# nipponjo/tts-arabic-pytorch

Hardware: AMD Instinct MI355X
Metric: audio samples/sec (FastPitch+HiFi-GAN, synthetic 64-phoneme inputs) (higher is better)
Workload: dtype f32

## Files before the change

include/ttsamd.h:

```cpp
#ifndef TTSAMD_H
#define TTSAMD_H

#include <stdint.h>

#ifdef __cplusplus
extern "C" {
#endif

#define TTSAMD_OK 0
#define TTSAMD_EINVAL (-1)
#define TTSAMD_EHIP (-2)
#define TTSAMD_ENOMEM (-3)

typedef struct ttsamd_tensor {
    const char* name;
    const float* data;
    int32_t ndim;
    int64_t shape[4];
} ttsamd_tensor;

typedef struct ttsamd_hifigan_cfg {
    int32_t num_mels;
    int32_t upsample_initial_channel;
    int32_t n_ups;
// ... 205 lines not shown
    int32_t hop_length;
    double fmin, fmax;
    int32_t n_thresholds;
    int32_t beta_a, beta_b;
    double boltzmann;
    double resolution;
    double max_transition_rate;
    double switch_prob;
    double no_trough_prob;
    int32_t pad_mode;
} ttsamd_pyin_cfg;
int32_t ttsamd_pyin_tables(const ttsamd_pyin_cfg* cfg, int32_t* dims, double* beta, double* expn, double* norm, double* trans,
                           float* logtrans, float* f0);
int32_t ttsamd_pyin_create(const ttsamd_pyin_cfg* cfg, void** handle);
int32_t ttsamd_pyin_destroy(void* handle);
int64_t ttsamd_pyin_workspace_bytes(void* handle, int32_t batch, int32_t n_frames);
int32_t ttsamd_pyin_forward(void* handle, const float* wave, int64_t wave_stride, const int64_t* nsamples, int32_t batch, int32_t t_max,
                            float* f0, uint8_t* voiced_flag, double* voiced_prob, int32_t* states, int64_t* frames_out,
                            void* workspace, int64_t workspace_bytes, void* stream);
int32_t ttsamd_pyin_obs_offsets(void* handle, int32_t batch, int32_t n_frames, int64_t* obs_offsets);

int32_t ttsamd_resample_create(const float* taps, int32_t o, int32_t n, int32_t width, void** handle);
int32_t ttsamd_resample_destroy(void* handle);
int64_t ttsamd_resample_out_len(void* handle, int64_t nsamples);
int32_t ttsamd_resample_mfma_eligible(void* handle);
int32_t ttsamd_resample_forward(void* handle, const float* wave, int64_t wave_stride, const int64_t* nsamples, int32_t batch, float* out,
                                int64_t out_stride, int64_t* nout, int32_t route, void* stream);

int64_t ttsamd_trim_workspace_bytes(int32_t batch, int64_t wave_stride, int32_t hop_length);
int32_t ttsamd_trim_bounds(const float* wave, int64_t wave_stride, const int64_t* nsamples, int32_t batch, float top_db,
                           int32_t frame_length, int32_t hop_length, float gain, int64_t* bounds, float* peak, void* workspace,
                           int64_t workspace_bytes, void* stream);
int32_t ttsamd_trim_apply(const float* wave, int64_t wave_stride, const int64_t* bounds, const float* peak, float gain, int64_t tail,
                          int32_t batch, float* out, int64_t out_stride, int64_t* lens_out, void* stream);
int32_t ttsamd_frames_compact(const float* mel, const float* extra, const int64_t* lens, int32_t batch, int32_t n_channels,
                              int32_t n_extra, int32_t t_max, float thresh, float* mel_out, float* extra_out, int64_t* lens_out,
                              void* stream);

int32_t ttsamd_tacotron2_create(const ttsamd_tensor* weights, int32_t n_weights,
                                const ttsamd_tacotron2_cfg* cfg, void** handle);
int32_t ttsamd_tacotron2_destroy(void* handle);
int64_t ttsamd_tacotron2_workspace_bytes(void* handle, int32_t batch, int32_t n_tokens, int32_t max_step);
int32_t ttsamd_tacotron2_infer(void* handle, const int64_t* tokens, const int64_t* lengths,
                               const int64_t* speaker_ids, int32_t batch, int32_t n_tokens, int32_t max_step,
                               int64_t dropout_seed, float* mel_post, int32_t* mel_lens, float* alignments,
                               float* mel_raw, int32_t* n_steps, void* workspace, int64_t workspace_bytes,
                               void* stream);

int64_t ttsamd_tacotron2_stream_bytes(void* handle, int32_t batch, int32_t n_tokens, int32_t max_step, int32_t max_chunk_steps);
int32_t ttsamd_tacotron2_stream_begin(void* handle, const int64_t* tokens, const int64_t* lengths, const int64_t* speaker_ids, int32_t batch,
                                      int32_t n_tokens, int32_t max_step, int32_t max_chunk_steps, int64_t dropout_seed,
                                      const int32_t* cut_columns, int32_t rows_to_batch_end, float* mel_raw, int32_t* mel_lens,
                                      float* alignments, void* workspace, int64_t workspace_bytes, void** session, void* stream);
int32_t ttsamd_tacotron2_stream_advance(void* session, int32_t n_steps, int32_t* steps_done, int32_t* ended, int32_t* rows, void* stream);
int32_t ttsamd_tacotron2_stream_end(void* session);
int32_t ttsamd_tacotron2_postnet_halo_frames(void* handle, int32_t* halo);
int64_t ttsamd_tacotron2_postnet_window_bytes(void* handle, int32_t batch, int32_t n_frames);
int32_t ttsamd_tacotron2_postnet_window(void* handle, const float* mel_raw, float* mel_post, int32_t batch, int32_t t_cap, int32_t t_known,
                                        int32_t t0, int32_t t1, int32_t ended, void* workspace, int64_t workspace_bytes, void* stream);

int32_t ttsamd_tagger_create(const ttsamd_tensor* weights, int32_t n_weights, const ttsamd_tagger_cfg* cfg,
                             void** handle);
int32_t ttsamd_tagger_destroy(void* handle);
int64_t ttsamd_tagger_workspace_bytes(void* handle, int32_t batch, int32_t n_chars);
int32_t ttsamd_tagger_forward(void* handle, const int64_t* ids, int32_t batch, int32_t n_chars, float* probs,
                              void* workspace, int64_t workspace_bytes, void* stream);


int64_t ttsamd_conv1d_packed_floats(int32_t cout, int32_t cin, int32_t k);
int32_t ttsamd_conv1d(const float* x, const float* w, const float* bias, const int64_t* lens,
                      int32_t batch, int32_t cin, int32_t cout, int32_t k, int32_t dilation,
                      int32_t lin, float in_slope, int32_t relu_out, float* y, float* packed,
                      void* stream);
int32_t ttsamd_conv1d_ex(const float* x, const float* w, const float* bias, const float* res, const int64_t* lens, int32_t batch,
                         int32_t cin, int32_t cout, int32_t k, int32_t dilation, int32_t lin, float in_slope,
                         int32_t relu_out, int32_t mode, float div, float* y, float* packed, void* stream);
int32_t ttsamd_conv1d_splitk(const float* x, const float* w, const float* bias, const float* res, const int64_t* lens, int32_t batch,
                             int32_t cin, int32_t cout, int32_t k, int32_t dilation, int32_t lin, float in_slope,
                             int32_t relu_out, int32_t mode, float div, float* y, float* packed, float* splitk_ws, int64_t splitk_floats,
                             void* stream);
int32_t ttsamd_conv_last_launch(int32_t* route, int32_t* ksplit);
int32_t ttsamd_conv1d_route(int32_t batch, int32_t cin, int32_t cout, int32_t k, int32_t dilation, int32_t lin, float in_slope,
                            int32_t relu_out, int32_t has_res, int32_t mode, int64_t splitk_floats, int32_t* route, int32_t* ksplit);
int64_t ttsamd_convt_packed_floats(int32_t cin, int32_t cout, int32_t u);
int64_t ttsamd_convt_wino_packed_floats(int32_t cin, int32_t cout, int32_t u);
int32_t ttsamd_convt_wino_pack_weight(const float* w, const float* bias, int32_t cin, int32_t cout, int32_t u, float* out);
int32_t ttsamd_conv_transpose1d(const float* x, const float* w, const float* bias, const int64_t* lens, int32_t batch, int32_t cin,
                                int32_t cout, int32_t u, int32_t lin, float in_slope, float* y, float* packed, void* stream);

int64_t ttsamd_resblock_pair_packed_floats(int32_t channels, int32_t k, int32_t variant);
int32_t ttsamd_resblock_pair(const float* x, float* y, const float* w1, const float* b1, const float* w2, const float* b2,
                             int32_t channels, int32_t k, int32_t dil, const int64_t* lens, int32_t len_mul, int32_t L,
                             int32_t batch, int32_t mode, float div, float slope, int32_t variant, float* packed, int64_t packed_floats,
                             void* stream);
int32_t ttsamd_resblock_pair_route(int32_t batch, int32_t channels, int32_t k, int32_t dilation, int32_t L, int32_t* kernel, int32_t* ntw,
                                   int32_t* wino_phases, int32_t* points, const char** name);

int64_t ttsamd_resblock2_packed_floats(int32_t channels, int32_t k, int32_t variant);
int32_t ttsamd_resblock2(const float* x, float* y, const float* w1, const float* b1, const float* w2, const float* b2, int32_t channels,
                         int32_t k, int32_t dil1, int32_t dil2, const int64_t* lens, int32_t len_mul, int32_t L, int32_t batch, int32_t mode,
                         float div, float slope, int32_t variant, float* packed, int64_t packed_floats, void* stream);

int32_t ttsamd_bfo_pack(const float* x, int32_t batch, int32_t channels, int32_t len, float slope, void* out, void* stream);
int32_t ttsamd_bfo_unpack(const void* in, int32_t batch, int32_t channels, int32_t len, float slope, float* out, void* stream);
int64_t ttsamd_bfo_weight_elems(int32_t cout, int32_t cin, int32_t k, int32_t up);
int32_t ttsamd_bfo_pack_weight(const float* w, int32_t cout, int32_t cin, int32_t k, int32_t up, uint16_t* out);
int32_t ttsamd_bfo_conv1d(const void* x, const void* w_packed, const float* bias, const void* res, const void* sum_in,
                          const int64_t* lens, int32_t len_mul, int32_t batch, int32_t cin, int32_t cout, int32_t k,
                          int32_t dilation, int32_t up, int32_t len_in, int32_t mode, float div, float res_slope,
                          float out_slope, void* y, float* y_f32, const float* res_f32, void* stream);
int32_t ttsamd_bfo_resblock_pair(const void* x, const void* w1, const float* b1, const void* w2, const float* b2,
                                 const void* sum_in, const int64_t* lens, int32_t len_mul, int32_t batch, int32_t channels,
                                 int32_t k, int32_t dilation, int32_t len, int32_t mode, float div, float in_slope,
                                 float mid_slope, float out_slope, void* y, void* stream);
int32_t ttsamd_bfo_resblock_chain(const void* x, const void* const* w1, const float* const* b1, const void* const* w2,
                                  const float* const* b2, const int32_t* dilations, const void* sum_in, const int64_t* lens,
                                  int32_t len_mul, int32_t batch, int32_t channels, int32_t len, int32_t mode, float div,
                                  float in_slope, float mid_slope, float out_slope, void* y, void* stream, int32_t k);
int32_t ttsamd_bfo_conv_post(const void* x, const float* w, const float* bias, const int64_t* lens, int32_t len_mul,
                             int32_t batch, int32_t channels, int32_t len, float* wave, int64_t wave_stride, void* stream);

int32_t ttsamd_bfo3_pack(const float* x, int32_t batch, int32_t channels, int32_t len, float slope, void* out, void* stream);
int32_t ttsamd_bfo3_unpack(const void* in, int32_t batch, int32_t channels, int32_t len, float slope, float* out, void* stream);
int64_t ttsamd_bfo3_weight_elems(int32_t cout, int32_t cin, int32_t k, int32_t up);
int32_t ttsamd_bfo3_pack_weight(const float* w, int32_t cout, int32_t cin, int32_t k, int32_t up, uint16_t* out);
int32_t ttsamd_bfo3_conv1d(const void* x, const void* w_packed, const float* bias, const void* res, const void* sum_in,
                           const int64_t* lens, int32_t len_mul, int32_t batch, int32_t cin, int32_t cout, int32_t k,
                           int32_t dilation, int32_t up, int32_t len_in, int32_t mode, float div, float res_slope,
                           float out_slope, void* y, float* y_f32, const float* res_f32, void* stream);
int32_t ttsamd_bfo3_resblock_pair(const void* x, const void* w1, const float* b1, const void* w2, const float* b2,
                                  const void* sum_in, const int64_t* lens, int32_t len_mul, int32_t batch, int32_t channels,
                                  int32_t k, int32_t dilation, int32_t len, int32_t mode, float div, float in_slope,
                                  float mid_slope, float out_slope, void* y, void* stream);
int32_t ttsamd_bfo3_resblock_chain(const void* x, const void* const* w1, const float* const* b1, const void* const* w2,
                                   const float* const* b2, const int32_t* dilations, const void* sum_in, const int64_t* lens,
                                   int32_t len_mul, int32_t batch, int32_t channels, int32_t len, int32_t mode, float div,
                                   float in_slope, float mid_slope, float out_slope, void* y, void* stream);
int32_t ttsamd_bfo3_conv_post(const void* x, const float* w, const float* bias, const int64_t* lens, int32_t len_mul,
                              int32_t batch, int32_t channels, int32_t len, float* wave, int64_t wave_stride, void* stream);

int32_t ttsamd_set_precision(int32_t precision);
int32_t ttsamd_get_precision(void);

#define TTSAMD_DP_ID_BYTES 128
#define TTSAMD_DP_HIFIGAN 0
#define TTSAMD_DP_FASTPITCH 1
int32_t ttsamd_dp_unique_id(void* id128 );
int32_t ttsamd_dp_init(int32_t rank, int32_t world, const void* id128 , void** comm);
int32_t ttsamd_dp_destroy(void* comm);
int32_t ttsamd_dp_rank(void* comm);
int32_t ttsamd_dp_world(void* comm);
int32_t ttsamd_dp_broadcast(void* comm, void* buf, int64_t nbytes, int32_t root, void* stream);
int32_t ttsamd_dp_broadcast_weights(void* comm, int32_t kind, void* handle, int32_t root, void* stream);
int32_t ttsamd_dp_allgather(void* comm, const void* send, void* recv, int64_t nbytes_per_rank, void* stream);
int32_t ttsamd_dp_pack_audio(const float* wave, int64_t wave_stride, const int64_t* nsamples, int32_t batch,
                             int64_t n_max, float* packed, void* stream);
int32_t ttsamd_dp_gather_audio(void* comm, const float* packed, float* recv, const int64_t* counts,
                               const int64_t* offsets, int32_t root, void* stream);

int32_t ttsamd_hifigan_halo_frames(void* handle, int32_t* left , int32_t* right );
int32_t ttsamd_denoiser_halo_frames(void);
#define TTSAMD_STREAM_MAX_WINDOWS 64
int32_t ttsamd_stream_gather(const float* pool, int32_t n_slots, int32_t num_mels, int32_t t_cap, const int32_t* slot ,
                             const int32_t* start , const int32_t* len , int32_t n_windows, int32_t w_max,
                             float* batch, int64_t* lens, void* stream);
int32_t ttsamd_stream_emit(const float* wave, int32_t n_windows, int32_t w_max, int32_t hop, const int32_t* core_off ,
// ... 84 lines not shown
```

profiles/launch_classes.py:

```python
import csv
import re
import sys
from collections import defaultdict


def classes(path):
    d = defaultdict(lambda: [0, 0])
    other = 0
    with open(path) as f:
        for r in csv.DictReader(f):
            dur = int(r['End_Timestamp']) - int(r['Start_Timestamp'])
            m = re.search(r'conv1d_wino4_f32<(\d+), (\d+), (\d+), (\d+), (\d+), (\d+)>', r['Kernel_Name'])
            if not m:
                other += dur
                continue
            k, noct, nst, epi, lp, pt = map(int, m.groups())
            key = (pt, k, lp, 'residual' if epi == 3 else 'plain', int(r['Grid_Size_X']) // int(r['Workgroup_Size_X']))
            d[key][0] += 1
            d[key][1] += dur
    return d, other


a, oa = classes(sys.argv[1])
b, ob = classes(sys.argv[2])
print(f'{"groups":>6} {"k":>3} {"window":>7} {"epilogue":>9} {"blocks":>7} {"calls":>6} {"us parent":>10} {"us tree":>9} {"ratio":>6}')
ta = tb = 0
for key in sorted(set(a) | set(b), key=lambda t: (-t[0], t[1], t[2], t[3], t[4])):
    ca, da = a.get(key, (0, 0))
    cb, db = b.get(key, (0, 0))
    ta += da
    tb += db
    ua, ub = (da / ca / 1e3 if ca else float('nan')), (db / cb / 1e3 if cb else float('nan'))
    print(f'{"seven" if key[0] == 7 else "six":>6} {key[1]:3d} {"vector" if key[2] == 1 else "strip":>7} {key[3]:>9} {key[4]:7d} {max(ca, cb):6d} '
          f'{ua:10.1f} {ub:9.1f} {ub / ua:6.3f}')
print(f'sum over the conv1d_wino4_f32 launches: {ta / 1e6:.2f} -> {tb / 1e6:.2f} ms; every other kernel: {oa / 1e6:.2f} -> {ob / 1e6:.2f} ms (whole trace)')
```

tts-arabic-pytorch_amd/csrc/api.hip:

```cpp
#include <cerrno>
#include <cstdio>
#include <cstdlib>
#include <cstring>
#include <algorithm>
#include <atomic>
#include <mutex>
#include <string>
#include <vector>

#include "kernels.hpp"

namespace ttsamd {

static thread_local std::string g_err;

void set_error(const char* fmt, ...) {
    char buf[1024];
    va_list ap;
    va_start(ap, fmt);
    vsnprintf(buf, sizeof(buf), fmt, ap);
    va_end(ap);
    g_err = buf;
}

// ... 155 lines not shown

__global__ void pack_conv_weight_kernel(const float* __restrict__ w, int cout, int cin, int k, int cp,
                                        float* __restrict__ out) {
    const int64_t i = (int64_t)blockIdx.x * 256 + threadIdx.x;
    const int64_t n = (int64_t)cin * k * cp;
    if (i >= n) return;
    const int pq = (int)(i % 4);
    const int co = (int)((i / 4) % cp);
    const int kk = (int)((i / (4 * (int64_t)cp)) % 2);
    const int t = (int)((i / (8 * (int64_t)cp)) % k);
    const int o = (int)(i / (8 * (int64_t)cp * k));
    out[i] = co < cout ? w[((int64_t)co * cin + (8 * o + 2 * pq + kk)) * k + t] : 0.f;
}

__global__ void pack_convt_weight_kernel(const float* __restrict__ w, int cin, int cout, int u, int cp, float* __restrict__ out) {
    const int64_t i = (int64_t)blockIdx.x * 256 + threadIdx.x;
    const int64_t n = (int64_t)u * cin * 2 * cp;
    if (i >= n) return;
    const int pq = (int)(i % 4);
    const int co = (int)((i / 4) % cp);
    const int kk = (int)((i / (4 * (int64_t)cp)) % 2);
    const int t = (int)((i / (8 * (int64_t)cp)) % 2);
    const int o = (int)((i / (16 * (int64_t)cp)) % (cin / 8));
    const int rho = (int)(i / (16 * (int64_t)cp * (cin / 8)));
    const int kidx = (rho + u / 2) % u + t * u;
    out[i] = co < cout ? w[((int64_t)(8 * o + 2 * pq + kk) * cout + co) * (2 * u) + kidx] : 0.f;
}

__global__ void pack_convt_wino_kernel(const float* __restrict__ w, const float* __restrict__ bias, int cin, int cout, int u,
                                       float* __restrict__ out) {
    const int64_t i = (int64_t)blockIdx.x * 256 + threadIdx.x;
    const int rows = u * cout;
    const int64_t n = (int64_t)6 * cin * rows;
    if (i >= n + rows) return;
    if (i >= n) {
        out[i] = bias ? bias[(i - n) / u] : 0.f;
        return;
    }
    const int pq = (int)(i & 3);
    const int64_t r = i >> 2;
    const int row = (int)(r % rows);
    const int64_t r2 = r / rows;
    const int kk = (int)(r2 & 1);
    const int64_t r3 = r2 >> 1;
    const int t = (int)(r3 % 6), o = (int)(r3 / 6);
    const int co = row / u, j = row % u;
    const float* g = w + ((int64_t)(8 * o + 2 * pq + kk) * cout + co) * 2 * u;
    const double g0 = g[j + u], g1 = g[j];
    out[i] = t == 0 ? (float)(g0 / 4) : (t == 1 ? (float)(-(g0 + g1) / 6) : (t == 2 ? (float)(-(g0 - g1) / 6) :
             (t == 3 ? (float)(g0 / 24 + g1 / 12) : (t == 4 ? (float)(g0 / 24 - g1 / 12) : 0.f))));
}

__global__ void split_bf16_kernel(const float* __restrict__ packed, int64_t n, unsigned short* __restrict__ out) {
    const int64_t i = (int64_t)blockIdx.x * 256 + threadIdx.x;
    if (i >= n) return;
    const float f = packed[i];
    unsigned u = __float_as_uint(f);
    u += 0x7fffu + ((u >> 16) & 1u);
    const unsigned h = u >> 16;
    const float r = f - __uint_as_float(h << 16);
    unsigned v = __float_as_uint(r);
    v += 0x7fffu + ((v >> 16) & 1u);
    out[i] = (unsigned short)h;
    out[n + i] = (unsigned short)(v >> 16);
}

namespace {
struct OptDesc { const char* name; int kind; long long lo, hi; };
const OptDesc kOpts[OPT_COUNT] = {
#define TTS_OPT_DESC(name, kind, lo, hi) {"TTSAMD_" #name, kind, lo, hi},
    TTS_OPTIONS(TTS_OPT_DESC)
#undef TTS_OPT_DESC
};
std::atomic<const char*> g_opt[OPT_COUNT];
std::once_flag g_opt_once;
std::string g_opt_env_error;

bool opt_valid(const OptDesc& d, const char* v) {
    if (!v || !*v) return false;
    char* end = nullptr;
    errno = 0;
    const long long x = std::strtoll(v, &end, d.kind == 1 ? 16 : 10);
    if (!(errno == 0 && end != v && *end == '\0' && x >= d.lo && x <= d.hi)) return false;
    if (&d == &kOpts[OPT_WINO4] && (((x & 32) && !(x & 2)) || ((x & 64) && !(x & 4)) || ((x & 128) && !(x & 8)))) return false;
    return true;
}
void opt_init() {
    std::call_once(g_opt_once, [] {
        for (int i = 0; i < OPT_COUNT; ++i) {
            const char* e = std::getenv(kOpts[i].name);
            if (!e || !*e) continue;
            if (!opt_valid(kOpts[i], e)) {
                if (g_opt_env_error.empty()) {
                    char buf[256];
                    std::snprintf(buf, sizeof buf, "%s='%s' in the environment is not a valid value (%s in [%llx, %llx])", kOpts[i].name, e,
                                  kOpts[i].kind == 1 ? "hex mask" : "integer", kOpts[i].lo, kOpts[i].hi);
                    g_opt_env_error = buf;
                }
                continue;
            }
            g_opt[i].store(strdup(e), std::memory_order_release);
        }
    });
}
int opt_find(const char* name) {
    if (!name) return -1;
    for (int i = 0; i < OPT_COUNT; ++i)
        if (std::strcmp(name, kOpts[i].name) == 0 || std::strcmp(name, kOpts[i].name + 7) == 0) return i;
    return -1;
}
}

int64_t opt_int(Opt o, int64_t unset) {
    opt_init();
    const char* v = g_opt[o].load(std::memory_order_acquire);
    return v ? (int64_t)std::strtoll(v, nullptr, kOpts[o].kind == 1 ? 16 : 10) : unset;
}

}

using namespace ttsamd;

extern "C" {

const char* ttsamd_last_error(void) { return g_err.c_str(); }
int32_t ttsamd_version(void) { return TTSAMD_ABI_VERSION; }

int32_t ttsamd_set_option(const char* name, const char* value) {
    opt_init();
    const int i = opt_find(name);
    TTS_REQUIRE(i >= 0, "set_option: unknown option '%s' (ttsamd_option_name lists them)", name ? name : "(null)");
    if (!value || !*value) {
        g_opt[i].store(nullptr, std::memory_order_release);
        return 0;
    }
    TTS_REQUIRE(opt_valid(kOpts[i], value), "set_option: %s='%s' is not a valid value (%s in [%llx, %llx])", kOpts[i].name, value,
                kOpts[i].kind == 1 ? "hex mask" : "integer", kOpts[i].lo, kOpts[i].hi);
    g_opt[i].store(strdup(value), std::memory_order_release);
    return 0;
}
int32_t ttsamd_get_option(const char* name, char* value, int32_t capacity) {
    opt_init();
    const int i = opt_find(name);
    TTS_REQUIRE(i >= 0 && value && capacity > 0, "get_option: unknown option '%s' or no buffer", name ? name : "(null)");
    const char* v = g_opt[i].load(std::memory_order_acquire);
    std::snprintf(value, (size_t)capacity, "%s", v ? v : "");
    return 0;
}
const char* ttsamd_option_name(int32_t index) { return (index >= 0 && index < OPT_COUNT) ? kOpts[index].name : nullptr; }
int32_t ttsamd_options_check(void) {
    opt_init();
    TTS_REQUIRE(g_opt_env_error.empty(), "%s", g_opt_env_error.c_str());
    return 0;
}

int32_t ttsamd_device_ok(void) {
    int n = 0;
    if (hipGetDeviceCount(&n) != hipSuccess || n <= 0) return 0;
    hipDeviceProp_t prop;
    if (hipGetDeviceProperties(&prop, 0) != hipSuccess) return 0;
    return std::string(prop.gcnArchName).rfind("gfx950", 0) == 0 ? 1 : 0;
}

int32_t ttsamd_hifigan_create(const ttsamd_tensor* weights, int32_t n, const ttsamd_hifigan_cfg* cfg, void** handle) {
    HifiGan* h = nullptr;
    const int32_t rc = hifigan_create(weights, n, cfg, &h);
    if (rc == 0) *handle = h;
// ... 508 lines not shown
            const double g0 = g[3 * s], g1 = g[3 * s + 1], g2 = g[3 * s + 2];
            v = j == 0 ? (float)g0 : (j == 1 ? (float)((g0 + g1 + g2) * 0.5) : (j == 2 ? (float)((g0 - g1 + g2) * 0.5) : (float)g2));
        } else {
            const int l = (t - 4 * ns) >> 1;
            v = ((t - 4 * ns) & 1) ? -g[3 * ns + l] : g[3 * ns + l];
        }
    }
    out[i] = v;
}

int32_t ttsamd_conv1d_ex(const float* x, const float* w, const float* bias, const float* res, const int64_t* lens, int32_t batch,
                         int32_t cin, int32_t cout, int32_t k, int32_t dilation, int32_t lin, float in_slope,
                         int32_t relu_out, int32_t mode, float div, float* y, float* packed, void* stream) {
    return ttsamd_conv1d_splitk(x, w, bias, res, lens, batch, cin, cout, k, dilation, lin, in_slope, relu_out, mode, div, y, packed, nullptr,
                                0, stream);
}

static int32_t conv1d_params(ConvParams& p, const float* x, const float* bias, const float* res, const int64_t* lens, int32_t batch,
                             int32_t cin, int32_t cout, int32_t k, int32_t dilation, int32_t lin, float in_slope, int32_t relu_out,
                             int32_t mode, float div, float* y, float* packed, float* splitk_ws, int64_t splitk_floats) {
    TTS_REQUIRE(mode >= 0 && mode <= 2 && (mode != 2 || div != 0.f), "conv1d: bad mode / div");
    TTS_REQUIRE(relu_out == 0 || mode == 0, "conv1d: relu_out with an accumulate mode (mode %d) is not defined", mode);
    const int cp = cout_padded(cout);
    const int64_t n = (int64_t)cin * k * cp;
    std::memset(&p, 0, sizeof(p));
    p.x = x; p.x_bs = (int64_t)cin * lin; p.x_cs = lin;
    p.w = packed; p.bias = bias;
    p.precision = default_precision();
    if (p.precision != 0) p.w_bf16 = packed + n;
    if ((k == 3 || k == 7 || k == 11) && p.precision == 0 && cin % 8 == 0) {
        p.w_wino = packed + 2 * n;
        p.w_wino4 = p.w_wino + (int64_t)cin * wino2_groups(k) * cp;
        if (wino44_groups(k) != 0) p.w_wino44 = p.w_wino4 + (int64_t)cin * wino4_groups(k) * cp;
    }
    p.y = y; p.y_bs = (int64_t)cout * lin; p.y_cs = lin; p.y_ts = 1;
    p.lens_in = lens; p.lens_out = lens; p.len_in_mul = 1; p.len_out_mul = 1;
    p.Lin = lin; p.Nout = lin; p.Cin = cin; p.Cout = cout; p.CoutP = cp; p.K = k;
    p.dil = dilation; p.pad = (k * dilation - dilation) / 2;
    p.res = res; p.r_bs = (int64_t)cout * lin; p.r_cs = lin;
    p.n_phase = 1; p.in_slope = in_slope; p.relu_out = relu_out; p.mode = mode; p.div = div; p.batch = batch;
    if (splitk_ws != nullptr && splitk_floats > 0) { p.splitk_ws = splitk_ws; p.splitk_floats = splitk_floats; }
    return 0;
}

int32_t ttsamd_conv1d_splitk(const float* x, const float* w, const float* bias, const float* res, const int64_t* lens, int32_t batch,
                             int32_t cin, int32_t cout, int32_t k, int32_t dilation, int32_t lin, float in_slope,
                             int32_t relu_out, int32_t mode, float div, float* y, float* packed, float* splitk_ws, int64_t splitk_floats,
                             void* stream) {
    TTS_REQUIRE(x && w && y && packed, "conv1d: null argument");
    TTS_REQUIRE(splitk_floats >= 0 && (splitk_ws != nullptr || splitk_floats == 0), "conv1d: %lld split-K floats without a workspace",
                (long long)splitk_floats);
    ConvParams p;
    TTS_TRY(conv1d_params(p, x, bias, res, lens, batch, cin, cout, k, dilation, lin, in_slope, relu_out, mode, div, y, packed, splitk_ws,
                          splitk_floats));
    hipStream_t s = (hipStream_t)stream;
    const int cp = p.CoutP;
    const int64_t n = (int64_t)cin * k * cp;
    const auto blocks = [](int64_t floats) { return dim3((unsigned)((floats + 255) / 256)); };
    hipLaunchKernelGGL(pack_conv_weight_kernel, blocks(n), dim3(256), 0, s, w, cout, cin, k, cp, packed);
    TTS_CHECK_HIP(hipGetLastError());
    if (p.w_bf16 != nullptr) {
        hipLaunchKernelGGL(split_bf16_kernel, blocks(n), dim3(256), 0, s, packed, n, reinterpret_cast<unsigned short*>(packed + n));
        TTS_CHECK_HIP(hipGetLastError());
    }
    if (p.w_wino != nullptr) {
        hipLaunchKernelGGL(pack_wino2_weight_kernel, blocks((int64_t)cin * wino2_groups(k) * cp), dim3(256), 0, s, w, cout, cin, k, cp,
                           const_cast<float*>(p.w_wino));
        TTS_CHECK_HIP(hipGetLastError());
        hipLaunchKernelGGL(pack_wino4_weight_kernel, blocks((int64_t)cin * wino4_groups(k) * cp), dim3(256), 0, s, w, cout, cin, k, cp,
                           const_cast<float*>(p.w_wino4));
        TTS_CHECK_HIP(hipGetLastError());
    }
    if (p.w_wino44 != nullptr) {
        hipLaunchKernelGGL(pack_wino44_weight_kernel, blocks((int64_t)cin * wino44_groups(k) * cp), dim3(256), 0, s, w, cout, cin, k, cp,
                           const_cast<float*>(p.w_wino44));
        TTS_CHECK_HIP(hipGetLastError());
    }
    prof_begin(s, 2.0 * cout * cin * k);
    const int32_t rc = launch_conv(p, s);
    prof_end(s);
    return rc;
}

int32_t ttsamd_conv1d_route(int32_t batch, int32_t cin, int32_t cout, int32_t k, int32_t dilation, int32_t lin, float in_slope,
                            int32_t relu_out, int32_t has_res, int32_t mode, int64_t splitk_floats, int32_t* route, int32_t* ksplit) {
    TTS_REQUIRE(route && ksplit, "conv1d_route: null argument");
    TTS_REQUIRE(batch >= 1 && cin >= 1 && cout >= 1 && k >= 1 && lin >= 1 && dilation >= 1 && dilation <= 5 && splitk_floats >= 0,
                "conv1d_route: bad shape");
    float* const any = reinterpret_cast<float*>((uintptr_t)256);
    ConvParams p;
    TTS_TRY(conv1d_params(p, any, any, has_res ? any : nullptr, nullptr, batch, cin, cout, k, dilation, lin, in_slope, relu_out, mode, 1.f, any,
                          any, any, splitk_floats));
    TTS_REQUIRE(p.precision == 0, "conv1d_route: the bf16 launchers keep their own choices (precision %d)", p.precision);
    const ConvRoute r = conv_route(p, conv_route_opts());
    TTS_REQUIRE(r.id >= 0 && (relu_out < 2 || k == 1 || k == 5), "conv1d_route: no fp32 kernel takes k = %d, Cin = %d, relu_out = %d", k, cin, relu_out);
    *route = r.id;
    *ksplit = r.ksplit;
    return 0;
}

int32_t ttsamd_conv1d(const float* x, const float* w, const float* bias, const int64_t* lens, int32_t batch,
                      int32_t cin, int32_t cout, int32_t k, int32_t dilation, int32_t lin, float in_slope,
                      int32_t relu_out, float* y, float* packed, void* stream) {
    return ttsamd_conv1d_ex(x, w, bias, nullptr, lens, batch, cin, cout, k, dilation, lin, in_slope, relu_out, 0, 1.f, y, packed, stream);
}

int32_t ttsamd_conv_last_launch(int32_t* route, int32_t* ksplit) {
    TTS_REQUIRE(route && ksplit, "conv_last_launch: null argument");
    last_conv_launch(route, ksplit);
    return 0;
}

int64_t ttsamd_convt_packed_floats(int32_t cin, int32_t cout, int32_t u) {
    if (cin < 1 || cout < 1 || u < 1) return 0;
    return 2 * (int64_t)u * cin * 2 * cout_padded(cout) + (convt_wino_packable(cin, cout, u) ? (int64_t)(6 * cin + 1) * u * cout : 0);
}

int64_t ttsamd_convt_wino_packed_floats(int32_t cin, int32_t cout, int32_t u) {
    return convt_wino_packable(cin, cout, u) ? (int64_t)(6 * cin + 1) * u * cout : 0;
}

int32_t ttsamd_convt_wino_pack_weight(const float* w, const float* bias, int32_t cin, int32_t cout, int32_t u, float* out) {
    TTS_REQUIRE(w && out, "convt_wino_pack_weight: null argument");
    TTS_REQUIRE(convt_wino_packable(cin, cout, u), "convt_wino_pack_weight: cin %d (a multiple of 16), cout %d, u %d (2 / 8, u cout a multiple of 64)",
                cin, cout, u);
    pack_convt_wino_weight(w, bias, cin, cout, u, out, out + (int64_t)6 * cin * u * cout);
    return 0;
}

int32_t ttsamd_conv_transpose1d(const float* x, const float* w, const float* bias, const int64_t* lens, int32_t batch, int32_t cin,
                                int32_t cout, int32_t u, int32_t lin, float in_slope, float* y, float* packed, void* stream) {
    TTS_REQUIRE(x && w && y && packed, "conv_transpose1d: null argument");
    TTS_REQUIRE(batch >= 1 && cin >= 8 && cin % 8 == 0 && cout >= 1 && lin >= 1, "conv_transpose1d: batch %d, cin %d (a multiple of 8), cout %d, lin %d",
                batch, cin, cout, lin);
    TTS_REQUIRE(u >= 2 && u % 2 == 0, "conv_transpose1d: stride %d (kernel 2 u, padding u / 2: u even)", u);
    TTS_REQUIRE((int64_t)lin * u < ((int64_t)1 << 31) / 4 / cout, "conv_transpose1d: %d x %d x %d outputs per row", cout, lin, u);
    hipStream_t s = (hipStream_t)stream;
    const int cp = cout_padded(cout);
    const int64_t n = (int64_t)u * cin * 2 * cp;
    hipLaunchKernelGGL(pack_convt_weight_kernel, dim3((unsigned)((n + 255) / 256)), dim3(256), 0, s, w, cin, cout, u, cp, packed);
    TTS_CHECK_HIP(hipGetLastError());
    unsigned short* planes = nullptr;
    if (default_precision() != 0) {
        planes = reinterpret_cast<unsigned short*>(packed + n);
        hipLaunchKernelGGL(split_bf16_kernel, dim3((unsigned)((n + 255) / 256)), dim3(256), 0, s, packed, n, planes);
        TTS_CHECK_HIP(hipGetLastError());
    }
    float* wino = nullptr;
    if (default_precision() == 0 && convt_wino_packable(cin, cout, u) && opt_int(OPT_CONVT_WINO, 1) != 0) {
        wino = packed + 2 * n;
        const int64_t nw = (int64_t)(6 * cin + 1) * u * cout;
        hipLaunchKernelGGL(pack_convt_wino_kernel, dim3((unsigned)((nw + 255) / 256)), dim3(256), 0, s, w, bias, cin, cout, u, wino);
        TTS_CHECK_HIP(hipGetLastError());
    }
    ConvParams p;
    std::memset(&p, 0, sizeof(p));
    p.batch = batch;
    p.lens_in = lens; p.lens_out = lens;
    prof_begin(s, 2.0 * cout * cin * 2 * u);
    const int32_t rc = launch_upsampler(p, x, packed, planes, bias, y, cin, cout, u, 2 * u, lin, 1, in_slope, opt_int(OPT_CONVT, 1) != 0, s, wino,
                                        wino ? wino + (int64_t)6 * cin * u * cout : nullptr);
    prof_end(s);
    return rc;
}

int64_t ttsamd_resblock_pair_packed_floats(int32_t channels, int32_t k, int32_t variant) {
    if (channels < 1 || k < 1) return 0;
    const int64_t n = 2 * (int64_t)channels * k * channels;
    const int nwino = (variant == 4 ? 1 : (variant == 5 ? 2 : 0));
    if (variant == 6) return n + ((k == 3 || k == 7 || k == 11) ? 2 * (int64_t)channels * wino4_groups(k) * channels : 0);
    if (variant == 7) return n + 2 * (int64_t)channels * wino44_groups(k) * channels;
    return n + ((k == 3 || k == 7 || k == 11) ? nwino * (int64_t)channels * wino2_groups(k) * channels : 0);
}

int32_t ttsamd_resblock_pair(const float* x, float* y, const float* w1, const float* b1, const float* w2, const float* b2,
                             int32_t channels, int32_t k, int32_t dil, const int64_t* lens, int32_t len_mul, int32_t L,
                             int32_t batch, int32_t mode, float div, float slope, int32_t variant, float* packed, int64_t packed_floats,
                             void* stream) {
    TTS_REQUIRE(x && y && w1 && b1 && w2 && b2 && packed && channels % 32 == 0 && k >= 1 && batch >= 1 && L >= 1 && len_mul >= 1 &&
                mode >= 0 && mode <= 2, "resblock_pair: bad argument");
    TTS_REQUIRE(packed_floats >= ttsamd_resblock_pair_packed_floats(channels, k, variant),
                "resblock_pair: `packed` holds %lld floats, variant %d at C = %d, k = %d needs %lld (ttsamd_resblock_pair_packed_floats)",
                (long long)packed_floats, variant, channels, k, (long long)ttsamd_resblock_pair_packed_floats(channels, k, variant));
    hipStream_t s = (hipStream_t)stream;
    PairConv c[2] = {{nullptr, b1, nullptr, nullptr, nullptr}, {nullptr, b2, nullptr, nullptr, nullptr}};
    float* next = packed;
    const auto pack = [&](void (*kernel)(const float*, int, int, int, int, float*), int groups, const float* w, const float*& form) {
        const int64_t nw = (int64_t)channels * groups * channels;
        hipLaunchKernelGGL(kernel, dim3((unsigned)((nw + 255) / 256)), dim3(256), 0, s, w, channels, channels, k, channels, next);
        form = next;
        next += nw;
        return hipGetLastError();
// ... 137 lines not shown
```

tts-arabic-pytorch_amd/csrc/common.hpp:

```cpp
#pragma once
#include <hip/hip_runtime.h>
#include <stdint.h>
#include <atomic>
#include <cstdarg>
#include <cstdio>
#include <cstdlib>
#include <string>

#include "../../include/ttsamd.h"

namespace ttsamd {

void set_error(const char* fmt, ...);

#define TTS_CHECK_HIP(expr)                                                         \
    do {                                                                            \
        hipError_t e_ = (expr);                                                     \
        if (e_ != hipSuccess) {                                                     \
            ttsamd::set_error("%s failed: %s (%s:%d)", #expr, hipGetErrorString(e_), \
                              __FILE__, __LINE__);                                  \
            return TTSAMD_EHIP;                                                     \
        }                                                                           \
    } while (0)

#define TTS_REQUIRE(cond, ...)              \
    do {                                    \
        if (!(cond)) {                      \
            ttsamd::set_error(__VA_ARGS__); \
            return TTSAMD_EINVAL;           \
        }                                   \
    } while (0)

#define TTS_TRY(expr)               \
    do {                            \
        int32_t rc_ = (expr);       \
        if (rc_ != 0) return rc_;   \
    } while (0)

inline int64_t align_up(int64_t x, int64_t a) { return (x + a - 1) / a * a; }

inline hipError_t lds_opt_in(const void* fn, int bytes, std::atomic<uint64_t>& done) {
    int dev = 0;
    hipError_t e = hipGetDevice(&dev);
    if (e != hipSuccess) return e;
    if (dev >= 0 && dev < 64 && ((done.load(std::memory_order_acquire) >> dev) & 1)) return hipSuccess;
    e = hipFuncSetAttribute(fn, hipFuncAttributeMaxDynamicSharedMemorySize, bytes);
    if (e == hipSuccess && dev >= 0 && dev < 64) done.fetch_or(1ull << dev, std::memory_order_release);
    return e;
}

#define TTS_OPTIONS(X)                                                                                     \
    X(HIFIGAN_STREAMS, 0, 0, 1)    \
    X(WINO, 0, 0, 1)                                              \
    X(WINO2, 0, 0, 31)             \
    X(WINO4, 0, 0, 255)            \
    X(FUSED_PAIR, 0, 0, 1)                   \
    X(FUSED2, 0, 0, 1)                                           \
    X(FUSED2_MASK, 1, 0, 0x1ff)               \
    X(FUSED2_MASK_N1, 1, 0, 0x1ff)          \
    X(FUSED2_WB, 0, 0, 2)                     \
    X(PAIR4, 0, 0, 2)              \
    X(CONVT, 0, 0, 1)                              \
    X(CONVT_WINO, 0, 0, 2)         \
    X(BFO, 0, 0, 1)                \
    X(BFO_CHAIN, 0, 0, 1)                           \
    X(BFO_CHAIN7, 0, 0, 1)                                 \
    X(BFO_FF, 0, 0, 1)                              \
    X(BFO_SPLITK, 0, 0, 1)                                              \
    X(BFO_SMALL_TILES, 0, 0, 1)            \
    X(BF16_ATTN, 0, 0, 1)                                         \
    X(BF16_PACKED_T, 0, 0, 1)                   \
    X(ATT_RA, 0, 1, 4)                             \
    X(ATT_SPLIT, 0, 0, 1)                      \
    X(XCD_W, 0, 0, 1)                            \
    X(XCD_WMAX_KB, 0, 0, 1 << 20)     \
    X(DEEP_SPLITK, 0, 0, 1)        \
    X(TACO_PERSISTENT, 0, 0, 2)    \
    X(TACO_SEG, 0, 8, 1 << 20)     \
    X(RESBLOCK2_PAIR, 1, 0, 0x3f)
enum Opt : int {
#define TTS_OPT_ENUM(name, kind, lo, hi) OPT_##name,
    TTS_OPTIONS(TTS_OPT_ENUM)
#undef TTS_OPT_ENUM
    OPT_COUNT
};
int64_t opt_int(Opt o, int64_t unset);

struct Arena {
    char* base;
    int64_t size;
    int64_t off = 0;
    bool ok = true;
    Arena(void* p, int64_t n) : base((char*)p), size(n) {}
    template <typename T>
    T* take(int64_t count) {
        int64_t bytes = align_up(count * (int64_t)sizeof(T), 256);
        if (base != nullptr && off + bytes > size) ok = false;
        T* r = base ? (T*)(base + off) : nullptr;
        off += bytes;
        return r;
    }
};

struct ConvParams {
    const float* x;
    int64_t x_bs;
    int32_t x_cs;
    const float* w;
    const void* w_bf16;
    const float* w_wino;
    const float* w_wino4;
    int32_t precision;
    const float* bias;
    float* y;
    int64_t y_bs;
    int32_t y_cs, y_ts;
    const float* res;
    int64_t r_bs;
    int32_t r_cs;
    const int64_t* lens_in;
    const int64_t* lens_out;
    int32_t len_in_mul, len_out_mul;
    int32_t Lin, Nout;
    int32_t Cin, Cout, CoutP, K;
    int32_t dil, pad;
    int32_t n_phase;
    int32_t phase_p;
    float in_slope;
    const float* scale;
    int32_t relu_out;
    int32_t mode;
    float div;
    int32_t batch;
    float* splitk_ws;
    int64_t splitk_floats;
    int32_t ksplit;
    int32_t y_packed;
    float pack_slope;
    int32_t x_packed;
    int32_t xcd_w;
    int32_t tile_major;
    int32_t compact;
    unsigned long long* timing;
    const float* w_wino44;
    int32_t res_late;
};
constexpr int64_t kSplitKFloats = 4 << 20;
constexpr int64_t kSplitKFloatsFp = 8 << 20;

void conv_log(const char* kind, int K, int cin, int cout, int nout, int batch, int has_res, int mode, int len_mul, int ragged,
              int n_phase);
bool compact_order(const void* lens, int batch);
int32_t launch_conv(const ConvParams& p, hipStream_t stream);
struct ConvRouteOpts { int wino, wino2, wino4, deep_splitk; };
struct ConvRoute {
    int id;
    int ksplit;
    int epi;
    int co_blk, nt_blk;
};
ConvRouteOpts conv_route_opts();
ConvRoute conv_route(const ConvParams& p, const ConvRouteOpts& o);
inline bool conv_rows_aligned(const ConvParams& p) {
    return (p.y_cs & 3) == 0 && (p.y_bs & 3) == 0 && ((uintptr_t)p.y & 15) == 0 &&
           (!p.res || ((p.r_cs & 3) == 0 && (p.r_bs & 3) == 0 && ((uintptr_t)p.res & 15) == 0));
}
constexpr int conv_chunk_channels(int k, int nt_blk, int co_blk) {
    return (k == 3 && nt_blk == 128 && co_blk == 128) ? 16 : (k == 1 ? 32 : (k == 2 ? 16 : 8));
}
void note_conv_launch(int32_t route, int32_t ksplit);
void last_conv_launch(int32_t* route, int32_t* ksplit);
bool convt_supported(const ConvParams& p);
int32_t launch_convt(const ConvParams& p, hipStream_t stream);
int32_t launch_upsampler(ConvParams& p, const float* x, const float* w, const void* w_bf16, const float* bias, float* y, int cin, int cout,
                         int u, int kt, int L, int len_mul, float in_slope, bool convt_ok, hipStream_t stream, const float* w_wino = nullptr,
                         const float* bias_wino = nullptr);
bool convt_wino_packable(int cin, int cout, int u);
void pack_convt_wino_weight(const float* w, const float* bias, int cin, int cout, int u, float* out_w, float* out_bias);
bool convt_wino_supported(const ConvParams& p, const float* w_wino, const float* bias_wino);
int32_t launch_convt_wino(const ConvParams& p, const float* w_wino, const float* bias_wino, hipStream_t stream);
struct PairRouteOpts { int fused_pair, fused2, fused2_mask, fused2_mask_n1, fused2_wb, pair4; };
struct ConvForms { bool wino2, wino4, wino44; };
struct PairShape { int32_t channels, k, dil, L, batch; bool square; const float *x, *y; ConvForms forms; int32_t precision; };
enum PairKernel : int32_t { PAIR_NONE = 0, PAIR_GEN1 = 1, PAIR_GEN2 = 2, PAIR_F43 = 3 };
struct PairRoute { int32_t kernel, ntw, wm, points; const char* name; };
PairRouteOpts pair_route_opts();
PairRoute pair_route(const PairShape& s, const PairRouteOpts& o);
PairRoute pair_route_of_variant(int32_t variant, int32_t channels, int32_t dil);
bool pair2_phases_built(int32_t channels, int32_t dil, int32_t ntw, int32_t wm);
ConvForms hifigan_conv_forms(int cin, int cout, int k);
struct PairConv { const float *w, *b, *w_wino2, *w_wino4, *w_wino44; };
struct PairArgs { int32_t channels, k, dil; const float* x; float* y; PairConv c1, c2; const int64_t* lens; int32_t len_mul, L, batch, mode; float div, slope; };
int32_t launch_pair(const PairRoute& r, const PairArgs& a, hipStream_t stream);
bool fused_pair_supported(int32_t channels, int32_t k, int32_t dil, int32_t L, const float* x, const float* y);
int32_t launch_fused_pair(const PairArgs& a, hipStream_t stream);
bool fused_pair2_supported(int32_t channels, int32_t k, int32_t dil, int32_t L, const float* x, const float* y, int32_t ntw);
int32_t launch_fused_pair2(const PairArgs& a, const PairRoute& r, hipStream_t stream);
bool fused_pair4_supported(int32_t channels, int32_t k, int32_t dil, int32_t L, const float* x, const float* y);
int32_t launch_fused_pair4(const PairArgs& a, const PairRoute& r, hipStream_t stream);
bool resblock2_conv_supported(int32_t channels, int32_t k, int32_t dil, int32_t L, const float* x, const float* y);
int32_t launch_resblock2_conv(int32_t channels, const float* x, float* y, const float* w, const float* b, int32_t k, int32_t dil,
                              const int64_t* lens, int32_t len_mul, int32_t L, int32_t batch, int32_t mode, float div, float slope,
                              hipStream_t stream);
bool resblock2_pair_supported(int32_t channels, int32_t k, int32_t d1, int32_t d2, int32_t L, const float* x, const float* y);
int32_t launch_resblock2_pair(int32_t channels, const float* x, float* y, const float* w1, const float* b1, const float* w2,
                              const float* b2, int32_t k, int32_t d1, int32_t d2, const int64_t* lens, int32_t len_mul, int32_t L,
                              int32_t batch, int32_t mode, float div, float slope, hipStream_t stream);
int32_t launch_wino(const ConvParams& p, hipStream_t stream);
void pack_wino_weight(const float* w, int cout, int cin, float* out);
int wino2_groups(int k);
__device__ __host__ constexpr int wino2_tile(int d, int npair) { return (2 * npair / ((d & 1) ? 4 * d : 2 * d)) * ((d & 1) ? 4 * d : 2 * d); }
int32_t launch_wino2(const ConvParams& p, hipStream_t stream);
void pack_wino2_weight(const float* w, int cout, int cin, int k, float* out);
int wino4_groups(int k);
int wino44_groups(int k);
constexpr int kWino4Default = 255;
__device__ __host__ constexpr int wino4_tile(int d, int ntup) { return (4 * ntup / (4 * d)) * (4 * d); }
__host__ __device__ constexpr int wino4_pk_tuples(int n, int d) { return d * ((n + 4 * d - 1) / (4 * d)); }
__host__ __device__ constexpr int wino4_pk_tiles(int n, int d) { return (wino4_pk_tuples(n, d) + 63) / 64; }
__host__ __device__ constexpr int wino4_pk_col(int t, int d) { return (t / d) * 4 * d + t % d; }
__host__ __device__ constexpr int wino4_pk_q0(int tile, int d) { return (64 * tile / d) * 4 * d; }
__host__ __device__ constexpr int wino4_pk_r0(int tile, int d) { return 64 * tile % d; }
int32_t launch_splitk_reduce(const ConvParams& q, hipStream_t stream);
int32_t launch_wino4(const ConvParams& p, const ConvRoute& r, hipStream_t stream);
void wino4_filter_groups(const float* g, int k, float* o);
void pack_wino4_weight(const float* w, int cout, int cin, int k, float* out);
void wino44_filter_groups(const float* g, int k, float* o);
void pack_wino44_weight(const float* w, int cout, int cin, int k, float* out);
void pack_conv_weight(const float* w, int cout, int cin, int k, float* out);
void pack_convt_weight(const float* w, int cin, int cout, int kt, int u, int p, float* out);
inline int cout_padded(int cout) { return (int)align_up(cout, 32); }
void split_packed_bf16(const float* packed, int64_t n, uint16_t* out);
int32_t default_precision();

#ifdef __HIPCC__
template <int EXTRA = 0, bool PACKED = false>
__device__ __forceinline__ bool live_tile(const int64_t* __restrict__ lens, const int mul, const int n_max, const int tile_w,
                                          const int batch, const unsigned lin, int& b, int& tile, const int pk_dil = 0) {
    const int lane = threadIdx.x & 63;
    unsigned base = 0;
    for (int u0 = 0; u0 < batch; u0 += 64) {
        int n = 0;
        if constexpr (EXTRA != 0) {
            if (u0 + lane < batch) {
                const int len = (int)lens[u0 + lane] * mul;
                n = (max(min(n_max, len > 0 ? len + EXTRA : 0), 0) + tile_w - 1) / tile_w;
            }
        } else if constexpr (PACKED) {
            if (u0 + lane < batch) n = wino4_pk_tiles(max(min(n_max, (int)lens[u0 + lane] * mul), 0), pk_dil);
        } else {
            if (u0 + lane < batch) n = (max(min(n_max, (int)lens[u0 + lane] * mul), 0) + tile_w - 1) / tile_w;
        }
        int incl = n;
#pragma unroll
        for (int d = 1; d < 64; d <<= 1) {
            const int t = __shfl_up(incl, d, 64);
            if (lane >= d) incl += t;
        }
        const unsigned total = (unsigned)__shfl(incl, 63, 64);
        if (lin < base + total) {
            const unsigned long long m = __ballot(base + (unsigned)incl > lin);
            const int l = __ffsll((long long)m) - 1;
            b = u0 + l;
            tile = (int)(lin - base) - (__shfl(incl, l, 64) - __shfl(n, l, 64));
            return true;
        }
        base += total;
    }
    return false;
}
#endif

}
```

tts-arabic-pytorch_amd/csrc/conv_mfma.hip:

```cpp
#include <cstdio>
#include <cstdlib>
#include <cstring>

#include <algorithm>

#include "conv_mfma_common.hpp"
#include "conv_row_epilogue.hpp"

namespace ttsamd {

template <int K, int NT_BLK, int CO_BLK>
struct Geo {
    static constexpr int KC = conv_chunk_channels(K, NT_BLK, CO_BLK);
    static constexpr int NOCT = KC / 8;
    static constexpr int WS = NT_BLK + (K - 1) * DMAX;
    static constexpr int XI = 2 * NOCT * WS;
    static constexpr int NXI = (XI + 255) / 256;
    static constexpr int W4 = NOCT * K * 2 * CO_BLK;
    static constexpr int NW = (W4 + 255) / 256;
    static constexpr int BUF4 = XI + W4;
    static constexpr int NSTAGE = (CO_BLK > 32 && 3 * BUF4 * 16 <= 80 * 1024 && !(K == 7 && CO_BLK == 64 && NT_BLK >= 128)) ? 3 : 2;
    static constexpr int NGRP = NOCT * K;
};

// ... 312 lines not shown
                    const int r = h * 8 + r8;
                    const int co = co_w0 + i * 32 + (r & 3) + 8 * (r >> 2) + 4 * kk;
                    const int coc = min(co, Cout - 1);
                    bv[r8] = bias ? bias[coc] : 0.f;
                    sv[r8] = scale ? scale[coc] : 1.f;
                    rv[r8] = rb ? rb[(int64_t)coc * r_cs + (int64_t)qc * y_ts] : 0.f;
                    pv[r8] = mode != 0 ? yb[(int64_t)coc * y_cs + (int64_t)qc * y_ts] : 0.f;
                }
#pragma unroll
                for (int r8 = 0; r8 < 8; ++r8) {
                    const int r = h * 8 + r8;
                    const int co = co_w0 + i * 32 + (r & 3) + 8 * (r >> 2) + 4 * kk;
                    float v = acc[i][j][r] + bv[r8];
                    if constexpr (K == 1 || K == 5) { if (relu_out == 2) v = 0.5f * v * (1.0f + erff(v * 0.70710678118654752440f)); }
                    v = v * sv[r8] + rv[r8];
                    if (relu_out == 1) v = fmaxf(v, 0.f);
                    if constexpr (K == 1 || K == 5) { if (relu_out == 3) v = tanhf(v); }
                    if (mode == 1) v = pv[r8] + v;
                    else if (mode == 2) v = (pv[r8] + v) / div;
                    if (q_ok && co < Cout) yb[(int64_t)co * y_cs + (int64_t)q * y_ts] = v;
                }
            }
        }
    }
    }
}

template <int K, int MT, int NTL, int WM, int WN, int EPI>
__global__ __launch_bounds__(256, kConvMinWaves) void conv1d_mfma_f32(const ConvParams p) {
    extern __shared__ __attribute__((aligned(16))) float4 smem4[];
    constexpr int NT_BLK = WN * NTL * 32;
    unsigned bx_ = blockIdx.x, by_ = blockIdx.y, bz_ = blockIdx.z;
    if (p.xcd_w) {
        const unsigned lin = bx_ + gridDim.x * (by_ + gridDim.y * bz_), xcd = lin & 7u, slot = lin >> 3;
        const unsigned nct = gridDim.y, g = (unsigned)p.xcd_w & 0xffu, per = nct / g;
        unsigned rest;
        if (p.xcd_w & 0x100) {
            rest = (slot / per) * (8u / g) + xcd / g;
            by_ = xcd % g + g * (slot % per);
        } else {
            const unsigned idx2 = slot * (8u / g) + xcd / g;
            rest = idx2 / per;
            by_ = xcd % g + g * (idx2 % per);
        }
        bx_ = rest % gridDim.x; bz_ = rest / gridDim.x;
    }
    int b = p.tile_major ? (int)((bx_ + bz_) % (unsigned)p.batch) : (int)bz_;
    int q0 = (p.tile_major ? bz_ : bx_) * NT_BLK;
    if (p.compact) {
        int tile = 0;
        if (!live_tile(p.lens_out, p.len_out_mul, p.Nout, NT_BLK, p.batch, bz_ * gridDim.x + bx_, b, tile)) return;
        b = __builtin_amdgcn_readfirstlane(b);
        q0 = __builtin_amdgcn_readfirstlane(tile) * NT_BLK;
    }
    conv_tile<K, MT, NTL, WM, WN, EPI>(p, smem4, b, q0, by_);
}

__global__ __launch_bounds__(256) void splitk_reduce_kernel(const ConvParams p) {
    const int b = blockIdx.z, co = blockIdx.y, q = blockIdx.x * 256 + threadIdx.x;
    int n_out = p.Nout;
    if (p.lens_out) n_out = min(n_out, (int)p.lens_out[b] * p.len_out_mul);
    if (q >= n_out) return;
    const int64_t per = (int64_t)p.batch * p.Cout * p.Nout;
    const float* __restrict__ pp = p.splitk_ws + ((int64_t)b * p.Cout + co) * p.Nout + q;
    float v = 0.f;
    for (int k0 = 0; k0 < p.ksplit; k0 += 8) {
        float tq[8];
#pragma unroll
        for (int j = 0; j < 8; ++j) tq[j] = pp[(int64_t)min(k0 + j, p.ksplit - 1) * per];
#pragma unroll
        for (int j = 0; j < 8; ++j) v = (k0 + j < p.ksplit) ? v + tq[j] : v;
    }
    v += p.bias ? p.bias[co] : 0.f;
    if (p.relu_out == 2) v = 0.5f * v * (1.0f + erff(v * 0.70710678118654752440f));
    v = v * (p.scale ? p.scale[co] : 1.f) + (p.res ? p.res[(int64_t)b * p.r_bs + (int64_t)co * p.r_cs + q] : 0.f);
    if (p.relu_out == 1) v = fmaxf(v, 0.f);
    else if (p.relu_out == 3) v = tanhf(v);
    float* yp = p.y + (int64_t)b * p.y_bs + (int64_t)co * p.y_cs + q;
    if (p.mode == 1) v = *yp + v;
    else if (p.mode == 2) v = (*yp + v) / p.div;
    *yp = v;
}

static thread_local int32_t t_last_route = -1, t_last_ksplit = 0;
void note_conv_launch(int32_t route, int32_t ksplit) { t_last_route = route; t_last_ksplit = ksplit; }
void last_conv_launch(int32_t* route, int32_t* ksplit) { *route = t_last_route; *ksplit = t_last_ksplit; }

int32_t launch_splitk_reduce(const ConvParams& q, hipStream_t stream) {
    dim3 rg((q.Nout + 255) / 256, q.Cout, q.batch);
    hipLaunchKernelGGL(splitk_reduce_kernel, rg, dim3(256), 0, stream, q);
    TTS_CHECK_HIP(hipGetLastError());
    return 0;
}

template <int K, int MT, int NTL, int WM, int WN, int EPI>
static int32_t launch_epi(const ConvParams& q, dim3 grid, size_t lds, hipStream_t stream) {
    static std::atomic<uint64_t> lds_done{0};
    const auto kern = conv1d_mfma_f32<K, MT, NTL, WM, WN, EPI>;
    TTS_CHECK_HIP(lds_opt_in((const void*)kern, (int)lds, lds_done));
    hipLaunchKernelGGL(kern, grid, dim3(256), lds, stream, q);
    TTS_CHECK_HIP(hipGetLastError());
    return 0;
}

bool compact_order(const void* lens, int batch) { return lens != nullptr && batch > 1; }

constexpr int kXcdWeightKB = 3000;

template <int K, int MT, int NTL, int WM, int WN>
static int32_t launch_cfg(const ConvParams& p, int ksplit, hipStream_t stream) {
    constexpr int CO_BLK = WM * MT * 32, NT_BLK = WN * NTL * 32;
    using G = Geo<K, NT_BLK, CO_BLK>;
    TTS_REQUIRE(p.Cin % G::KC == 0, "conv: Cin=%d must be a multiple of %d for K=%d", p.Cin, G::KC, K);
    const size_t lds = (size_t)G::NSTAGE * G::BUF4 * sizeof(float4);
    dim3 grid((p.Nout + NT_BLK - 1) / NT_BLK, (p.CoutP / CO_BLK) * p.n_phase, p.batch);
    ConvParams q = p;
    q.ksplit = ksplit;
    q.tile_major = 0;
    q.compact = compact_order(p.lens_out, p.batch) ? 1 : 0;
    {
        const bool xw = opt_int(OPT_XCD_W, 1) != 0;
        const unsigned nct = grid.y;
        const unsigned g = (nct % 8 == 0) ? 8 : (nct % 4 == 0 ? 4 : (nct % 2 == 0 ? 2 : 1));
        const bool can = xw && p.n_phase == 1 && ((int64_t)grid.x * grid.y * grid.z) % 8 == 0;
        q.xcd_w = (can && g > 1) ? (int)g : 0;
        const int64_t wmax = opt_int(OPT_XCD_WMAX_KB, kXcdWeightKB) * 1024;
        if (can && wmax > 0 && nct > 1) {
            const int64_t wbytes = (int64_t)p.CoutP * p.Cin * K * 4;
            unsigned g2 = g;
            while (g2 > 1 && wbytes / (g2 / 2) <= wmax) g2 /= 2;
            if (nct / g2 > 1 && ((int64_t)grid.x * grid.z * g2) % 8 == 0)
                q.xcd_w = (int)g2 | 0x100 | (q.xcd_w << 16);
        }
    }
    if (q.ksplit > 1 && (q.xcd_w & 0x100)) q.xcd_w >>= 16;
    if (q.xcd_w & 0x100) q.xcd_w &= 0x1ff;
    grid.y *= q.ksplit;
    const bool vec_ok = q.ksplit == 1 && p.y_ts == 1 && p.n_phase == 1 && conv_rows_aligned(p);
    TTS_REQUIRE(p.relu_out < 2 || K == 1 || K == 5, "conv: GELU / tanh epilogues are built for kernel sizes 1 and 5 only (K=%d)", K);
    const bool pre_ok = p.res != nullptr && !p.res_late && p.scale == nullptr && p.relu_out < 2 &&
                        (int64_t)p.Cout * std::max(p.r_cs, p.y_cs) * 4 < ((int64_t)1 << 31);
    const int epi = !vec_ok ? 2 : (p.relu_out >= 2 ? 1 : (pre_ok ? 3 : 0));
    int32_t rc;
    if (epi == 3) rc = launch_epi<K, MT, NTL, WM, WN, 3>(q, grid, lds, stream);
    else if (epi == 0) rc = launch_epi<K, MT, NTL, WM, WN, 0>(q, grid, lds, stream);
    else if (epi == 1) rc = launch_epi<K, MT, NTL, WM, WN, (K == 1 || K == 5) ? 1 : 2>(q, grid, lds, stream);
    else rc = launch_epi<K, MT, NTL, WM, WN, 2>(q, grid, lds, stream);
    if (rc != 0) return rc;
    if (q.ksplit > 1) return launch_splitk_reduce(q, stream);
    return 0;
}

template <int K>
static int32_t launch_k(const ConvParams& p, const ConvRoute& r, hipStream_t stream) {
    if (r.co_blk == 128 && r.nt_blk == 64) return launch_cfg<K, 1, 2, 4, 1>(p, r.ksplit, stream);
    if (r.co_blk == 64 && r.nt_blk == 128) return launch_cfg<K, 1, 2, 2, 2>(p, r.ksplit, stream);
    if (r.co_blk == 128 && r.nt_blk == 128) return launch_cfg<K, 2, 2, 2, 2>(p, r.ksplit, stream);
    if (r.co_blk == 64 && r.nt_blk == 256) return launch_cfg<K, 2, 2, 1, 4>(p, r.ksplit, stream);
    if (r.co_blk == 64 && r.nt_blk == 64) return launch_cfg<K, 1, 1, 2, 2>(p, r.ksplit, stream);
    if (r.co_blk == 32 && r.nt_blk == 256) return launch_cfg<K, 1, 2, 1, 4>(p, r.ksplit, stream);
    return launch_cfg<K, 1, 1, 1, 4>(p, r.ksplit, stream);
}

void conv_log(const char* kind, int K, int cin, int cout, int nout, int batch, int has_res, int mode, int len_mul, int ragged,
              int n_phase) {
    static FILE* f = [] { const char* e = getenv("TTSAMD_CONV_LOG"); return e ? fopen(e, "a") : (FILE*)nullptr; }();
    if (!f) return;
    fprintf(f, "%s,%d,%d,%d,%d,%d,%d,%d,%d,%d,%d\n", kind, K, cin, cout, nout, batch, has_res, mode, len_mul, ragged, n_phase);
    fflush(f);
}

int32_t launch_conv(const ConvParams& p, hipStream_t stream) {
    TTS_REQUIRE(p.CoutP % 32 == 0 && p.CoutP >= p.Cout, "conv: bad CoutP=%d", p.CoutP);
    TTS_REQUIRE(p.n_phase >= 1 && p.batch >= 1, "conv: bad n_phase/batch");
    TTS_REQUIRE(p.dil >= -DMAX && p.dil <= DMAX && p.dil != 0, "conv: dilation %d outside [-%d,%d]", p.dil, DMAX, DMAX);
    if (p.Nout <= 0) return 0;
    const ConvRoute r = p.precision == 0 ? conv_route(p, conv_route_opts()) : ConvRoute{0, 1, 0, 0, 0};
    conv_log(p.precision == 0 ? (r.id >= 3 ? "f32_wino4" : (r.id > 0 ? "f32_wino" : "f32")) : "bf16", p.K, p.Cin, p.Cout, p.Nout, p.batch, p.res != nullptr, p.mode, p.len_out_mul,
             p.lens_out != nullptr, p.n_phase);
    if (p.precision != 0) return launch_conv_bf16_any(p, stream);
    TTS_REQUIRE(!p.x_packed && !p.y_packed, "conv: packed bf16 activations exist only in the bf16 mode");
    if (r.id >= 0) note_conv_launch(r.id, r.ksplit);
    if (r.id > 0) return r.id >= 3 ? launch_wino4(p, r, stream) : (r.id == 2 ? launch_wino2(p, stream) : launch_wino(p, stream));
    switch (p.K) {
        case 1: return launch_k<1>(p, r, stream);
        case 2: return launch_k<2>(p, r, stream);
        case 3: return launch_k<3>(p, r, stream);
        case 5: return launch_k<5>(p, r, stream);
        case 7: return launch_k<7>(p, r, stream);
        case 11: return launch_k<11>(p, r, stream);
        default:
            set_error("conv: kernel size %d not instantiated (1,2,3,5,7,11)", p.K);
            return TTSAMD_EINVAL;
    }
}

void pack_conv_weight(const float* w, int cout, int cin, int k, float* out) {
    const int cp = cout_padded(cout);
    for (int o = 0; o < cin / 8; ++o)
        for (int t = 0; t < k; ++t)
            for (int kk = 0; kk < 2; ++kk) {
                float* dst = out + (((int64_t)o * k + t) * 2 + kk) * cp * 4;
                for (int co = 0; co < cp; ++co)
                    for (int pq = 0; pq < 4; ++pq)
                        dst[co * 4 + pq] = co < cout ? w[((int64_t)co * cin + (8 * o + 2 * pq + kk)) * k + t] : 0.f;
            }
}

static inline uint16_t host_bf16_rne(float f) {
    uint32_t u;
    memcpy(&u, &f, 4);
    u += 0x7fffu + ((u >> 16) & 1u);
    return (uint16_t)(u >> 16);
}
static inline float host_bf16_to_f(uint16_t h) {
    uint32_t u = (uint32_t)h << 16;
    float f;
    memcpy(&f, &u, 4);
    return f;
}

void split_packed_bf16(const float* packed, int64_t n, uint16_t* out) {
    for (int64_t i = 0; i < n; ++i) {
        const uint16_t h = host_bf16_rne(packed[i]);
        out[i] = h;
        out[n + i] = host_bf16_rne(packed[i] - host_bf16_to_f(h));
    }
}

void pack_convt_weight(const float* w, int cin, int cout, int kt, int u, int p, float* out) {
    const int cp = cout_padded(cout);
    for (int rho = 0; rho < u; ++rho) {
        const int ka = (rho + p) % u;
        for (int o = 0; o < cin / 8; ++o)
            for (int t = 0; t < 2; ++t) {
                const int kidx = ka + t * u;
                for (int kk = 0; kk < 2; ++kk) {
                    float* dst = out + ((((int64_t)rho * (cin / 8) + o) * 2 + t) * 2 + kk) * cp * 4;
                    for (int co = 0; co < cp; ++co)
                        for (int pq = 0; pq < 4; ++pq)
                            dst[co * 4 + pq] = (co < cout && kidx < kt)
                                                   ? w[((int64_t)(8 * o + 2 * pq + kk) * cout + co) * kt + kidx]
                                                   : 0.f;
                }
            }
    }
}

}
```

tts-arabic-pytorch_amd/csrc/conv_route.hip:

```cpp
#include <algorithm>

#include "common.hpp"

namespace ttsamd {

ConvRouteOpts conv_route_opts() {
    return {(int)opt_int(OPT_WINO, 1), (int)opt_int(OPT_WINO2, 31), (int)opt_int(OPT_WINO4, kWino4Default), (int)opt_int(OPT_DEEP_SPLITK, 1)};
}

static int wino4_ksplit(const ConvParams& p, int64_t blocks) {
    constexpr int sk_blocks = 192, sk_target = 224;
    if (blocks >= sk_blocks || p.splitk_ws == nullptr) return 1;
    const int n_chunks = p.Cin / (p.K == 1 ? 32 : (p.K == 3 ? 16 : 8));
    const int64_t per = (int64_t)p.batch * p.Cout * p.Nout;
    int64_t ks = std::min<int64_t>((sk_target + blocks - 1) / blocks, n_chunks / 8);
    ks = std::min<int64_t>(ks, p.splitk_floats / std::max<int64_t>(per, 1));
    return ks >= 2 ? (int)ks : 1;
}

static ConvRoute route_direct(const ConvParams& p, const ConvRouteOpts& o) {
    const int K = p.K;
    ConvRoute r = {0, 1, 0, 0, 0};
    if (K != 1 && K != 2 && K != 3 && K != 5 && K != 7 && K != 11) return ConvRoute{-1, 1, 0, 0, 0};
    auto blocks = [&](int co_blk, int nt_blk) -> int64_t {
        return (int64_t)((p.Nout + nt_blk - 1) / nt_blk) * (p.CoutP / co_blk) * p.n_phase * p.batch;
    };
    auto tile = [&](int co_blk, int nt_blk) { r.co_blk = co_blk, r.nt_blk = nt_blk; };
    const int64_t want = blocks(64, 64) <= 1024 ? (int64_t)200 : (int64_t)768;
    const bool tiny = p.Nout <= 96;
    if (p.CoutP % 128 == 0) {
        const bool few_long = p.Cin >= 256 && p.CoutP <= p.Cin && !tiny && blocks(128, 128) < 4 * want;
        if (few_long && K == 3 && blocks(128, 64) >= want) tile(128, 64);
        else if (few_long && K >= 7 && blocks(64, 128) >= want) tile(64, 128);
        else if (K < 11 && !tiny && blocks(128, 128) >= want && (K != 3 || p.Cin % 16 == 0)) tile(128, 128);
        else if (K == 11 && !tiny && blocks(64, 256) >= want) tile(64, 256);
        else if (p.splitk_ws && p.Cin >= 1024 && !tiny && blocks(128, 64) >= 160 && blocks(128, 64) < 320 &&
                 (int64_t)2 * p.batch * p.Cout * p.Nout <= p.splitk_floats && o.deep_splitk != 0) tile(128, 64);
        else if (blocks(128, 64) >= want || (tiny && blocks(64, 64) < 2 * want)) tile(128, 64);
        else tile(64, 64);
    } else if (p.CoutP % 64 == 0) tile(64, !tiny && blocks(64, 256) >= want ? 256 : 64);
    else tile(32, !tiny && blocks(32, 256) >= want ? 256 : 128);
    const int kc = conv_chunk_channels(K, r.nt_blk, r.co_blk);
    if (p.Cin % kc != 0) return ConvRoute{-1, 1, 0, r.co_blk, r.nt_blk};
    const int64_t nblk = blocks(r.co_blk, r.nt_blk), per = (int64_t)p.batch * p.Cout * p.Nout;
    const int n_chunks = p.Cin / kc;
    constexpr int sk_blocks = 320, sk_target = 640, sk_chunks = 8;
    if (p.splitk_ws && p.n_phase == 1 && p.y_ts == 1 && nblk < sk_blocks && n_chunks >= sk_chunks) {
        int64_t ks = std::min<int64_t>((sk_target + nblk - 1) / nblk, n_chunks / 4);
        ks = std::min<int64_t>(ks, p.splitk_floats / per);
        if (ks >= 2) r.ksplit = (int)ks;
    }
    return r;
}

static ConvRoute route_wino(const ConvParams& p, const ConvRouteOpts& o) {
    constexpr ConvRoute direct = {0, 1, 0, 0, 0};
    if (o.wino == 0) return direct;
    const bool rows_vec_ok = conv_rows_aligned(p) && (int64_t)p.Cout * std::max(std::max(p.r_cs, p.y_cs), 1) * 4 < ((int64_t)1 << 31);
    if (p.n_phase != 1 || p.y_ts != 1 || p.CoutP % 64 != 0 || !(p.in_slope >= 0.f && p.in_slope <= 1.f) || !rows_vec_ok) return direct;
    if (p.K == 1) {
        if (!((o.wino4 & 16) && p.w != nullptr && p.dil == 1 && p.pad == 0 && p.Cin % 32 == 0 && !p.x_packed && !p.y_packed)) return direct;
        const int64_t tiles1 = (int64_t)((p.Nout + 255) / 256) * (p.CoutP / 64) * p.batch;
        const int ks1 = wino4_ksplit(p, tiles1);
        return (tiles1 * ks1 >= 512 && p.Nout >= 256) ? ConvRoute{3, ks1, 0, 0, 0} : direct;
    }
    if ((p.w_wino == nullptr && p.w_wino4 == nullptr) || (p.K != 3 && p.K != 7 && p.K != 11)) return direct;
    if ((p.dil != 1 && p.dil != 3 && p.dil != 5) || p.pad != p.dil * (p.K - 1) / 2 || p.Cin % 8 != 0 || p.scale != nullptr || p.relu_out >= 2)
        return direct;
    const int kbit = p.K == 3 ? 1 : (p.K == 7 ? 2 : 4);
    auto takes = [&](int mask) { return (mask & kbit) && (p.dil == 1 || (mask & 8)) && (p.K != 3 || p.Cin % 16 == 0); };
    if (p.w_wino4 != nullptr) {
        if (takes(o.wino4)) {
            const int bo4 = wino4_tile(p.dil, 64);
            const int64_t tiles4 = (int64_t)((p.Nout + bo4 - 1) / bo4) * (p.CoutP / 64) * p.batch;
            const int ks4 = wino4_ksplit(p, tiles4);
            if (tiles4 * ks4 >= 192 && p.Nout >= 256) {
                const bool seven = p.w_wino44 != nullptr && p.K != 3 && (o.wino4 & (p.K == 7 ? 32 : 64)) != 0;
                const int epi = p.dil == 1 ? (ks4 != 1 ? 0 : (p.res != nullptr ? 3 : 4))
                                           : (((o.wino4 & 128) && p.res == nullptr && p.mode == 0 && ks4 == 1) ? 7 : 0);
                return ConvRoute{(epi == 7 ? 7 : 3) + (seven ? 1 : 0), ks4, epi, 0, 0};
            }
        }
        if (p.w_wino == nullptr) return direct;
    }
    const bool rows64 = p.CoutP % 128 != 0;
    const bool w2 = takes(o.wino2) && (!rows64 || (o.wino2 & 16));
    const bool w1 = p.K == 3 && p.dil == 1 && !rows64;
    if (!w2 && !w1) return direct;
    const int bo = wino2_tile(p.dil, rows64 ? 128 : 64);
    const int64_t blocks = (int64_t)((p.Nout + bo - 1) / bo) * (p.CoutP / (rows64 ? 64 : 128)) * p.batch;
    if (blocks < 192 || p.Nout < 256) return direct;
    return ConvRoute{w2 ? 2 : 1, 1, 0, 0, 0};
}

ConvRoute conv_route(const ConvParams& p, const ConvRouteOpts& o) {
    const ConvRoute r = route_wino(p, o);
    return r.id != 0 ? r : route_direct(p, o);
}

constexpr unsigned kFused2Mask = 0x00F;
constexpr int kPair4MinK = 7;
constexpr unsigned kPair44Mask = 0x3;
constexpr unsigned kFused2MaskN1 = 0x000;
constexpr int64_t kFused2SmallColumns = 2 * 256 * 252;

PairRouteOpts pair_route_opts() {
    return {(int)opt_int(OPT_FUSED_PAIR, 1), (int)opt_int(OPT_FUSED2, 1), (int)opt_int(OPT_FUSED2_MASK, -1),
            (int)opt_int(OPT_FUSED2_MASK_N1, kFused2MaskN1), (int)opt_int(OPT_FUSED2_WB, 2), (int)opt_int(OPT_PAIR4, 1)};
}

ConvForms hifigan_conv_forms(int cin, int cout, int k) {
    const bool wino2 = (k == 3 || k == 7 || k == 11) && cin % 8 == 0 && cout % 32 == 0;
    const bool wino4 = wino2 && (cout >= 64 || (cout == 32 && cin == 32 && k >= kPair4MinK));
    return {wino2, wino4, wino4 && wino44_groups(k) != 0};
}

bool pair2_phases_built(int32_t channels, int32_t dil, int32_t ntw, int32_t wm) {
    if (wm == 0) return true;
    if (ntw != 2) return false;
    return wm == 1 ? channels <= 64 : (wm == 2 && (dil == 1 || dil == 3 || dil == 5));
}

static int pair2_phases(int32_t channels, int32_t dil, int32_t ntw, bool have_b, bool have_a) {
    if (have_b && have_a && pair2_phases_built(channels, dil, ntw, 2)) return 2;
    return (have_b && pair2_phases_built(channels, dil, ntw, 1)) ? 1 : 0;
}

static PairRoute make_pair_route(int32_t kernel, int32_t ntw, int32_t wm, int32_t points) {
    if (kernel == PAIR_GEN1) return {PAIR_GEN1, 0, 0, 0, "fused_pair"};
    if (kernel == PAIR_GEN2) return {PAIR_GEN2, ntw, wm, 0, wm == 2 ? "fused_pair2ww" : (wm == 1 ? "fused_pair2w" : (ntw == 2 ? "fused_pair2" : "fused_pair2n"))};
    if (kernel == PAIR_F43) return {PAIR_F43, 0, 0, points, points == 7 ? "fused_pair44" : "fused_pair4"};
    return {PAIR_NONE, 0, 0, 0, ""};
}

static int fused2_width(const PairShape& s, const PairRouteOpts& o) {
    if (o.fused2 == 0) return 0;
    const int ci = s.channels == 32 ? 0 : (s.channels == 64 ? 1 : (s.channels == 128 ? 2 : -1));
    const int ki = s.k == 3 ? 0 : (s.k == 7 ? 1 : (s.k == 11 ? 2 : -1));
    if (ci < 0 || ki < 0) return 0;
    const unsigned bit = 1u << (3 * ci + ki);
    if ((int64_t)s.batch * s.L < kFused2SmallColumns && o.fused2_mask < 0) return 0;
    if (!((o.fused2_mask < 0 ? kFused2Mask : (unsigned)o.fused2_mask) & bit)) return 0;
    const int ntw = ((unsigned)o.fused2_mask_n1 & bit) ? 1 : 2;
    const auto fits = [&](int n) { return fused_pair2_supported(s.channels, s.k, s.dil, s.L, s.x, s.y, n); };
    return fits(ntw) ? ntw : (fits(3 - ntw) ? 3 - ntw : 0);
}

PairRoute pair_route(const PairShape& s, const PairRouteOpts& o) {
    if (s.precision != 0 || o.fused_pair == 0 || !s.square) return make_pair_route(PAIR_NONE, 0, 0, 0);
    const int ntw = fused2_width(s, o);
    if (ntw == 0) {
        return make_pair_route(fused_pair_supported(s.channels, s.k, s.dil, s.L, s.x, s.y) ? PAIR_GEN1 : PAIR_NONE, 0, 0, 0);
    }
    if (ntw == 2 && o.pair4 != 0 && o.fused2_wb == 2 && s.k >= kPair4MinK && s.forms.wino4 &&
        fused_pair4_supported(s.channels, s.k, s.dil, s.L, s.x, s.y)) {
        const bool seven = o.pair4 == 1 && (kPair44Mask & (s.k == 7 ? 1u : (s.k == 11 ? 2u : 0u))) != 0 && s.forms.wino44;
        return make_pair_route(PAIR_F43, 0, 0, seven ? 7 : 6);
    }
    return make_pair_route(PAIR_GEN2, ntw, pair2_phases(s.channels, s.dil, ntw, o.fused2_wb != 0 && s.forms.wino2, o.fused2_wb == 2 && s.forms.wino2), 0);
}

PairRoute pair_route_of_variant(int32_t variant, int32_t channels, int32_t dil) {
    if (variant == 2 || variant == 3) return make_pair_route(PAIR_GEN2, variant == 3 ? 1 : 2, 0, 0);
// ... 15 lines not shown
```

tts-arabic-pytorch_amd/csrc/conv_wino4.hip:

```cpp
#include <cstdlib>
#include <cstring>

#include <algorithm>
#include <vector>

#include "conv_mfma_common.hpp"
#include "conv_row_epilogue.hpp"
#include "bfo.hpp"

namespace ttsamd {

typedef float w4_f32x4 __attribute__((ext_vector_type(4)));
typedef float w4_f32x2 __attribute__((ext_vector_type(2)));

template <int K, int NOCT_, int NSTAGE_, int PT_ = 6, int LP_ = 1, int CT_ = 0, int PK_ = 0>
struct Wino4Geo {
    static_assert(PK_ == 0 || LP_ == 2, "packed tiles: the strip kernels");
    static constexpr bool PT7 = PT_ == 7;
    static_assert(PT_ == 6 || (PT7 && (K == 7 || K == 11)), "seven-point groups: k = 7 / 11");
    static_assert(CT_ == 0 || (K == 3 && PT_ == 6 && LP_ == 1), "transposed conv: the k = 3 six-point form at dilation 1");
    static constexpr int WM = 2, WN = 2;
    static constexpr int NSF = K == 1 ? 0 : (K == 3 ? 1 : (K == 7 ? 2 : (PT7 ? 3 : 4)));
    static constexpr int NL = (!PT7 && (K == 7 || K == 1)) ? 1 : 0;
    static constexpr int GSF = PT7 ? 7 : 6;
    static constexpr int SSF = PT7 ? 4 : 3;
    static constexpr int NG = PT7 ? (K == 7 ? 13 : 20) : (K == 1 ? 4 : (K == 3 ? (CT_ ? 5 : 6) : (K == 7 ? 16 : 23)));
    static constexpr int NGQ = PT7 ? NG : ((NG + 1) & ~1);
    static constexpr bool WSHARE = K == 1;
    static constexpr int NGW = WSHARE ? 1 : NGQ;
    static constexpr int NPL = PT7 ? 7 : (NL ? 8 : (CT_ ? 5 : 6));
    static constexpr int NPOS = K == 1 ? 4 : (K == 3 ? (CT_ ? 5 : 6) : (K == 7 ? 10 : 14));
    static constexpr int NOCT = NOCT_, NSTAGE = NSTAGE_;
    static constexpr int NPH = PT7 ? ((K == 11 && LP_ == 2) ? 2 : 1) : (K == 11 ? 2 : 1);
    static constexpr int PH0 = PT7 ? 8 : 12;
    static constexpr int NGPM = NPH == 1 ? NG : 12;
    static_assert(NPH == 1 || (PH0 <= NGPM && NG - PH0 <= NGPM), "phase sizes");
    static constexpr int CO_BLK = WM * 32;
    static constexpr int NTUP = WN * 32;
    static constexpr int NT_BLK = 4 * NTUP;
    static constexpr int BUF4 = NOCT * 2 * NGPM * NTUP;
    static constexpr int PF = 4;
    static constexpr int NM = 4;
    __host__ __device__ static constexpr int glo(int ph) { return NPH == 1 ? 0 : PH0 * ph; }
    __host__ __device__ static constexpr int ngp(int ph) { return NPH == 1 ? NG : (ph == 0 ? PH0 : NG - PH0); }
    __host__ __device__ static constexpr int ngq(int ph) { return NPH == 1 ? NGQ : (PT7 ? ngp(ph) : 12); }
    __host__ __device__ static constexpr int gfirst(int g) {
        return g < GSF * NSF ? SSF * (g / GSF) : 3 * NSF + (g - 6 * NSF);
    }
    __host__ __device__ static constexpr int glast(int g) {
        if (PT7) return 4 * (g / 7) + (g % 7 == 6 ? 6 : 5);
        return g < 6 * NSF ? (3 * (g / 6) + 5 < NPOS ? 3 * (g / 6) + 5 : NPOS - 1) : 3 * NSF + (g - 6 * NSF);
    }
    __host__ __device__ static constexpr int plane(int g) {
        if (PT7) return g % 7;
        return g < 6 * NSF ? g % 6 : ((g - 6 * NSF) == 0 ? 0 : ((g - 6 * NSF) == 1 ? 6 : ((g - 6 * NSF) == 2 ? 7 : 5)));
    }
    __host__ __device__ static constexpr int mlo(int ph) { return gfirst(glo(ph)); }
    __host__ __device__ static constexpr int mhi(int ph) {
        int m = 0;
        for (int g = glo(ph); g < glo(ph) + ngp(ph); ++g) m = glast(g) > m ? glast(g) : m;
        return m;
    }
    static_assert(mhi(NPH - 1) == NPOS - 1 && mlo(0) == 0, "the groups cover the window and nothing past it");
    __host__ __device__ static constexpr int npos(int ph) { return mhi(ph) - mlo(ph) + 1; }
    static constexpr int NPOSP = npos(0) > npos(NPH - 1) ? npos(0) : npos(NPH - 1);
    __host__ __device__ static constexpr int ngap(int ph) { return NOCT * ngp(ph) * NM; }
    __host__ __device__ static constexpr int sph(int ph) { return ((ph - (NSTAGE - 1)) % NPH + NPH) % NPH; }
    __host__ __device__ static constexpr int sgap(int ph) { return ngap(sph(ph)); }
    static constexpr int JSF = 10;
    __host__ __device__ static constexpr int sflo(int ph) { return glo(ph) / 7; }
    __host__ __device__ static constexpr bool inph(int ph, int g) { return g >= glo(ph) && g < glo(ph) + ngp(ph); }
    __host__ __device__ static constexpr int glast_ph(int ph) { return glo(ph) + ngp(ph) - 1; }
    __host__ __device__ static constexpr int nwj(int ph) {
        return PT7 ? JSF * (glast_ph(ph) / 7 - sflo(ph)) + (glast_ph(ph) % 7 == 0 ? 3 : JSF) : NOCT * ngp(ph);
    }
    static_assert(!PT7 || (NOCT == 1 && glo(0) % 7 <= 1 && glo(NPH - 1) % 7 <= 1 &&
                           (glast_ph(0) % 7 == 0 || glast_ph(0) % 7 >= 5) && glast_ph(NPH - 1) % 7 >= 5),
                  "seven-point phases: start on V0 / V1 of a sub-filter (the partial sums are formed per phase), end on V0 or the last row");
    __host__ __device__ static constexpr int fdiv4(int e) { return e >= 0 ? e / 4 : -((3 - e) / 4); }
    __host__ __device__ static constexpr int vlo(int ph) { return fdiv4(mlo(ph) - (K - 1) / 2); }
    __host__ __device__ static constexpr int nvec(int ph) { return fdiv4(mhi(ph) - (K - 1) / 2) - vlo(ph) + 1; }
    static constexpr int NVP = nvec(0) > nvec(NPH - 1) ? nvec(0) : nvec(NPH - 1);
    __host__ __device__ static constexpr int nljv(int ph) { return NOCT * 2 * nvec(ph); }
    static constexpr int DAV = (K == 3 || K == 1) ? 8 : 16;
    __host__ __device__ static constexpr int tw0v(int ph) { return DAV + 2 * nljv(ph); }
    __host__ __device__ static constexpr int wsv(int ph) { return (sgap(ph) - tw0v(ph)) / nwj(ph); }
    static_assert(LP_ != 1 || (wsv(0) >= 1 && wsv(NPH - 1) >= 1), "one write job per gap at most (vector loads)");
    __host__ __device__ static constexpr int strip_need(int d) {
        return 3 + (PK_ ? wino4_pk_col(d - 1 + 63, d) : wino4_pk_col(4 * 64 / (4 * d) * d - 1, d)) + (NPOS - 1) * d + 1;
    }
    static constexpr int RAWW = (PK_ && K == 11) ? 332 : 320;
    static_assert(RAWW % 4 == 0 && RAWW >= 256 && RAWW <= 512 && strip_need(3) <= RAWW && strip_need(5) <= RAWW, "the strip holds every tuple's window");
    static constexpr int NV2 = (RAWW - 256) / 4;
    static constexpr int NROW = 2 * NOCT;
    static constexpr int RAW_BYTES = 4 * (NROW * RAWW * 4 + 16);
    static constexpr int DAT = K == 7 ? 16 : (K == 11 ? 12 : 8);
    __host__ __device__ static constexpr int nrj(int ph) { return NROW * ((npos(ph) + 1) / 2); }
    __host__ __device__ static constexpr bool loads_in(int ph) { return ph == 0; }
    __host__ __device__ static constexpr int tr_r0(int ph) { return loads_in(ph) ? DAT + 2 * NROW : 0; }
    __host__ __device__ static constexpr int tw0t(int ph) { return tr_r0(ph) + nrj(ph) + 1; }
    __host__ __device__ static constexpr int wst(int ph) { return (sgap(ph) - tw0t(ph)) / nwj(ph); }
    static_assert(LP_ != 2 || (wst(0) >= 1 && wst(NPH - 1) >= 1), "one write job per gap at most (strip path)");
    static constexpr int QX = WSHARE ? 0 : (NOCT * ngq(0)) % PF;
    static constexpr int QMAIN = NOCT * ngq(0) - QX;
    static_assert(QX == 0 || (NPH == 1 && NOCT == 1 && QMAIN >= 2 * PF), "extra queue slots: one phase, one octet");
    static_assert((WSHARE ? NOCT : NOCT * ngq(NPH - 1)) % PF == 0 || QX != 0, "queue slots line up across steps");
    static_assert((size_t)NSTAGE * BUF4 * 16 + (LP_ == 2 ? RAW_BYTES : 0) <= 80 * 1024, "two blocks per CU");
    static_assert(NPH == 1 || NOCT == 1, "phases split an octet's groups");
};

static_assert(Wino4Geo<3, 2, 2, 6, 2, 0, 1>::RAWW == 320 && Wino4Geo<7, 1, 2, 7, 2, 0, 1>::RAWW == 320 && Wino4Geo<7, 1, 2, 6, 2, 0, 1>::RAWW == 320 &&
              Wino4Geo<11, 1, 2, 7, 2, 0, 1>::RAWW == 332 && Wino4Geo<11, 1, 2, 6, 2, 0, 1>::RAWW == 332, "strip lengths of the packed form");

__host__ __device__ constexpr bool wino4_pk_covers(int n, int d) {
    const int T = wino4_pk_tuples(n, d);
    if (4 * T < n || wino4_pk_tiles(n, d) != (T + 63) / 64 || (d == 1 && wino4_pk_tiles(n, 1) != (n + 255) / 256)) return false;
    for (int c = 0; c < n; ++c) {
        const int t = (c / (4 * d)) * d + c % d, j = (c % (4 * d)) / d;
        const int tile = t / 64, pe = t % 64;
        if (t >= T || tile >= wino4_pk_tiles(n, d)) return false;
        if (wino4_pk_q0(tile, d) + wino4_pk_col(wino4_pk_r0(tile, d) + pe, d) + j * d != c) return false;
        if (wino4_pk_col(t, d) + j * d != c) return false;
    }
    return true;
}
__host__ __device__ constexpr bool wino4_pk_covers_range(int d, int n_lo, int n_hi, int step) {
    for (int n = n_lo; n <= n_hi; n += step)
        if (!wino4_pk_covers(n, d)) return false;
    return true;
}
static_assert(wino4_pk_covers_range(1, 1, 130, 1) && wino4_pk_covers_range(1, 131, 700, 13), "packed tiles, d = 1: rows of 1 .. 700 outputs");
static_assert(wino4_pk_covers_range(3, 1, 130, 1) && wino4_pk_covers_range(3, 131, 700, 13), "packed tiles, d = 3: rows of 1 .. 700 outputs");
static_assert(wino4_pk_covers_range(5, 1, 130, 1) && wino4_pk_covers_range(5, 131, 700, 13), "packed tiles, d = 5: rows of 1 .. 700 outputs");
static_assert(wino4_pk_covers_range(3, 1020, 1030, 1) && wino4_pk_covers_range(5, 1020, 1030, 1), "packed tiles: around 1028");
static_assert(wino4_pk_covers(1357, 3) && wino4_pk_covers(1357, 5) && wino4_pk_covers(2048, 3) && wino4_pk_covers(2048, 5), "packed tiles: long rows");
static_assert(wino4_pk_covers(28672, 3), "packed tiles, d = 3: a row of 28672");
static_assert(wino4_pk_covers(28672, 5), "packed tiles, d = 5: a row of 28672");
static_assert(wino4_pk_tiles(1028, 5) == 5 && wino4_pk_tuples(1028, 5) == 260 && wino4_pk_tuples(1028, 3) == 258, "packed tiles of a row of 1028");

template <int K, int NOCT_, int NSTAGE_, int EPI, int LP, int PT = 6>
__global__ __launch_bounds__(256, kConvMinWaves) void conv1d_wino4_f32(const ConvParams p) {
    extern __shared__ __attribute__((aligned(16))) float4 smem4[];
    constexpr int CTU = EPI == 5 ? 8 : (EPI == 6 ? 2 : 0);
    constexpr bool CT = CTU != 0;
    constexpr bool PK = EPI == 7;
    using G = Wino4Geo<K, NOCT_, NSTAGE_, PT, LP, CTU, PK ? 1 : 0>;
    constexpr bool PT7 = G::PT7;
    constexpr int WN = G::WN, NSF = G::NSF, NOCT = G::NOCT, NSTAGE = G::NSTAGE, NPL = G::NPL, NGPM = G::NGPM;
    constexpr int CO_BLK = G::CO_BLK, NTUP = G::NTUP, NT_BLK = G::NT_BLK, PF = G::PF;
    constexpr int NPH = G::NPH, NPOSP = G::NPOSP, NM = G::NM;
    constexpr bool D1 = LP == 1, TR = LP == 2;
    static_assert(D1 || TR, "window path");
    const int dil = D1 ? 1 : p.dil;
    const int nt_eff = wino4_tile(dil, NTUP), ntup_eff = nt_eff / 4;
    const int tiles_y = p.CoutP / CO_BLK;
    const int per_tile = tiles_y * p.ksplit;
    const unsigned sidx = blockIdx.x, xcd = sidx & 7u, u = sidx >> 3;
    const int yk = (int)(u % (unsigned)per_tile);
    const unsigned gt = (u / (unsigned)per_tile) * 8u + xcd;
    const int n_tiles_x = PK ? wino4_pk_tiles(p.Nout, dil) : (p.Nout + nt_eff - 1) / nt_eff;
    const int tile_w = PK ? 1 : nt_eff;
    int b = (int)(gt / (unsigned)n_tiles_x);
    int q0 = (int)(gt % (unsigned)n_tiles_x) * tile_w;
    if (p.compact) {
        int tile = 0;
        if (!live_tile<CT ? 1 : 0, PK>(p.lens_out, p.len_out_mul, p.Nout, nt_eff, p.batch, gt, b, tile, dil)) return;
        b = __builtin_amdgcn_readfirstlane(b);
        q0 = __builtin_amdgcn_readfirstlane(tile) * tile_w;
    } else if (b >= p.batch) {
        return;
    }
    int r0 = 0;
    if constexpr (PK) {
        r0 = wino4_pk_r0(q0, dil);
        q0 = wino4_pk_q0(q0, dil);
    }
    const int tid = threadIdx.x, lane = tid & 63, wid = tid >> 6;
    const int wm = wid / WN, wn = wid % WN;
    const int ks = yk / tiles_y;
    const int co_blk0 = (yk - ks * tiles_y) * CO_BLK;
    int n_out = p.Nout;
    if constexpr (CT) {
        if (p.lens_out) {
            const int len = min(p.Lin, (int)p.lens_out[b] * p.len_out_mul);
            n_out = len > 0 ? len + 1 : 0;
        }
    } else {
        if (p.lens_out) n_out = min(n_out, (int)p.lens_out[b] * p.len_out_mul);
    }
    if (q0 >= n_out) return;
    int in_len = p.Lin;
    if (p.lens_in) in_len = min(in_len, (int)p.lens_in[b] * p.len_in_mul);

    const int x_cs = p.x_cs, CoutP = p.CoutP;
    const int chunks_all = p.Cin / (8 * NOCT);
    const int c_beg = (int)((int64_t)ks * chunks_all / p.ksplit), n_chunks = (int)((int64_t)(ks + 1) * chunks_all / p.ksplit);
    const int n_groups = (p.Cin / 8) * G::NGW;
    const float* __restrict__ xb = p.x + (int64_t)b * p.x_bs;
    const float in_slope = p.in_slope;

    constexpr bool REG = EPI >= 3, RES = EPI == 3;
    static_assert(!REG || ((LP == 1 || PK) && K != 1), "register epilogue: dilation 1 or the packed strip form, k = 3 / 7 / 11");
    static_assert(!PK || LP == 2, "packed tiles: the strip kernels");
    static_assert(EPI <= 7 && (!CT || K == 3), "epilogues 0, 3, 4, 7 and the transposed conv's 5 / 6 (k = 3 form)");
    float ep_bias = 0.f;
    if constexpr (!REG) {
        if (tid < CO_BLK && p.bias) ep_bias = p.bias[min(co_blk0 + tid, p.Cout - 1)];
    }

    const int kk = lane >> 5, l31 = lane & 31;
    const int pe = wn * 32 + l31;
    const int col_e = PK ? wino4_pk_col(r0 + pe, dil) : (dil == 1 ? 4 * pe : (pe / dil) * 4 * dil + pe % dil);
    f32x16 acc[NPL];
#pragma unroll
    for (int g = 0; g < NPL; ++g)
#pragma unroll
        for (int r = 0; r < 16; ++r) acc[g][r] = 0.f;
    const int ep_row0 = REG ? co_blk0 + __builtin_amdgcn_readfirstlane(wm) * 32 : 0;
    const int ep_voff = (q0 + col_e < n_out ? q0 + col_e : 0) * 4;
    const int ep_rrow = ep_row0 + 4 * kk;
    const bfo_i4 ep_rs = bfo_rsrc(RES ? p.res + (int64_t)b * p.r_bs : nullptr, RES ? (unsigned)p.Cout * (unsigned)p.r_cs * 4u : 0u);
    const bfo_i4 ep_bs = bfo_rsrc(p.bias, (REG && p.bias) ? (unsigned)p.Cout * 4u : 0u);
    w4_f32x4 rq[RES ? 16 : 1], bsq[REG ? 4 : 1];
    constexpr int EP_T0 = RES ? 16 : 0;
#define TTS_EPLOAD_JOB(T)                                                                            \
    {                                                                                                \
        if (RES && (T) < 16)                                                                         \
            rq[RES ? (T) : 0] = __builtin_bit_cast(w4_f32x4, bfo_ld16(ep_rs, ep_voff + (ep_rrow + ((T) & 3) + 8 * ((T) >> 2)) * p.r_cs * 4, 0, 0)); \
        if ((T) >= EP_T0 && (T) < EP_T0 + 4)                                                         \
            bsq[REG ? (T) - EP_T0 : 0] = __builtin_bit_cast(w4_f32x4, bfo_ld16(ep_bs, (ep_rrow + 8 * ((T) - EP_T0)) * 4, 0, 0)); \
    }

    const bfo_i4 wrs = bfo_rsrc(K == 1 ? p.w : (PT7 ? p.w_wino44 : p.w_wino4), (unsigned)n_groups * 2u * (unsigned)CoutP * 16u);
    const int wv = (kk * CoutP + co_blk0 + wm * 32 + l31) * 16;
    const int wstep = 2 * CoutP * 16, wlast = (n_groups - 1) * wstep;
    int wso = c_beg * NOCT * G::NGW * wstep;
    w4_f32x4 aq[PF + G::QX];
    if constexpr (G::QX == 0) {
#pragma unroll
        for (int g = 0; g < PF; ++g) {
            aq[g] = __builtin_bit_cast(w4_f32x4, bfo_ld16(wrs, wv, wso, 0));
            wso = min(wso + wstep, wlast);
        }
    } else {
#pragma unroll
        for (int g = 0; g < PF + G::QX; ++g)
            aq[g] = __builtin_bit_cast(w4_f32x4, bfo_ld16(wrs, wv, min(wso + (g < PF ? g : G::QMAIN + g - PF) * wstep, wlast), 0));
    }

    const int sh = __builtin_amdgcn_readfirstlane((tid >> 7) & 1), skk = __builtin_amdgcn_readfirstlane((tid >> 6) & 1);
    w4_f32x2 sx[D1 ? 1 : NOCT][D1 ? 1 : NPOSP];
    w4_f32x4 sv[D1 ? NOCT : 1][2][D1 ? G::NVP : 1];
    w4_f32x2 ta[NOCT], tb[NOCT];
    w4_f32x2 tf[PT7 ? 5 : 1], te[PT7 ? 4 : 1], td[PT7 ? 3 : 1], th[PT7 ? 2 : 1];
    const int spe = PK ? r0 + lane : min(lane, ntup_eff - 1);
    const int xw0 = (q0 + 4 * lane) * 4;
    constexpr int pad_c = (K - 1) / 2;
    const int ch_off = (4 * sh + skk) * x_cs;

#define TTS_VJOB_IDX(PH, J)                                                                          \
        const int nv_ = G::nvec(PH);                                                                 \
        const int ol_ = (J) / (2 * nv_), pp_ = ((J) / nv_) % 2, vi_ = (J) % nv_;
#define TTS_VLOAD_JOB(PH, J, XSO)                                                                    \
    {                                                                                                \
        TTS_VJOB_IDX(PH, J)                                                                          \
        const bfo_i4 xrs_ = bfo_rsrc(xb + ((XSO) + ch_off + (8 * ol_ + 2 * pp_) * x_cs), (unsigned)in_len * 4u);     \
        sv[ol_][pp_][vi_] = __builtin_bit_cast(w4_f32x4, bfo_ld16(xrs_, xw0 + 16 * (G::vlo(PH) + vi_), 0, 0));      \
    }
#define TTS_VACT_JOB(PH, A)                                                                          \
    {                                                                                                \
        TTS_VJOB_IDX(PH, (A) / 2)                                                                    \
        if ((A) % 2 == 0) {                                                                          \
            sv[ol_][pp_][vi_].x = bfo_lrelu(sv[ol_][pp_][vi_].x, in_slope);                          \
            sv[ol_][pp_][vi_].y = bfo_lrelu(sv[ol_][pp_][vi_].y, in_slope);                          \
        } else {                                                                                     \
            sv[ol_][pp_][vi_].z = bfo_lrelu(sv[ol_][pp_][vi_].z, in_slope);                          \
            sv[ol_][pp_][vi_].w = bfo_lrelu(sv[ol_][pp_][vi_].w, in_slope);                          \
        }                                                                                            \
    }
    float* const strip = reinterpret_cast<float*>(smem4 + NSTAGE * G::BUF4) + wid * (G::NROW * G::RAWW + 4);
    const int tr_a = (q0 - pad_c * dil) & ~3;
    const int tr_off = q0 + (dil == 1 ? 4 * spe : (spe / dil) * 4 * dil + spe % dil) - pad_c * dil - tr_a;
    w4_f32x4 rv[TR ? G::NROW : 1][2];
#define TTS_TLOAD_JOB(J, XSO)                                                                        \
    {                                                                                                \
        const int pp_ = (J) / 2, vs_ = (J) % 2;                                                      \
        const bfo_i4 xrs_ = bfo_rsrc(xb + ((XSO) + ch_off + (8 * (pp_ / 2) + 2 * (pp_ % 2)) * x_cs), (unsigned)in_len * 4u); \
        const int v_ = lane + 64 * vs_;                                                              \
        rv[pp_][vs_] = __builtin_bit_cast(w4_f32x4, bfo_ld16(xrs_, (vs_ == 1 && lane >= G::NV2) ? BFO_OOB : (tr_a + 4 * v_) * 4, 0, 0)); \
    }
#define TTS_TSTORE_JOB(J)                                                                            \
    {                                                                                                \
        const int pp_ = (J) / 2, vs_ = (J) % 2;                                                      \
        w4_f32x4 a_ = rv[pp_][vs_];                                                                  \
        a_.x = bfo_lrelu(a_.x, in_slope); a_.y = bfo_lrelu(a_.y, in_slope);                          \
        a_.z = bfo_lrelu(a_.z, in_slope); a_.w = bfo_lrelu(a_.w, in_slope);                          \
        const int v_ = lane + 64 * vs_;                                                              \
        float* dst_ = (vs_ == 1 && lane >= G::NV2) ? strip + G::NROW * G::RAWW : strip + pp_ * G::RAWW + 4 * v_;    \
        *reinterpret_cast<w4_f32x4*>(dst_) = a_;                                                     \
    }
#define TTS_TREAD_JOB(PH, J)                                                                         \
    {                                                                                                \
        const int npr_ = (G::npos(PH) + 1) / 2;                                                      \
        const int pp_ = (J) / npr_, jp_ = (J) % npr_;                                                \
        const float* src_ = strip + pp_ * G::RAWW + tr_off + (G::mlo(PH) + 2 * jp_) * dil;           \
        sx[pp_ / 2][2 * jp_][pp_ % 2] = src_[0];                                                     \
        if (2 * jp_ + 1 < G::npos(PH)) sx[pp_ / 2][2 * jp_ + 1][pp_ % 2] = src_[dil];                \
    }
#define TTS_SXV(M) (w4_f32x2{sv[ol_][0][G::fdiv4((M) - pad_c) - G::vlo(PH_)][((M) - pad_c) - 4 * G::fdiv4((M) - pad_c)],     \
                             sv[ol_][1][G::fdiv4((M) - pad_c) - G::vlo(PH_)][((M) - pad_c) - 4 * G::fdiv4((M) - pad_c)]})
#define TTS_SX(M) (D1 ? TTS_SXV(M) : sx[D1 ? 0 : ol_][D1 ? 0 : (M) - G::mlo(PH_)])
#define TTS_WRITE_JOB(PH, J, WR)                                                                     \
    {                                                                                                \
        const int PH_ = (PH);                                                                        \
        const int ol_ = PT7 ? 0 : (J) / G::ngp(PH_), gl_ = (J) % G::ngp(PH_), g_ = G::glo(PH_) + gl_;                          \
        w4_f32x2 v2;                                                                                 \
        if constexpr (PT7) {                                                                         \
             \
            const int sf_ = G::sflo(PH_) + (J) / G::JSF, kd_ = (J) % G::JSF, s4 = 4 * sf_, g0_ = 7 * sf_;                      \
            const bool v0_ = G::inph(PH_, g0_), tap4_ = g0_ + 6 < G::NG;                             \
            int row_ = -1;                                                                           \
            if (kd_ == 0) {                         \
                if (v0_) tf[0] = sf_ > G::sflo(PH_) ? tf[4] : TTS_SX(s4 + 2) - 4.f * TTS_SX(s4);    \
                tf[1] = TTS_SX(s4 + 3) - 4.f * TTS_SX(s4 + 1);                                       \
                tf[2] = TTS_SX(s4 + 4) - 4.f * TTS_SX(s4 + 2);                                       \
            } else if (kd_ == 1) {                                                                   \
                tf[3] = TTS_SX(s4 + 5) - 4.f * TTS_SX(s4 + 3);                                       \
                if (v0_) te[0] = tf[0] - 2.f * tf[1];                                                \
            } else if (kd_ == 2) {                                                                   \
                te[2] = tf[2] - 2.f * tf[3];                                                         \
                if (v0_) { v2 = te[2] - te[0]; row_ = 0; }                                           \
            } else if (kd_ == 3) {                                                                   \
                te[1] = tf[1] - 2.f * tf[2];                                                         \
                v2 = te[1] + te[2]; row_ = 1;                                                        \
            } else if (kd_ == 4) {                                                                   \
                v2 = te[1] - te[2]; row_ = 2;                                                        \
            } else if (kd_ == 5) {                                                                   \
                v2 = tf[3] - tf[1]; row_ = 5;                                                        \
            } else if (kd_ == 6) {                                                                   \
                if (tap4_) {                                                                         \
                    tf[4] = TTS_SX(s4 + 6) - 4.f * TTS_SX(s4 + 4);                                   \
                    te[3] = tf[3] - 2.f * tf[4];                                                     \
                    v2 = te[1] - te[3]; row_ = 6;                                                    \
                }                                                                                    \
            } else if (kd_ == 7) {                                                                   \
                td[0] = TTS_SX(s4 + 1) - TTS_SX(s4 + 3);                                             \
                td[1] = TTS_SX(s4 + 2) - TTS_SX(s4 + 4);                                             \
                td[2] = TTS_SX(s4 + 3) - TTS_SX(s4 + 5);                                             \
            } else if (kd_ == 8) {                                                                   \
                th[0] = td[0] - 2.f * td[1];                                                         \
                th[1] = td[1] - 2.f * td[2];                                                         \
                v2 = 2.f * th[0] + th[1]; row_ = 3;                                                  \
            } else {                                                                                 \
                v2 = 2.f * th[0] - th[1]; row_ = 4;                                                  \
// ... 159 lines not shown
    if constexpr (CT) {
        const int tau0 = q0 + col_e, y_cs = p.y_cs;
        if constexpr (CTU == 8) {
            if (tau0 >= n_out) return;
        }
        const int olen = CTU * (n_out - 1);
        const int ch0 = ep_row0 / CTU;
#define TTS_CT_QUAD(R, Y)                                                                            \
        {                                                                                            \
            const float s12 = acc[1][R] + acc[2][R], d12 = acc[1][R] - acc[2][R];                    \
            const float s34 = acc[3][R] + acc[4][R], d34 = acc[3][R] - acc[4][R];                    \
            (Y)[0] = acc[0][R] + s12 + s34;                                                          \
            (Y)[1] = d12 + 2.f * d34;                                                                \
            (Y)[2] = s12 + 4.f * s34;                                                                \
            (Y)[3] = d12 + 8.f * d34;                                                                \
        }
        if constexpr (CTU == 8) {
#pragma unroll
            for (int c = 0; c < 4; ++c) {
                float yq[4][4];
#pragma unroll
                for (int i = 0; i < 4; ++i) TTS_CT_QUAD(4 * c + i, yq[i])
                float* yr = yb + (int64_t)(ch0 + c) * y_cs;
#pragma unroll
                for (int e = 0; e < 4; ++e) {
                    const int n = 8 * (tau0 + e) + 4 * kk - 4;
                    if (n >= 0 && n < olen)
                        *reinterpret_cast<w4_f32x4*>(yr + n) = w4_f32x4{yq[0][e] + bsq[c][0], yq[1][e] + bsq[c][1], yq[2][e] + bsq[c][2], yq[3][e] + bsq[c][3]};
                }
            }
        } else {
#pragma unroll
            for (int m = 0; m < 8; ++m) {
                float ya[4], yc[4];
                TTS_CT_QUAD(2 * m, ya)
                TTS_CT_QUAD(2 * m + 1, yc)
                const float b0 = bsq[m >> 1][(2 * m) & 3], b1 = bsq[m >> 1][(2 * m + 1) & 3];
                const float v[8] = {ya[0] + b0, yc[0] + b1, ya[1] + b0, yc[1] + b1, ya[2] + b0, yc[2] + b1, ya[3] + b0, yc[3] + b1};
                const int n0 = 2 * tau0 - 1;
                float* yr = yb + (int64_t)(ch0 + 2 * kk + (m & 1) + 4 * (m >> 1)) * y_cs + n0;
                const float nb = __shfl_down(v[0], 1, 64);
                const bool has_nb = l31 != 31;
                if (l31 == 0 && n0 >= 0 && n0 < olen) yr[0] = v[0];
                if (n0 + 8 < olen) {
                    *reinterpret_cast<w4_f32x4*>(yr + 1) = w4_f32x4{v[1], v[2], v[3], v[4]};
                    if (has_nb) {
                        *reinterpret_cast<w4_f32x4*>(yr + 5) = w4_f32x4{v[5], v[6], v[7], nb};
                    } else {
                        *reinterpret_cast<w4_f32x2*>(yr + 5) = w4_f32x2{v[5], v[6]};
                        yr[7] = v[7];
                    }
                } else {
#pragma unroll
                    for (int e = 1; e < 8; ++e)
                        if (n0 + e < olen) yr[e] = v[e];
                }
            }
        }
#undef TTS_CT_QUAD
        return;
    }
    const int mode = p.mode, relu_out = p.relu_out, Cout = p.Cout;
    const float div = p.div;
    if constexpr (PK) {
        const int q = q0 + col_e, y_cs = p.y_cs;
        if (q >= n_out) return;
        const float lo = relu_out == 1 ? 0.f : -__builtin_inff();
        const bool in1 = q + dil < n_out, in2 = q + 2 * dil < n_out, in3 = q + 3 * dil < n_out;
#pragma unroll
        for (int r = 0; r < 16; ++r) {
            const int co = ep_rrow + (r & 3) + 8 * (r >> 2);
            TTS_OUT_QUAD(r)
            const float bsv = bsq[REG ? r >> 2 : 0][r & 3];
            if (co >= Cout) continue;
            float* yp = yb + (int64_t)co * y_cs + q;
            yp[0] = fmaxf(y0 + bsv, lo);
            if (in1) yp[dil] = fmaxf(y1 + bsv, lo);
            if (in2) yp[2 * dil] = fmaxf(y2 + bsv, lo);
            if (in3) yp[3 * dil] = fmaxf(y3 + bsv, lo);
        }
        return;
    }
    if constexpr (REG) {
        const int q = q0 + col_e, y_cs = p.y_cs;
        if (q >= n_out) return;
        const bool full = q + 3 < n_out;
        const bfo_i4 ys = bfo_rsrc(yb, (unsigned)Cout * (unsigned)y_cs * 4u);
        const float lo = relu_out == 1 ? 0.f : -__builtin_inff();
        constexpr int PB = NPL >= 8 ? 4 : 8;
#pragma unroll
        for (int h = 0; h < 16 / PB; ++h) {
            w4_f32x4 pq[PB];
#pragma unroll
            for (int i = 0; i < PB; ++i) {
                const int r = PB * h + i;
                pq[i] = w4_f32x4{0.f, 0.f, 0.f, 0.f};
                if (mode != 0)
                    pq[i] = __builtin_bit_cast(w4_f32x4, bfo_ld16(ys, ep_voff + (ep_rrow + (r & 3) + 8 * (r >> 2)) * y_cs * 4, 0, 0));
            }
#pragma unroll
            for (int i = 0; i < PB; ++i) {
                const int r = PB * h + i;
                const int co = ep_rrow + (r & 3) + 8 * (r >> 2);
                TTS_OUT_QUAD(r)
                w4_f32x4 v = {y0, y1, y2, y3};
                const float bsv = bsq[REG ? r >> 2 : 0][r & 3];
#pragma unroll
                for (int e = 0; e < 4; ++e) {
                    float x = v[e] + bsv;
                    if constexpr (RES) x += rq[RES ? r : 0][e];
                    v[e] = fmaxf(x, lo);
                }
                if (mode != 0) {
                    v = pq[i] + v;
                    if (mode == 2) {
#pragma unroll
                        for (int e = 0; e < 4; ++e) v[e] = v[e] / div;
                    }
                }
                if (co >= Cout) continue;
                float* yp = yb + (int64_t)co * y_cs + q;
                if (full) {
                    *reinterpret_cast<w4_f32x4*>(yp) = v;
                } else {
#pragma unroll
                    for (int e = 0; e < 4; ++e)
                        if (q + e < n_out) yp[e] = v[e];
                }
            }
        }
        return;
    }
    constexpr int LDS_F = CO_BLK * NT_BLK + CO_BLK;
    static_assert(NT_BLK / 4 == 64, "one wave instruction per row: a lane's columns are the same in every row");
    float* ep = reinterpret_cast<float*>(smem4);
    float* epb = ep + LDS_F - CO_BLK;
    __syncthreads();
    if (tid < CO_BLK) epb[tid] = ep_bias;
#pragma unroll
    for (int r = 0; r < 16; ++r) {
        const int row = wm * 32 + (r & 3) + 8 * (r >> 2) + 4 * kk;
        TTS_OUT_QUAD(r)
        if (pe < ntup_eff) {
            if (dil == 1) {
                *reinterpret_cast<float4*>(ep + row * NT_BLK + col_e) = make_float4(y0, y1, y2, y3);
            } else {
                ep[row * NT_BLK + col_e] = y0;
                ep[row * NT_BLK + col_e + dil] = y1;
                ep[row * NT_BLK + col_e + 2 * dil] = y2;
                ep[row * NT_BLK + col_e + 3 * dil] = y3;
            }
        }
    }
#undef TTS_OUT_QUAD
    __syncthreads();
    const int col = lane * 4, q = q0 + col;
    if (q >= n_out || col >= nt_eff) return;
    if (p.ksplit > 1) {
        constexpr int NR = CO_BLK / 4;
        const bool full = q + 3 < n_out;
        float* __restrict__ pb = p.splitk_ws + ((int64_t)ks * p.batch + b) * Cout * p.Nout;
#pragma unroll 4
        for (int it = 0; it < NR; ++it) {
            const int rl = wid + it * 4;
            const int co = co_blk0 + rl;
            if (co >= Cout) continue;
            const float4 a4 = *reinterpret_cast<const float4*>(ep + rl * NT_BLK + col);
            float* yp = pb + (int64_t)co * p.Nout + q;
            if (full && (p.Nout & 3) == 0) {
                *reinterpret_cast<float4*>(yp) = a4;
            } else {
                const float v[4] = {a4.x, a4.y, a4.z, a4.w};
#pragma unroll
                for (int e = 0; e < 4; ++e)
                    if (q + e < n_out) yp[e] = v[e];
            }
        }
        return;
    }
    conv_row_epilogue<NT_BLK, CO_BLK, K == 1 ? kRowScaleGlobal : kRowScaleNone, K == 1, false, true>(p, ep, epb, K == 1 ? p.scale : nullptr, b,
                                                                                                      co_blk0, CO_BLK, q0, n_out, nt_eff);
}

template <int K, int NOCT, int NSTAGE, int EPI, int LP, int PT = 6>
static int32_t launch_wino4_epi(const ConvParams& p, int ksplit, hipStream_t stream) {
    constexpr bool PK = EPI == 7;
    using G = Wino4Geo<K, NOCT, NSTAGE, PT, LP, 0, PK ? 1 : 0>;
    constexpr size_t ring = (size_t)G::NSTAGE * G::BUF4 * sizeof(float4);
    constexpr size_t epi = ((size_t)G::CO_BLK * G::NT_BLK + G::CO_BLK) * sizeof(float);
    constexpr size_t strip = LP == 2 ? (size_t)G::RAW_BYTES : 0;
    constexpr size_t lds = (EPI >= 3 || ring + strip > epi) ? ring + strip : epi;
    static_assert(lds <= 80 * 1024, "two blocks per CU");
    static_assert(EPI < 3 || lds == ring + strip, "register epilogue: the ring (and the strip) set the LDS size");
    static std::atomic<uint64_t> lds_done{0};
    const auto kern = conv1d_wino4_f32<K, NOCT, NSTAGE, EPI, LP, PT>;
    TTS_CHECK_HIP(lds_opt_in((const void*)kern, (int)lds, lds_done));
    const int nt = wino4_tile(p.dil, G::NTUP);
    ConvParams q = p;
    q.ksplit = ksplit;
    const int64_t n_tiles = (int64_t)(PK ? wino4_pk_tiles(p.Nout, p.dil) : (p.Nout + nt - 1) / nt) * p.batch;
    const int64_t n_blocks = ((n_tiles + 7) / 8) * 8 * (p.CoutP / G::CO_BLK) * q.ksplit;
    TTS_REQUIRE(n_blocks < ((int64_t)1 << 31), "wino4: %lld blocks", (long long)n_blocks);
    dim3 grid((unsigned)n_blocks, 1, 1);
    q.compact = compact_order(p.lens_out, p.batch) ? 1 : 0;
    hipLaunchKernelGGL(kern, grid, dim3(256), lds, stream, q);
    TTS_CHECK_HIP(hipGetLastError());
    if (q.ksplit > 1) return launch_splitk_reduce(q, stream);
    return 0;
}

template <int K, int NOCT, int NSTAGE, int PT = 6>
static int32_t launch_wino4_cfg(const ConvParams& p, const ConvRoute& r, hipStream_t stream) {
    if (p.dil == 1) {
        if (r.epi == 0) return launch_wino4_epi<K, NOCT, NSTAGE, 0, 1, PT>(p, r.ksplit, stream);
        if (r.epi == 3) return launch_wino4_epi<K, NOCT, NSTAGE, 3, 1, PT>(p, r.ksplit, stream);
        return launch_wino4_epi<K, NOCT, NSTAGE, 4, 1, PT>(p, r.ksplit, stream);
    }
    if (r.epi == 7) return launch_wino4_epi<K, NOCT, 2, 7, 2, PT>(p, r.ksplit, stream);
    return launch_wino4_epi<K, NOCT, 2, 0, 2, PT>(p, r.ksplit, stream);
}

int32_t launch_wino4(const ConvParams& p, const ConvRoute& r, hipStream_t stream) {
    if (r.id == 4 || r.id == 8) return p.K == 7 ? launch_wino4_cfg<7, 1, 2, 7>(p, r, stream) : launch_wino4_cfg<11, 1, 2, 7>(p, r, stream);
    if (p.K == 1) return launch_wino4_epi<1, 4, 2, 0, 1>(p, r.ksplit, stream);
    if (p.K == 3) return launch_wino4_cfg<3, 2, 3>(p, r, stream);
    if (p.K == 7) return launch_wino4_cfg<7, 1, 2>(p, r, stream);
    if (p.K == 11) return launch_wino4_cfg<11, 1, 3>(p, r, stream);
    set_error("wino4: kernel size %d not built (1, 3, 7, 11)", p.K);
    return TTSAMD_EINVAL;
}

bool convt_wino_packable(int cin, int cout, int u) { return (u == 2 || u == 8) && cin >= 16 && cin % 16 == 0 && cout >= 1 && (u * cout) % 64 == 0; }

bool convt_wino_supported(const ConvParams& p, const float* w_wino, const float* bias_wino) {
    const int u = p.n_phase;
    return w_wino != nullptr && bias_wino != nullptr && p.precision == 0 && convt_wino_packable(p.Cin, p.Cout, u) && p.K == 2 && p.dil == -1 &&
           p.phase_p * 2 == u && p.y_ts == u && p.res == nullptr && p.mode == 0 && p.scale == nullptr && p.relu_out == 0 &&
           !p.x_packed && !p.y_packed && p.in_slope >= 0.f && p.in_slope <= 1.f && p.Lin == p.Nout &&
           (p.x_cs & 3) == 0 && (p.x_bs & 3) == 0 && ((uintptr_t)p.x & 15) == 0 &&
           (p.y_cs & 3) == 0 && (p.y_bs & 3) == 0 && ((uintptr_t)p.y & 15) == 0 &&
           (int64_t)p.Lin * 4 + 64 < ((int64_t)1 << 31) && (int64_t)p.Cout * p.y_cs * 4 < ((int64_t)1 << 31);
}

template <int U>
static int32_t launch_convt_wino_u(const ConvParams& p, const float* w_wino, const float* bias_wino, hipStream_t stream) {
    constexpr int EPI = U == 8 ? 5 : 6;
    using G = Wino4Geo<3, 2, 3, 6, 1, U>;
    constexpr size_t lds = (size_t)G::NSTAGE * G::BUF4 * sizeof(float4);
    static_assert(lds <= 80 * 1024, "two blocks per CU");
    static std::atomic<uint64_t> lds_done{0};
    const auto kern = conv1d_wino4_f32<3, 2, 3, EPI, 1, 6>;
    TTS_CHECK_HIP(lds_opt_in((const void*)kern, (int)lds, lds_done));
    ConvParams q = p;
    q.w_wino4 = w_wino; q.bias = bias_wino;
    q.Cout = U * p.Cout; q.CoutP = q.Cout;
    q.Nout = p.Lin + 1;
    q.K = 3; q.dil = 1; q.pad = 1; q.n_phase = 1; q.ksplit = 1;
    const int64_t n_tiles = (int64_t)((q.Nout + G::NT_BLK - 1) / G::NT_BLK) * p.batch;
    const int64_t n_blocks = ((n_tiles + 7) / 8) * 8 * (q.CoutP / G::CO_BLK);
    TTS_REQUIRE(n_blocks < ((int64_t)1 << 31), "convt wino: %lld blocks", (long long)n_blocks);
    q.compact = compact_order(p.lens_out, p.batch) ? 1 : 0;
    hipLaunchKernelGGL(kern, dim3((unsigned)n_blocks, 1, 1), dim3(256), lds, stream, q);
    TTS_CHECK_HIP(hipGetLastError());
    return 0;
}

int32_t launch_convt_wino(const ConvParams& p, const float* w_wino, const float* bias_wino, hipStream_t stream) {
    TTS_REQUIRE(convt_wino_supported(p, w_wino, bias_wino), "convt wino: unsupported geometry");
    if (p.Nout <= 0) return 0;
    conv_log("convt_wino", 2, p.Cin, p.Cout, p.Nout, p.batch, 0, 0, p.len_out_mul, p.lens_out != nullptr, p.n_phase);
    note_conv_launch(6, 1);
    return p.n_phase == 8 ? launch_convt_wino_u<8>(p, w_wino, bias_wino, stream) : launch_convt_wino_u<2>(p, w_wino, bias_wino, stream);
}

void pack_convt_wino_weight(const float* w, const float* bias, int cin, int cout, int u, float* out_w, float* out_bias) {
    const int rows = u * cout;
    std::vector<float> t((size_t)rows * cin * 3);
    for (int ci = 0; ci < cin; ++ci)
        for (int co = 0; co < cout; ++co)
            for (int j = 0; j < u; ++j) {
                const float* g = w + ((int64_t)ci * cout + co) * 2 * u;
                float* d = t.data() + ((int64_t)(co * u + j) * cin + ci) * 3;
                d[0] = g[j + u]; d[1] = g[j]; d[2] = 0.f;
            }
    pack_wino4_weight(t.data(), rows, cin, 3, out_w);
    for (int r = 0; r < rows; ++r) out_bias[r] = bias ? bias[r / u] : 0.f;
}

int wino4_groups(int k) { return k == 3 ? 6 : (k == 7 ? 16 : 24); }
int wino44_groups(int k) { return k == 7 ? 13 : (k == 11 ? 20 : 0); }

void wino4_filter_groups(const float* g, int k, float* o) {
    const int nsf = k == 3 ? 1 : (k == 7 ? 2 : 4);
    for (int s = 0; s < nsf; ++s) {
        const double g0 = g[3 * s], g1 = 3 * s + 1 < k ? g[3 * s + 1] : 0.0, g2 = 3 * s + 2 < k ? g[3 * s + 2] : 0.0;
        o[6 * s] = (float)(g0 / 4);
        o[6 * s + 1] = (float)(-(g0 + g1 + g2) / 6);
// ... 39 lines not shown
```

tts-arabic-pytorch_amd/ttsamd/engine.py:

```python
import ctypes as C

import numpy as np
import torch

from . import lib as L
from .config import NET_CONFIG, HIFIGAN_CONFIG, VOCOS_22K_CONFIG, TACOTRON2_CONFIG


def _require_gpu():
    if not torch.cuda.is_available():
        raise L.TtsAmdError('no ROCm device visible: the ttsamd engines run only on an MI355X (gfx950); '
                            'there is no CPU fallback')
    lib = L.load()
    if not lib.ttsamd_device_ok():
        raise L.TtsAmdError('device 0 is not gfx950')
    return lib


PRECISIONS = {'f32': 0, 'bf16': 1, 'bf16x3': 2}


def set_precision(name):
    lib = L.load()
    L.check(lib.ttsamd_set_precision(PRECISIONS[name]), 'set_precision')
# ... 760 lines not shown


class TaggerEngine:

    RENAME = {'emb0.weight': 'emb.weight', 'emb_input.weight': 'emb.weight'}

    def __init__(self, state_dict, config, device='cuda'):
        self.lib = _require_gpu()
        self.device = torch.device(device if device != 'cuda' else 'cuda:0')
        c = dict(config)
        cfg = L.TaggerCfg()
        cfg.n_vocab, cfg.emb_dim = c['n_vocab'], c['emb_dim']
        cfg.n_lstm, cfg.n_dense = len(c['lstm_hidden']), len(c['dense_dim'])
        for i, v in enumerate(c['lstm_hidden']):
            cfg.lstm_hidden[i] = v
        for i, v in enumerate(c['dense_dim']):
            cfg.dense_dim[i] = v
        cfg.hard_sigmoid, cfg.bn_after_lstm0, cfg.bn_eps = c['hard_sigmoid'], c['bn_after_lstm0'], c['bn_eps']
        self.n_classes = c['dense_dim'][-1]
        self.n_vocab = c['n_vocab']
        arr, keep = L.make_tensors({self.RENAME.get(k, k): v for k, v in state_dict.items()})
        handle = C.c_void_p()
        with torch.cuda.device(self.device):
            L.check(self.lib.ttsamd_tagger_create(arr, len(arr), C.byref(cfg), C.byref(handle)), 'tagger_create')
        self.handle = handle
        self.ws = _Workspace()

    def __del__(self):
        if getattr(self, 'handle', None):
            self.lib.ttsamd_tagger_destroy(self.handle)
            self.handle = None

    def forward(self, ids):
        ids = torch.as_tensor(ids)
        _check_ids(ids, self.n_vocab, 'tagger ids')
        ids = ids.to(device=self.device, dtype=torch.int64).contiguous()
        B, T = ids.shape
        probs = torch.empty(B, T, self.n_classes, dtype=torch.float32, device=self.device)
        if T == 0:
            return probs
        with torch.cuda.device(self.device):
            nb = self.lib.ttsamd_tagger_workspace_bytes(self.handle, B, T)
            ws = self.ws.get(nb, self.device)
            L.check(self.lib.ttsamd_tagger_forward(self.handle, _ptr(ids), B, T, _ptr(probs), _ptr(ws), nb, _stream()),
                    'tagger_forward')
        return probs


def conv1d(x, w, bias=None, lens=None, dilation=1, in_slope=1.0, relu_out=False, res=None, mode=0, div=1.0, y=None, splitk_floats=None):
    lib = _require_gpu()
    x = x.contiguous().float()
    w = w.contiguous().float()
    B, cin, lin = x.shape
    cout, cin2, k = w.shape
    assert cin == cin2
    if y is None:
        y = torch.zeros(B, cout, lin, dtype=torch.float32, device=x.device)
    packed = torch.empty(lib.ttsamd_conv1d_packed_floats(cout, cin, k), dtype=torch.float32, device=x.device)
    with torch.cuda.device(x.device):
        if splitk_floats is None:
            L.check(lib.ttsamd_conv1d_ex(_ptr(x), _ptr(w), _ptr(bias), _ptr(res), _ptr(lens), B, cin, cout, k, dilation, lin,
                                         float(in_slope), int(relu_out), int(mode), float(div), _ptr(y), _ptr(packed), _stream()), 'conv1d')
        else:
            ws = torch.full((max(int(splitk_floats), 1),), float('nan'), dtype=torch.float32, device=x.device)
            L.check(lib.ttsamd_conv1d_splitk(_ptr(x), _ptr(w), _ptr(bias), _ptr(res), _ptr(lens), B, cin, cout, k, dilation, lin,
                                             float(in_slope), int(relu_out), int(mode), float(div), _ptr(y), _ptr(packed), _ptr(ws),
                                             int(splitk_floats), _stream()), 'conv1d_splitk')
    return y


def last_conv_launch():
    route, ksplit = C.c_int32(-1), C.c_int32(0)
    L.check(L.load().ttsamd_conv_last_launch(C.byref(route), C.byref(ksplit)), 'conv_last_launch')
    return route.value, ksplit.value


def conv_route(batch, cin, cout, k, lin, dilation=1, in_slope=1.0, relu_out=False, has_res=False, mode=0, splitk_floats=None):
    route, ksplit = C.c_int32(-1), C.c_int32(0)
    L.check(L.load().ttsamd_conv1d_route(batch, cin, cout, k, dilation, lin, float(in_slope), int(relu_out), int(bool(has_res)), mode,
                                         int(splitk_floats or 0), C.byref(route), C.byref(ksplit)), 'conv1d_route')
    return route.value, ksplit.value


def pair_route(batch, channels, k, lin, dilation=1):
    kernel, ntw, wm, points, name = C.c_int32(), C.c_int32(), C.c_int32(), C.c_int32(), C.c_char_p()
    L.check(L.load().ttsamd_resblock_pair_route(batch, channels, k, dilation, lin, C.byref(kernel), C.byref(ntw), C.byref(wm), C.byref(points),
                                                C.byref(name)), 'resblock_pair_route')
    return {'kernel': kernel.value, 'ntw': ntw.value, 'wino_phases': wm.value, 'points': points.value, 'name': name.value.decode()}


def conv_transpose1d(x, w, bias=None, lens=None, in_slope=1.0, y=None):
    lib = _require_gpu()
    x = x.contiguous().float()
    w = w.contiguous().float()
    B, cin, lin = x.shape
    cin2, cout, kt = w.shape
    assert cin == cin2 and kt % 2 == 0
    u = kt // 2
    if y is None:
        y = torch.zeros(B, cout, lin * u, dtype=torch.float32, device=x.device)
    assert tuple(y.shape) == (B, cout, lin * u) and y.is_contiguous() and y.dtype == torch.float32
    if lens is not None:
        lens = lens.to(device=x.device, dtype=torch.int64).contiguous()
    packed = torch.empty(max(int(lib.ttsamd_convt_packed_floats(cin, cout, u)), 1), dtype=torch.float32, device=x.device)
    with torch.cuda.device(x.device):
        L.check(lib.ttsamd_conv_transpose1d(_ptr(x), _ptr(w), _ptr(bias), _ptr(lens), B, cin, cout, u, lin, float(in_slope), _ptr(y),
                                            _ptr(packed), _stream()), 'conv_transpose1d')
    return y


def resblock_pair(x, w1, b1, w2, b2, dil, lens=None, len_mul=1, y=None, mode=0, div=1.0, slope=0.1, variant=2):
    lib = _require_gpu()
    x = x.contiguous().float()
    w1, w2, b1, b2 = (t.contiguous().float() for t in (w1, w2, b1, b2))
    B, Cc, Lx = x.shape
    k = w1.shape[2]
    assert tuple(w1.shape) == tuple(w2.shape) == (Cc, Cc, k)
    if y is None:
        assert mode == 0
        y = torch.zeros_like(x)
    if lens is not None:
        lens = lens.to(device=x.device, dtype=torch.int64).contiguous()
    n_packed = int(lib.ttsamd_resblock_pair_packed_floats(Cc, k, int(variant)))
    packed = torch.empty(max(n_packed, 1), dtype=torch.float32, device=x.device)
    with torch.cuda.device(x.device):
        L.check(lib.ttsamd_resblock_pair(_ptr(x), _ptr(y), _ptr(w1), _ptr(b1), _ptr(w2), _ptr(b2), Cc, k, int(dil), _ptr(lens),
                                         int(len_mul), Lx, B, int(mode), float(div), float(slope), int(variant), _ptr(packed),
                                         n_packed, _stream()), 'resblock_pair')
    return y


def resblock2(x, w1, b1, w2, b2, dil1, dil2, lens=None, len_mul=1, y=None, mode=0, div=1.0, slope=0.1, variant=2):
    lib = _require_gpu()
    x = x.contiguous().float()
    w1, w2, b1, b2 = (t.contiguous().float() for t in (w1, w2, b1, b2))
    B, Cc, Lx = x.shape
    k = w1.shape[2]
    assert tuple(w1.shape) == tuple(w2.shape) == (Cc, Cc, k)
    if y is None:
        assert mode == 0
        y = torch.zeros_like(x)
    if lens is not None:
        lens = lens.to(device=x.device, dtype=torch.int64).contiguous()
    n_packed = int(lib.ttsamd_resblock2_packed_floats(Cc, k, int(variant)))
    packed = torch.empty(max(n_packed, 1), dtype=torch.float32, device=x.device)
    with torch.cuda.device(x.device):
        L.check(lib.ttsamd_resblock2(_ptr(x), _ptr(y), _ptr(w1), _ptr(b1), _ptr(w2), _ptr(b2), Cc, k, int(dil1), int(dil2), _ptr(lens),
                                     int(len_mul), Lx, B, int(mode), float(div), float(slope), int(variant), _ptr(packed), n_packed,
                                     _stream()), 'resblock2')
    return y


def length_regulate(enc, reps, t_max):
    lib = _require_gpu()
    enc = enc.contiguous().float()
    reps = reps.contiguous().to(torch.int64)
    B, Cc, Lt = enc.shape
    out = torch.empty(B, Cc, t_max, dtype=torch.float32, device=enc.device)
    idx = torch.empty(B, t_max, dtype=torch.int32, device=enc.device)
    with torch.cuda.device(enc.device):
        L.check(lib.ttsamd_length_regulate(_ptr(enc), _ptr(reps), B, Lt, Cc, t_max, _ptr(out), _ptr(idx), _stream()),
                'length_regulate')
    return out, idx


OVERSMOOTH_KEYS = ('HQER', 'CSlope', 'CCentroid', 'CRoll95')
# ... 1127 lines not shown
```

tts-arabic-pytorch_amd/ttsamd/lib.py:

```python
import ctypes as C
import os

_HERE = os.path.dirname(os.path.abspath(__file__))
LIB_PATH = os.environ.get('TTSAMD_LIB') or os.path.join(_HERE, 'lib', 'libttsamd.so')


class TtsAmdError(RuntimeError):
    pass


class Tensor(C.Structure):
    _fields_ = [('name', C.c_char_p), ('data', C.POINTER(C.c_float)), ('ndim', C.c_int32),
                ('shape', C.c_int64 * 4)]


class HifiGanCfg(C.Structure):
    _fields_ = [('num_mels', C.c_int32), ('upsample_initial_channel', C.c_int32), ('n_ups', C.c_int32),
                ('upsample_rates', C.c_int32 * 8), ('upsample_kernel_sizes', C.c_int32 * 8),
                ('n_kernels', C.c_int32), ('resblock_kernel_sizes', C.c_int32 * 8),
                ('n_dilations', C.c_int32), ('resblock_dilations', (C.c_int32 * 8) * 8), ('resblock', C.c_int32)]


class FastPitchCfg(C.Structure):
    _fields_ = [(n, C.c_int32) for n in (
# ... 86 lines not shown
    'ttsamd_cepstral_series': (_I32, [_P, _P, _I32, _I32, _I32, _I32, _I32, _I32, _F, _P, _P, _P]),
    'ttsamd_cepstral_series_from_power': (_I32, [_P, _P, _I32, _I32, _I32, _I32, _I32, _I32, C.c_double, C.c_double, _F, _P, _P]),
    'ttsamd_series_summary': (_I32, [_P, _P, _I32, _I32, _I32, _P, _P, _P]),
    'ttsamd_dtw_workspace_bytes': (_I64, [_I32, _I32, _I32, _I32]),
    'ttsamd_dtw': (_I32, [_P, _P, _P, _P, _I32, _I32, _I32, _I32, _I32, _I32, _P, _P, _P, _P, _I64, _P]),
    'ttsamd_dtw_aligned_mae': (_I32, [_P, _P, _I32, _I32, _I32, _P, _P, _P, _P]),
    'ttsamd_mel_cepstrum': (_I32, [_P, _P, _I32, _I32, _I32, _I32, _P, _P]),
    'ttsamd_dtw_aligned_eval': (_I32, [_P, _P, _I32, _I32, _P, _P, _I32, _P, _P, _I32, _I32, _I32, _P, _P, C.c_double, _P, _P]),
    'ttsamd_aligner_create': (_I32, [C.POINTER(Tensor), _I32, C.POINTER(AlignerCfg), C.POINTER(_P)]),
    'ttsamd_aligner_destroy': (_I32, [_P]),
    'ttsamd_aligner_workspace_bytes': (_I64, [_P, _I32, _I32, _I32]),
    'ttsamd_aligner_forward': (_I32, [_P, _P, _P, _P, _P, _P, _I32, _I32, _I32, _P, _P, _P, _I64, _P]),
    'ttsamd_mas_workspace_bytes': (_I64, [_I32, _I32, _I32]),
    'ttsamd_mas': (_I32, [_P, _I32, _P, _P, _I32, _I32, _I32, _P, _P, _P, _I64, _P]),
    'ttsamd_average_pitch': (_I32, [_P, _P, _I32, _I32, _I32, _I32, _P, _P]),
    'ttsamd_attn_prior': (_I32, [_P, _P, _I32, _I32, _I32, _I32, C.c_double, _P, _P]),
    'ttsamd_attn_prior_tables': (_I32, [_I32, _P]),
    'ttsamd_attn_ctc_loss_workspace_bytes': (_I64, [_I32, _I32, _I32]),
    'ttsamd_attn_ctc_loss': (_I32, [_P, _P, _P, _I32, _I32, _I32, C.c_double, _P, _P, _I64, _P]),
    'ttsamd_attn_bin_loss': (_I32, [_P, _P, _I32, _I32, _I32, C.c_double, _P, _P, _P]),
    'ttsamd_pyin_tables': (_I32, [C.POINTER(PyinCfg), _P, _P, _P, _P, _P, _P, _P]),
    'ttsamd_pyin_create': (_I32, [C.POINTER(PyinCfg), C.POINTER(_P)]),
    'ttsamd_pyin_destroy': (_I32, [_P]),
    'ttsamd_pyin_workspace_bytes': (_I64, [_P, _I32, _I32]),
    'ttsamd_pyin_obs_offsets': (_I32, [_P, _I32, _I32, _P]),
    'ttsamd_pyin_forward': (_I32, [_P, _P, _I64, _P, _I32, _I32, _P, _P, _P, _P, _P, _P, _I64, _P]),
    'ttsamd_resample_create': (_I32, [_P, _I32, _I32, _I32, C.POINTER(_P)]),
    'ttsamd_resample_destroy': (_I32, [_P]),
    'ttsamd_resample_out_len': (_I64, [_P, _I64]),
    'ttsamd_resample_mfma_eligible': (_I32, [_P]),
    'ttsamd_resample_forward': (_I32, [_P, _P, _I64, _P, _I32, _P, _I64, _P, _I32, _P]),
    'ttsamd_trim_workspace_bytes': (_I64, [_I32, _I64, _I32]),
    'ttsamd_trim_bounds': (_I32, [_P, _I64, _P, _I32, _F, _I32, _I32, _F, _P, _P, _P, _I64, _P]),
    'ttsamd_trim_apply': (_I32, [_P, _I64, _P, _P, _F, _I64, _I32, _P, _I64, _P, _P]),
    'ttsamd_frames_compact': (_I32, [_P, _P, _P, _I32, _I32, _I32, _I32, _F, _P, _P, _P, _P]),
    'ttsamd_loudness_coefficients': (_I32, [_I32, C.POINTER(C.c_double)]),
    'ttsamd_loudness_workspace_bytes': (_I64, [_I32, _I64, _I32]),
    'ttsamd_loudness_measure': (_I32, [_P, _I64, _P, _I32, _I32, _P, _P, _P, _I64, _P]),
    'ttsamd_wave_level': (_I32, [_P, _I64, _P, _I32, _P, _P, _F, _P, _P, _P, _P]),
    'ttsamd_wave_limit_workspace_bytes': (_I64, [_I32, _I64]),
    'ttsamd_wave_limit': (_I32, [_P, _I64, _P, _I32, _P, _P, _F, _F, _I32, _I32, _P, _P, _P, _P, _I64, _P]),
    'ttsamd_true_peak_taps': (_I32, [C.POINTER(C.c_double)]),
    'ttsamd_true_peak': (_I32, [_P, _I64, _P, _I32, _P, _P]),
    'ttsamd_wave_limit_true_peak': (_I32, [_P, _I64, _P, _I32, _P, _P, _F, _F, _I32, _I32, _P, _P, _P, _P, _I64, _P]),
    'ttsamd_loudness_meter_workspace_bytes': (_I64, [_I32, _I64, _I32]),
    'ttsamd_loudness_meter': (_I32, [_P, _I64, _P, _I32, _I32, _P, _P, _P, _P, _P, _P, _P, _I64, _P, _I64, _P, _I64, _P]),
    'ttsamd_meter_state_bytes': (_I64, [_I32, _I64, _I32]),
    'ttsamd_meter_push_workspace_bytes': (_I64, [_I32, _I64, _I32]),
    'ttsamd_meter_reset': (_I32, [_P, _I64, _I32, _I64, _I32, _P, _I32, _P]),
    'ttsamd_meter_push': (_I32, [_P, _I64, _I32, _I64, _I32, _P, _I64, _P, _P, _I32, _P, _P, _P, _P, _I64, _P]),
    'ttsamd_meter_result': (_I32, [_P, _I64, _I32, _I64, _I32, _P, _I32, _P, _P, _P, _P, _P, _P, _P, _P]),
    'ttsamd_stoi_workspace_bytes': (_I64, [_I32, _I64]),
    'ttsamd_stoi': (_I32, [_P, _P, _I64, _P, _I32, _I32, _P, _P, _P, _P, _I32, _P, _I64, _P]),
    'ttsamd_wave_sdr': (_I32, [_P, _P, _I64, _P, _I32, _I32, _P, _P]),
    'ttsamd_log_spectral_distance': (_I32, [_P, _P, _I64, _P, _I32, _P, _P]),
    'ttsamd_mr_stft_workspace_bytes': (_I64, [_I32, _I64, C.POINTER(_I32), C.POINTER(_I32), C.POINTER(_I32), _I32]),
    'ttsamd_mr_stft': (_I32, [_P, _P, _I64, _P, _I32, C.POINTER(_I32), C.POINTER(_I32), C.POINTER(_I32), _I32, _P, _P, _P, _I64, _P]),
    'ttsamd_griffinlim_workspace_bytes': (_I64, [_I32, _I32, _F]),
    'ttsamd_griffinlim': (_I32, [_P, _P, _I32, _I32, _I32, _I32, _F, _I32, _P, C.c_uint64, _P, _P, _I64, _P, _P, _I64, _P]),
    'ttsamd_mel_to_linear': (_I32, [_P, _P, _I32, _I32, _I32, _P, _I32, _F, _P, _P]),
    'ttsamd_tacotron2_create': (_I32, [C.POINTER(Tensor), _I32, C.POINTER(Tacotron2Cfg), C.POINTER(_P)]),
    'ttsamd_tacotron2_destroy': (_I32, [_P]),
    'ttsamd_tacotron2_workspace_bytes': (_I64, [_P, _I32, _I32, _I32]),
    'ttsamd_tacotron2_infer': (_I32, [_P, _P, _P, _P, _I32, _I32, _I32, _I64, _P, _P, _P, _P,
                                      C.POINTER(_I32), _P, _I64, _P]),
    'ttsamd_tacotron2_stream_bytes': (_I64, [_P, _I32, _I32, _I32, _I32]),
    'ttsamd_tacotron2_stream_begin': (_I32, [_P, _P, _P, _P, _I32, _I32, _I32, _I32, _I64, _P, _I32, _P, _P, _P, _P, _I64,
                                             C.POINTER(_P), _P]),
    'ttsamd_tacotron2_stream_advance': (_I32, [_P, _I32, C.POINTER(_I32), C.POINTER(_I32), C.POINTER(_I32), _P]),
    'ttsamd_tacotron2_stream_end': (_I32, [_P]),
    'ttsamd_tacotron2_postnet_halo_frames': (_I32, [_P, C.POINTER(_I32)]),
    'ttsamd_tacotron2_postnet_window_bytes': (_I64, [_P, _I32, _I32]),
    'ttsamd_tacotron2_postnet_window': (_I32, [_P, _P, _P, _I32, _I32, _I32, _I32, _I32, _I32, _P, _I64, _P]),
    'ttsamd_tagger_create': (_I32, [C.POINTER(Tensor), _I32, C.POINTER(TaggerCfg), C.POINTER(_P)]),
    'ttsamd_tagger_destroy': (_I32, [_P]),
    'ttsamd_tagger_workspace_bytes': (_I64, [_P, _I32, _I32]),
    'ttsamd_tagger_forward': (_I32, [_P, _P, _I32, _I32, _P, _P, _I64, _P]),
    'ttsamd_conv1d_packed_floats': (_I64, [_I32, _I32, _I32]),
    'ttsamd_conv1d': (_I32, [_P, _P, _P, _P, _I32, _I32, _I32, _I32, _I32, _I32, _F, _I32, _P, _P, _P]),
    'ttsamd_conv1d_ex': (_I32, [_P, _P, _P, _P, _P, _I32, _I32, _I32, _I32, _I32, _I32, _F, _I32, _I32, _F, _P, _P, _P]),
    'ttsamd_conv1d_splitk': (_I32, [_P, _P, _P, _P, _P, _I32, _I32, _I32, _I32, _I32, _I32, _F, _I32, _I32, _F, _P, _P, _P, _I64, _P]),
    'ttsamd_conv_last_launch': (_I32, [C.POINTER(_I32), C.POINTER(_I32)]),
    'ttsamd_conv1d_route': (_I32, [_I32, _I32, _I32, _I32, _I32, _I32, _F, _I32, _I32, _I32, _I64, C.POINTER(_I32), C.POINTER(_I32)]),
    'ttsamd_convt_packed_floats': (_I64, [_I32, _I32, _I32]),
    'ttsamd_conv_transpose1d': (_I32, [_P, _P, _P, _P, _I32, _I32, _I32, _I32, _I32, _F, _P, _P, _P]),
    'ttsamd_convt_wino_packed_floats': (_I64, [_I32, _I32, _I32]),
    'ttsamd_convt_wino_pack_weight': (_I32, [_P, _P, _I32, _I32, _I32, _P]),
    'ttsamd_resblock_pair_packed_floats': (_I64, [_I32, _I32, _I32]),
    'ttsamd_resblock_pair': (_I32, [_P, _P, _P, _P, _P, _P, _I32, _I32, _I32, _P, _I32, _I32, _I32, _I32, _F, _F, _I32, _P, _I64, _P]),
    'ttsamd_resblock_pair_route': (_I32, [_I32, _I32, _I32, _I32, _I32] + [C.POINTER(_I32)] * 4 + [C.POINTER(C.c_char_p)]),
    'ttsamd_resblock2_packed_floats': (_I64, [_I32, _I32, _I32]),
    'ttsamd_resblock2': (_I32, [_P, _P, _P, _P, _P, _P, _I32, _I32, _I32, _I32, _P, _I32, _I32, _I32, _I32, _F, _F, _I32, _P, _I64, _P]),
    'ttsamd_set_precision': (_I32, [_I32]),
    'ttsamd_get_precision': (_I32, []),
    'ttsamd_dp_unique_id': (_I32, [_P]),
    'ttsamd_dp_init': (_I32, [_I32, _I32, _P, C.POINTER(_P)]),
    'ttsamd_dp_destroy': (_I32, [_P]),
    'ttsamd_dp_rank': (_I32, [_P]),
    'ttsamd_dp_world': (_I32, [_P]),
    'ttsamd_dp_broadcast': (_I32, [_P, _P, _I64, _I32, _P]),
    'ttsamd_dp_broadcast_weights': (_I32, [_P, _I32, _P, _I32, _P]),
    'ttsamd_dp_allgather': (_I32, [_P, _P, _P, _I64, _P]),
    'ttsamd_dp_pack_audio': (_I32, [_P, _I64, _P, _I32, _I64, _P, _P]),
    'ttsamd_dp_gather_audio': (_I32, [_P, _P, _P, C.POINTER(_I64), C.POINTER(_I64), _I32, _P]),
    'ttsamd_profile_enable': (_I32, [_I32]),
    'ttsamd_profile_read': (_I32, [C.POINTER(C.c_double)]),
}
_BFO = {
    'pack': (_I32, [_P, _I32, _I32, _I32, _F, _P, _P]),
    'unpack': (_I32, [_P, _I32, _I32, _I32, _F, _P, _P]),
    'weight_elems': (_I64, [_I32, _I32, _I32, _I32]),
    'pack_weight': (_I32, [_P, _I32, _I32, _I32, _I32, _P]),
    'conv1d': (_I32, [_P, _P, _P, _P, _P, _P, _I32, _I32, _I32, _I32, _I32, _I32, _I32, _I32, _I32, _F, _F, _F, _P, _P, _P, _P]),
    'resblock_pair': (_I32, [_P, _P, _P, _P, _P, _P, _P, _I32, _I32, _I32, _I32, _I32, _I32, _I32, _F, _F, _F, _F, _P, _P]),
    'resblock_chain': (_I32, [_P, _P, _P, _P, _P, _P, _P, _P, _I32, _I32, _I32, _I32, _I32, _F, _F, _F, _F, _P, _P, _I32]),
    'conv_post': (_I32, [_P, _P, _P, _P, _I32, _I32, _I32, _I32, _P, _I64, _P]),
}
for _prefix in ('bfo', 'bfo3'):
    for _name, (_res, _args) in _BFO.items():
        SYMBOLS[f'ttsamd_{_prefix}_{_name}'] = (_res, _args[:-1] if (_prefix, _name) == ('bfo3', 'resblock_chain') else _args)

_lib = None
ABI_VERSION = 8


def load():
    global _lib
    if _lib is not None:
        return _lib
    if not os.path.exists(LIB_PATH):
        raise TtsAmdError(f'{LIB_PATH} is missing: build it with `make -C tts-arabic-pytorch_amd/csrc` '
                          '(hipcc --offload-arch=gfx950); there is no CPU/PyTorch fallback')
    import torch
    lib = C.CDLL(LIB_PATH)
    for name, (res, args) in SYMBOLS.items():
        fn = getattr(lib, name)
        fn.restype, fn.argtypes = res, args
    got = lib.ttsamd_version()
    if got != ABI_VERSION:
        raise TtsAmdError(f'{LIB_PATH} was built from another revision of include/ttsamd.h (library ABI {got}, this binding '
                          f'{ABI_VERSION}): rebuild it with `make -C tts-arabic-pytorch_amd/csrc`')
    if lib.ttsamd_options_check() != 0:
        msg = lib.ttsamd_last_error()
        raise TtsAmdError(f'bad routing option in the environment: {msg.decode() if msg else "?"}')
    _lib = lib
    return lib


def set_option(name, value):
    v = None if value is None else str(value).encode()
    check(load().ttsamd_set_option(name.encode(), v), f'set_option({name}={value})')


def get_option(name):
    buf = C.create_string_buffer(64)
    check(load().ttsamd_get_option(name.encode(), buf, 64), f'get_option({name})')
    return buf.value.decode() or None


def option_names():
    lib, out, i = load(), [], 0
    while True:
        n = lib.ttsamd_option_name(i)
        if not n:
            return out
        out.append(n.decode())
# ... 48 lines not shown
```

Baseline: 81.01 million.

## Add row-packed Winograd conv form that packs ragged batch rows into shared tiles

Adds a row-packed variant (epilogues 8/9) of the wino4 fp32 conv kernel. Each block computes a per-row tuple prefix sum over the lengths with wave shuffles and maps its tiles onto live (row, tuple) slots. Tiles that fall in padding past each utterance's length are no longer launched, and the grid is capped by the packed tile count. The form is enabled by default through a new WINO4 mask bit and a block-threshold option. In exchange, every block does extra prefix-sum work and out-of-length inputs must be masked, which adds complexity and correctness risk.

```diff
diff --git a/include/ttsamd.h b/include/ttsamd.h
--- a/include/ttsamd.h
+++ b/include/ttsamd.h
@@ -311,6 +311,10 @@
 int32_t ttsamd_conv_last_launch(int32_t* route, int32_t* ksplit);
 int32_t ttsamd_conv1d_route(int32_t batch, int32_t cin, int32_t cout, int32_t k, int32_t dilation, int32_t lin, float in_slope,
                             int32_t relu_out, int32_t has_res, int32_t mode, int64_t splitk_floats, int32_t* route, int32_t* ksplit);
+int32_t ttsamd_conv1d_route_form(int32_t batch, int32_t cin, int32_t cout, int32_t k, int32_t dilation, int32_t lin, float in_slope,
+                                 int32_t relu_out, int32_t has_res, int32_t mode, int64_t splitk_floats, int32_t ragged, int32_t* route,
+                                 int32_t* ksplit, int32_t* form);
+int32_t ttsamd_conv_last_launch_form(int32_t* form, int64_t* rowpacked_launches);
 int64_t ttsamd_convt_packed_floats(int32_t cin, int32_t cout, int32_t u);
 int64_t ttsamd_convt_wino_packed_floats(int32_t cin, int32_t cout, int32_t u);
 int32_t ttsamd_convt_wino_pack_weight(const float* w, const float* bias, int32_t cin, int32_t cout, int32_t u, float* out);
diff --git a/profiles/launch_classes.py b/profiles/launch_classes.py
--- a/profiles/launch_classes.py
+++ b/profiles/launch_classes.py
@@ -4,26 +4,38 @@
 from collections import defaultdict
 
 
-def classes(path):
-    d = defaultdict(lambda: [0, 0])
-    other = 0
+def launches(path):
+    out, other = [], 0
     with open(path) as f:
-        for r in csv.DictReader(f):
-            dur = int(r['End_Timestamp']) - int(r['Start_Timestamp'])
-            m = re.search(r'conv1d_wino4_f32<(\d+), (\d+), (\d+), (\d+), (\d+), (\d+)>', r['Kernel_Name'])
-            if not m:
-                other += dur
-                continue
-            k, noct, nst, epi, lp, pt = map(int, m.groups())
-            key = (pt, k, lp, 'residual' if epi == 3 else 'plain', int(r['Grid_Size_X']) // int(r['Workgroup_Size_X']))
-            d[key][0] += 1
-            d[key][1] += dur
-    return d, other
+        rows = sorted(csv.DictReader(f), key=lambda r: int(r['Start_Timestamp']))
+    for r in rows:
+        dur = int(r['End_Timestamp']) - int(r['Start_Timestamp'])
+        m = re.search(r'conv1d_wino4_f32<(\d+), (\d+), (\d+), (\d+), (\d+), (\d+)>', r['Kernel_Name'])
+        if not m:
+            other += dur
+            continue
+        k, noct, nst, epi, lp, pt = map(int, m.groups())
+        key = (pt, k, lp, 'residual' if epi in (3, 8) else 'plain', int(r['Grid_Size_X']) // int(r['Workgroup_Size_X']))
+        out.append((key, epi in (8, 9), dur))
+    return out, other
 
 
-a, oa = classes(sys.argv[1])
-b, ob = classes(sys.argv[2])
-print(f'{"groups":>6} {"k":>3} {"window":>7} {"epilogue":>9} {"blocks":>7} {"calls":>6} {"us parent":>10} {"us tree":>9} {"ratio":>6}')
+la, oa = launches(sys.argv[1])
+lb, ob = launches(sys.argv[2])
+a, b = defaultdict(lambda: [0, 0]), defaultdict(lambda: [0, 0])
+form = {}
+in_order = len(la) == len(lb) and all(x[0][:4] == y[0][:4] for x, y in zip(la, lb))
+for i, (key, _, dur) in enumerate(la):
+    a[key][0] += 1
+    a[key][1] += dur
+for i, (key, rp, dur) in enumerate(lb):
+    pkey = la[i][0] if in_order else key
+    b[pkey][0] += 1
+    b[pkey][1] += dur
+    if rp:
+        form[pkey] = key[4]
+print(f'({"launches paired in order" if in_order else "launches paired by class"}; "row-packed": the grid of the tree\'s row-packed launch)')
+print(f'{"groups":>6} {"k":>3} {"window":>7} {"epilogue":>9} {"blocks":>7} {"calls":>6} {"us parent":>10} {"us tree":>9} {"ratio":>6} {"row-packed":>10}')
 ta = tb = 0
 for key in sorted(set(a) | set(b), key=lambda t: (-t[0], t[1], t[2], t[3], t[4])):
     ca, da = a.get(key, (0, 0))
@@ -32,5 +44,5 @@
     tb += db
     ua, ub = (da / ca / 1e3 if ca else float('nan')), (db / cb / 1e3 if cb else float('nan'))
     print(f'{"seven" if key[0] == 7 else "six":>6} {key[1]:3d} {"vector" if key[2] == 1 else "strip":>7} {key[3]:>9} {key[4]:7d} {max(ca, cb):6d} '
-          f'{ua:10.1f} {ub:9.1f} {ub / ua:6.3f}')
+          f'{ua:10.1f} {ub:9.1f} {ub / ua:6.3f} {form.get(key, ""):>10}')
 print(f'sum over the conv1d_wino4_f32 launches: {ta / 1e6:.2f} -> {tb / 1e6:.2f} ms; every other kernel: {oa / 1e6:.2f} -> {ob / 1e6:.2f} ms (whole trace)')
diff --git a/tts-arabic-pytorch_amd/csrc/api.hip b/tts-arabic-pytorch_amd/csrc/api.hip
--- a/tts-arabic-pytorch_amd/csrc/api.hip
+++ b/tts-arabic-pytorch_amd/csrc/api.hip
@@ -261,7 +261,8 @@
     errno = 0;
     const long long x = std::strtoll(v, &end, d.kind == 1 ? 16 : 10);
     if (!(errno == 0 && end != v && *end == '\0' && x >= d.lo && x <= d.hi)) return false;
-    if (&d == &kOpts[OPT_WINO4] && (((x & 32) && !(x & 2)) || ((x & 64) && !(x & 4)) || ((x & 128) && !(x & 8)))) return false;
+    if (&d == &kOpts[OPT_WINO4] &&
+        (((x & 32) && !(x & 2)) || ((x & 64) && !(x & 4)) || ((x & 128) && !(x & 8)) || ((x & 256) && !(x & 7)))) return false;
     return true;
 }
 void opt_init() {
@@ -936,20 +937,39 @@
     return rc;
 }
 
-int32_t ttsamd_conv1d_route(int32_t batch, int32_t cin, int32_t cout, int32_t k, int32_t dilation, int32_t lin, float in_slope,
-                            int32_t relu_out, int32_t has_res, int32_t mode, int64_t splitk_floats, int32_t* route, int32_t* ksplit) {
-    TTS_REQUIRE(route && ksplit, "conv1d_route: null argument");
+static int32_t conv1d_route_any(int32_t batch, int32_t cin, int32_t cout, int32_t k, int32_t dilation, int32_t lin, float in_slope,
+                                int32_t relu_out, int32_t has_res, int32_t mode, int64_t splitk_floats, bool ragged, ConvRoute& r) {
     TTS_REQUIRE(batch >= 1 && cin >= 1 && cout >= 1 && k >= 1 && lin >= 1 && dilation >= 1 && dilation <= 5 && splitk_floats >= 0,
                 "conv1d_route: bad shape");
     float* const any = reinterpret_cast<float*>((uintptr_t)256);
     ConvParams p;
-    TTS_TRY(conv1d_params(p, any, any, has_res ? any : nullptr, nullptr, batch, cin, cout, k, dilation, lin, in_slope, relu_out, mode, 1.f, any,
-                          any, any, splitk_floats));
+    TTS_TRY(conv1d_params(p, any, any, has_res ? any : nullptr, ragged ? reinterpret_cast<const int64_t*>(any) : nullptr, batch, cin, cout, k,
+                          dilation, lin, in_slope, relu_out, mode, 1.f, any, any, any, splitk_floats));
     TTS_REQUIRE(p.precision == 0, "conv1d_route: the bf16 launchers keep their own choices (precision %d)", p.precision);
-    const ConvRoute r = conv_route(p, conv_route_opts());
+    r = conv_route(p, conv_route_opts());
     TTS_REQUIRE(r.id >= 0 && (relu_out < 2 || k == 1 || k == 5), "conv1d_route: no fp32 kernel takes k = %d, Cin = %d, relu_out = %d", k, cin, relu_out);
+    return 0;
+}
+
+int32_t ttsamd_conv1d_route(int32_t batch, int32_t cin, int32_t cout, int32_t k, int32_t dilation, int32_t lin, float in_slope,
+                            int32_t relu_out, int32_t has_res, int32_t mode, int64_t splitk_floats, int32_t* route, int32_t* ksplit) {
+    TTS_REQUIRE(route && ksplit, "conv1d_route: null argument");
+    ConvRoute r;
+    TTS_TRY(conv1d_route_any(batch, cin, cout, k, dilation, lin, in_slope, relu_out, has_res, mode, splitk_floats, false, r));
     *route = r.id;
     *ksplit = r.ksplit;
+    return 0;
+}
+
+int32_t ttsamd_conv1d_route_form(int32_t batch, int32_t cin, int32_t cout, int32_t k, int32_t dilation, int32_t lin, float in_slope,
+                                 int32_t relu_out, int32_t has_res, int32_t mode, int64_t splitk_floats, int32_t ragged, int32_t* route,
+                                 int32_t* ksplit, int32_t* form) {
+    TTS_REQUIRE(route && ksplit && form, "conv1d_route_form: null argument");
+    ConvRoute r;
+    TTS_TRY(conv1d_route_any(batch, cin, cout, k, dilation, lin, in_slope, relu_out, has_res, mode, splitk_floats, ragged != 0, r));
+    *route = r.id;
+    *ksplit = r.ksplit;
+    *form = r.rowpack;
     return 0;
 }
 
@@ -962,6 +982,14 @@
 int32_t ttsamd_conv_last_launch(int32_t* route, int32_t* ksplit) {
     TTS_REQUIRE(route && ksplit, "conv_last_launch: null argument");
     last_conv_launch(route, ksplit);
+    return 0;
+}
+
+int32_t ttsamd_conv_last_launch_form(int32_t* form, int64_t* rowpacked_launches) {
+    TTS_REQUIRE(form && rowpacked_launches, "conv_last_launch_form: null argument");
+    int32_t route = 0, ksplit = 0;
+    last_conv_launch(&route, &ksplit, form);
+    *rowpacked_launches = rowpacked_conv_launches();
     return 0;
 }
 
diff --git a/tts-arabic-pytorch_amd/csrc/common.hpp b/tts-arabic-pytorch_amd/csrc/common.hpp
--- a/tts-arabic-pytorch_amd/csrc/common.hpp
+++ b/tts-arabic-pytorch_amd/csrc/common.hpp
@@ -53,7 +53,8 @@
     X(HIFIGAN_STREAMS, 0, 0, 1)    \
     X(WINO, 0, 0, 1)                                              \
     X(WINO2, 0, 0, 31)             \
-    X(WINO4, 0, 0, 255)            \
+    X(WINO4, 0, 0, 511)            \
+    X(WINO4_BLOCKS, 0, 1, 1 << 20)  \
     X(FUSED_PAIR, 0, 0, 1)                   \
     X(FUSED2, 0, 0, 1)                                           \
     X(FUSED2_MASK, 1, 0, 0x1ff)               \
@@ -152,12 +153,13 @@
               int n_phase);
 bool compact_order(const void* lens, int batch);
 int32_t launch_conv(const ConvParams& p, hipStream_t stream);
-struct ConvRouteOpts { int wino, wino2, wino4, deep_splitk; };
+struct ConvRouteOpts { int wino, wino2, wino4, deep_splitk, wino4_blocks; };
 struct ConvRoute {
     int id;
     int ksplit;
     int epi;
     int co_blk, nt_blk;
+    int rowpack;
 };
 ConvRouteOpts conv_route_opts();
 ConvRoute conv_route(const ConvParams& p, const ConvRouteOpts& o);
@@ -168,8 +170,9 @@
 constexpr int conv_chunk_channels(int k, int nt_blk, int co_blk) {
     return (k == 3 && nt_blk == 128 && co_blk == 128) ? 16 : (k == 1 ? 32 : (k == 2 ? 16 : 8));
 }
-void note_conv_launch(int32_t route, int32_t ksplit);
-void last_conv_launch(int32_t* route, int32_t* ksplit);
+void note_conv_launch(int32_t route, int32_t ksplit, int32_t form = 0);
+void last_conv_launch(int32_t* route, int32_t* ksplit, int32_t* form = nullptr);
+int64_t rowpacked_conv_launches();
 bool convt_supported(const ConvParams& p);
 int32_t launch_convt(const ConvParams& p, hipStream_t stream);
 int32_t launch_upsampler(ConvParams& p, const float* x, const float* w, const void* w_bf16, const float* bias, float* y, int cin, int cout,
@@ -214,13 +217,16 @@
 void pack_wino2_weight(const float* w, int cout, int cin, int k, float* out);
 int wino4_groups(int k);
 int wino44_groups(int k);
-constexpr int kWino4Default = 255;
+constexpr int kWino4Default = 511;
+constexpr int kWino4Blocks = 192;
 __device__ __host__ constexpr int wino4_tile(int d, int ntup) { return (4 * ntup / (4 * d)) * (4 * d); }
 __host__ __device__ constexpr int wino4_pk_tuples(int n, int d) { return d * ((n + 4 * d - 1) / (4 * d)); }
 __host__ __device__ constexpr int wino4_pk_tiles(int n, int d) { return (wino4_pk_tuples(n, d) + 63) / 64; }
 __host__ __device__ constexpr int wino4_pk_col(int t, int d) { return (t / d) * 4 * d + t % d; }
 __host__ __device__ constexpr int wino4_pk_q0(int tile, int d) { return (64 * tile / d) * 4 * d; }
 __host__ __device__ constexpr int wino4_pk_r0(int tile, int d) { return 64 * tile % d; }
+__host__ __device__ constexpr int wino4_rp_tuples(int n) { return (n + 3) / 4; }
+__host__ __device__ constexpr int64_t wino4_rp_tiles_max(int batch, int n_max) { return ((int64_t)batch * wino4_rp_tuples(n_max) + 63) / 64; }
 int32_t launch_splitk_reduce(const ConvParams& q, hipStream_t stream);
 int32_t launch_wino4(const ConvParams& p, const ConvRoute& r, hipStream_t stream);
 void wino4_filter_groups(const float* g, int k, float* o);
@@ -269,6 +275,48 @@
     }
     return false;
 }
+
+struct RowSlot { int row, tup, n, live; };
+__device__ __forceinline__ void rowpack_find(const int incl, const int T, const int n, const int gl, const int total, const int u0, RowSlot& s) {
+    int lo = 0;
+#pragma unroll
+    for (int step = 32; step >= 1; step >>= 1) {
+        const int v = __shfl(incl, lo + step - 1, 64);
+        if (v <= gl) lo += step;
+    }
+    const int excl = __shfl(incl - T, lo, 64), nr = __shfl(n, lo, 64);
+    if (gl >= 0 && gl < total) s = RowSlot{u0 + lo, gl - excl, nr, 1};
+}
+__device__ __forceinline__ int rowpack_slots(const int64_t* __restrict__ lens, const int mul, const int n_max, const int batch, const int ga,
+                                             const int gb, RowSlot& a, RowSlot& b) {
+    const int lane = threadIdx.x & 63;
+    int base = 0;
+    RowSlot last = {0, 0, 0, 0};
+    a = b = RowSlot{-1, 0, 0, 0};
+    for (int u0 = 0; u0 < batch; u0 += 64) {
+        int n = 0;
+        if (u0 + lane < batch) n = max(min(n_max, (int)lens[u0 + lane] * mul), 0);
+        const int T = wino4_rp_tuples(n);
+        int incl = T;
+#pragma unroll
+        for (int d = 1; d < 64; d <<= 1) {
+            const int t = __shfl_up(incl, d, 64);
+            if (lane >= d) incl += t;
+        }
+        const int total = __shfl(incl, 63, 64);
+        rowpack_find(incl, T, n, ga - base, total, u0, a);
+        rowpack_find(incl, T, n, gb - base, total, u0, b);
+        const unsigned long long m = __ballot(T > 0);
+        if (m != 0) {
+            const int l = 63 - __clzll((long long)m);
+            last = RowSlot{u0 + l, __shfl(T, l, 64) - 1, __shfl(n, l, 64), 0};
+        }
+        base += total;
+    }
+    if (a.row < 0) a = last;
+    if (b.row < 0) b = last;
+    return base;
+}
 #endif
 
 }
diff --git a/tts-arabic-pytorch_amd/csrc/conv_mfma.hip b/tts-arabic-pytorch_amd/csrc/conv_mfma.hip
--- a/tts-arabic-pytorch_amd/csrc/conv_mfma.hip
+++ b/tts-arabic-pytorch_amd/csrc/conv_mfma.hip
@@ -418,9 +418,17 @@
     *yp = v;
 }
 
-static thread_local int32_t t_last_route = -1, t_last_ksplit = 0;
-void note_conv_launch(int32_t route, int32_t ksplit) { t_last_route = route; t_last_ksplit = ksplit; }
-void last_conv_launch(int32_t* route, int32_t* ksplit) { *route = t_last_route; *ksplit = t_last_ksplit; }
+static thread_local int32_t t_last_route = -1, t_last_ksplit = 0, t_last_form = 0;
+static thread_local int64_t t_rowpacked = 0;
+void note_conv_launch(int32_t route, int32_t ksplit, int32_t form) {
+    t_last_route = route; t_last_ksplit = ksplit; t_last_form = form;
+    if (form == 1) ++t_rowpacked;
+}
+void last_conv_launch(int32_t* route, int32_t* ksplit, int32_t* form) {
+    *route = t_last_route; *ksplit = t_last_ksplit;
+    if (form) *form = t_last_form;
+}
+int64_t rowpacked_conv_launches() { return t_rowpacked; }
 
 int32_t launch_splitk_reduce(const ConvParams& q, hipStream_t stream) {
     dim3 rg((q.Nout + 255) / 256, q.Cout, q.batch);
@@ -516,7 +524,7 @@
              p.lens_out != nullptr, p.n_phase);
     if (p.precision != 0) return launch_conv_bf16_any(p, stream);
     TTS_REQUIRE(!p.x_packed && !p.y_packed, "conv: packed bf16 activations exist only in the bf16 mode");
-    if (r.id >= 0) note_conv_launch(r.id, r.ksplit);
+    if (r.id >= 0) note_conv_launch(r.id, r.ksplit, r.rowpack);
     if (r.id > 0) return r.id >= 3 ? launch_wino4(p, r, stream) : (r.id == 2 ? launch_wino2(p, stream) : launch_wino(p, stream));
     switch (p.K) {
         case 1: return launch_k<1>(p, r, stream);
diff --git a/tts-arabic-pytorch_amd/csrc/conv_route.hip b/tts-arabic-pytorch_amd/csrc/conv_route.hip
--- a/tts-arabic-pytorch_amd/csrc/conv_route.hip
+++ b/tts-arabic-pytorch_amd/csrc/conv_route.hip
@@ -5,11 +5,13 @@
 namespace ttsamd {
 
 ConvRouteOpts conv_route_opts() {
-    return {(int)opt_int(OPT_WINO, 1), (int)opt_int(OPT_WINO2, 31), (int)opt_int(OPT_WINO4, kWino4Default), (int)opt_int(OPT_DEEP_SPLITK, 1)};
+    return {(int)opt_int(OPT_WINO, 1), (int)opt_int(OPT_WINO2, 31), (int)opt_int(OPT_WINO4, kWino4Default), (int)opt_int(OPT_DEEP_SPLITK, 1),
+            (int)opt_int(OPT_WINO4_BLOCKS, kWino4Blocks)};
 }
 
-static int wino4_ksplit(const ConvParams& p, int64_t blocks) {
-    constexpr int sk_blocks = 192, sk_target = 224;
+static int wino4_ksplit(const ConvParams& p, int64_t blocks, const ConvRouteOpts& o) {
+    const int sk_blocks = std::min(kWino4Blocks, o.wino4_blocks);
+    constexpr int sk_target = 224;
     if (blocks >= sk_blocks || p.splitk_ws == nullptr) return 1;
     const int n_chunks = p.Cin / (p.K == 1 ? 32 : (p.K == 3 ? 16 : 8));
     const int64_t per = (int64_t)p.batch * p.Cout * p.Nout;
@@ -61,7 +63,7 @@
     if (p.K == 1) {
         if (!((o.wino4 & 16) && p.w != nullptr && p.dil == 1 && p.pad == 0 && p.Cin % 32 == 0 && !p.x_packed && !p.y_packed)) return direct;
         const int64_t tiles1 = (int64_t)((p.Nout + 255) / 256) * (p.CoutP / 64) * p.batch;
-        const int ks1 = wino4_ksplit(p, tiles1);
+        const int ks1 = wino4_ksplit(p, tiles1, o);
         return (tiles1 * ks1 >= 512 && p.Nout >= 256) ? ConvRoute{3, ks1, 0, 0, 0} : direct;
     }
     if ((p.w_wino == nullptr && p.w_wino4 == nullptr) || (p.K != 3 && p.K != 7 && p.K != 11)) return direct;
@@ -73,12 +75,16 @@
         if (takes(o.wino4)) {
             const int bo4 = wino4_tile(p.dil, 64);
             const int64_t tiles4 = (int64_t)((p.Nout + bo4 - 1) / bo4) * (p.CoutP / 64) * p.batch;
-            const int ks4 = wino4_ksplit(p, tiles4);
-            if (tiles4 * ks4 >= 192 && p.Nout >= 256) {
+            const int ks4 = wino4_ksplit(p, tiles4, o);
+            if (tiles4 * ks4 >= o.wino4_blocks && p.Nout >= 256) {
                 const bool seven = p.w_wino44 != nullptr && p.K != 3 && (o.wino4 & (p.K == 7 ? 32 : 64)) != 0;
                 const int epi = p.dil == 1 ? (ks4 != 1 ? 0 : (p.res != nullptr ? 3 : 4))
                                            : (((o.wino4 & 128) && p.res == nullptr && p.mode == 0 && ks4 == 1) ? 7 : 0);
-                return ConvRoute{(epi == 7 ? 7 : 3) + (seven ? 1 : 0), ks4, epi, 0, 0};
+                constexpr int64_t span_max = 0x7ffffff0;
+                const int rowpack = (o.wino4 & 256) && (epi == 3 || epi == 4) && (p.K == 3 || seven) && p.lens_out != nullptr && p.batch >= 2 &&
+                                    p.Nout < 16 * 256 && (int64_t)p.batch * p.x_bs * 4 < span_max && (int64_t)p.batch * p.y_bs * 4 < span_max &&
+                                    (p.res == nullptr || (int64_t)p.batch * p.r_bs * 4 < span_max);
+                return ConvRoute{(epi == 7 ? 7 : 3) + (seven ? 1 : 0), ks4, epi, 0, 0, rowpack ? 1 : 0};
             }
         }
         if (p.w_wino == nullptr) return direct;
diff --git a/tts-arabic-pytorch_amd/csrc/conv_wino4.hip b/tts-arabic-pytorch_amd/csrc/conv_wino4.hip
--- a/tts-arabic-pytorch_amd/csrc/conv_wino4.hip
+++ b/tts-arabic-pytorch_amd/csrc/conv_wino4.hip
@@ -13,9 +13,10 @@
 typedef float w4_f32x4 __attribute__((ext_vector_type(4)));
 typedef float w4_f32x2 __attribute__((ext_vector_type(2)));
 
-template <int K, int NOCT_, int NSTAGE_, int PT_ = 6, int LP_ = 1, int CT_ = 0, int PK_ = 0>
+template <int K, int NOCT_, int NSTAGE_, int PT_ = 6, int LP_ = 1, int CT_ = 0, int PK_ = 0, int RP_ = 0>
 struct Wino4Geo {
     static_assert(PK_ == 0 || LP_ == 2, "packed tiles: the strip kernels");
+    static_assert(RP_ == 0 || (LP_ == 1 && CT_ == 0 && K != 1), "row-packed tiles: the dilation-1 launches of k = 3 / 7 / 11");
     static constexpr bool PT7 = PT_ == 7;
     static_assert(PT_ == 6 || (PT7 && (K == 7 || K == 11)), "seven-point groups: k = 7 / 11");
     static_assert(CT_ == 0 || (K == 3 && PT_ == 6 && LP_ == 1), "transposed conv: the k = 3 six-point form at dilation 1");
@@ -86,6 +87,8 @@
     __host__ __device__ static constexpr int tw0v(int ph) { return DAV + 2 * nljv(ph); }
     __host__ __device__ static constexpr int wsv(int ph) { return (sgap(ph) - tw0v(ph)) / nwj(ph); }
     static_assert(LP_ != 1 || (wsv(0) >= 1 && wsv(NPH - 1) >= 1), "one write job per gap at most (vector loads)");
+    static constexpr int VLA = vlo(0), NVA = fdiv4(NPOS - 1 - (K - 1) / 2) - vlo(0) + 1;
+    static_assert(vlo(NPH - 1) >= VLA && vlo(NPH - 1) + nvec(NPH - 1) <= VLA + NVA && nvec(0) <= NVA, "the window's vectors");
     __host__ __device__ static constexpr int strip_need(int d) {
         return 3 + (PK_ ? wino4_pk_col(d - 1 + 63, d) : wino4_pk_col(4 * 64 / (4 * d) * d - 1, d)) + (NPOS - 1) * d + 1;
     }
@@ -144,7 +147,8 @@
     constexpr int CTU = EPI == 5 ? 8 : (EPI == 6 ? 2 : 0);
     constexpr bool CT = CTU != 0;
     constexpr bool PK = EPI == 7;
-    using G = Wino4Geo<K, NOCT_, NSTAGE_, PT, LP, CTU, PK ? 1 : 0>;
+    constexpr bool RP = EPI == 8 || EPI == 9;
+    using G = Wino4Geo<K, NOCT_, NSTAGE_, PT, LP, CTU, PK ? 1 : 0, RP ? 1 : 0>;
     constexpr bool PT7 = G::PT7;
     constexpr int WN = G::WN, NSF = G::NSF, NOCT = G::NOCT, NSTAGE = G::NSTAGE, NPL = G::NPL, NGPM = G::NGPM;
     constexpr int CO_BLK = G::CO_BLK, NTUP = G::NTUP, NT_BLK = G::NT_BLK, PF = G::PF;
@@ -160,9 +164,15 @@
     const unsigned gt = (u / (unsigned)per_tile) * 8u + xcd;
     const int n_tiles_x = PK ? wino4_pk_tiles(p.Nout, dil) : (p.Nout + nt_eff - 1) / nt_eff;
     const int tile_w = PK ? 1 : nt_eff;
-    int b = (int)(gt / (unsigned)n_tiles_x);
-    int q0 = (int)(gt % (unsigned)n_tiles_x) * tile_w;
-    if (p.compact) {
+    int b = RP ? 0 : (int)(gt / (unsigned)n_tiles_x);
+    int q0 = RP ? 0 : (int)(gt % (unsigned)n_tiles_x) * tile_w;
+    RowSlot rs_s = {0, 0, 0, 0}, rs_e = {0, 0, 0, 0};
+    if constexpr (RP) {
+        const int tuples = __builtin_amdgcn_readfirstlane(
+            rowpack_slots(p.lens_out, p.len_out_mul, p.Nout, p.batch, 64 * (int)gt + (int)(threadIdx.x & 63),
+                          64 * (int)gt + (int)((threadIdx.x >> 6) % WN) * 32 + (int)(threadIdx.x & 31), rs_s, rs_e));
+        if (64 * (int64_t)gt >= (int64_t)tuples) return;
+    } else if (p.compact) {
         int tile = 0;
         if (!live_tile<CT ? 1 : 0, PK>(p.lens_out, p.len_out_mul, p.Nout, nt_eff, p.batch, gt, b, tile, dil)) return;
         b = __builtin_amdgcn_readfirstlane(b);
@@ -188,9 +198,16 @@
     } else {
         if (p.lens_out) n_out = min(n_out, (int)p.lens_out[b] * p.len_out_mul);
     }
-    if (q0 >= n_out) return;
+    if (!RP && q0 >= n_out) return;
     int in_len = p.Lin;
-    if (p.lens_in) in_len = min(in_len, (int)p.lens_in[b] * p.len_in_mul);
+    if (p.lens_in) in_len = min(in_len, (int)p.lens_in[RP ? rs_s.row : b] * p.len_in_mul);
+    bool vok[RP ? G::NVA : 1][4];
+    if constexpr (RP) {
+#pragma unroll
+        for (int va = 0; va < G::NVA; ++va)
+#pragma unroll
+            for (int e = 0; e < 4; ++e) vok[va][e] = rs_s.tup + G::VLA + va >= 0 && 4 * (rs_s.tup + G::VLA + va) + e < in_len;
+    }
 
     const int x_cs = p.x_cs, CoutP = p.CoutP;
     const int chunks_all = p.Cin / (8 * NOCT);
@@ -199,10 +216,11 @@
     const float* __restrict__ xb = p.x + (int64_t)b * p.x_bs;
     const float in_slope = p.in_slope;
 
-    constexpr bool REG = EPI >= 3, RES = EPI == 3;
+    constexpr bool REG = EPI >= 3, RES = EPI == 3 || EPI == 8;
     static_assert(!REG || ((LP == 1 || PK) && K != 1), "register epilogue: dilation 1 or the packed strip form, k = 3 / 7 / 11");
     static_assert(!PK || LP == 2, "packed tiles: the strip kernels");
-    static_assert(EPI <= 7 && (!CT || K == 3), "epilogues 0, 3, 4, 7 and the transposed conv's 5 / 6 (k = 3 form)");
+    static_assert(EPI <= 9 && (!CT || K == 3), "epilogues 0, 3, 4, 7, the row-packed 8 / 9 and the transposed conv's 5 / 6 (k = 3 form)");
+    static_assert(!RP || (LP == 1 && !PK && !CT), "row-packed tiles: EPI 3 / 4 at dilation 1");
     float ep_bias = 0.f;
     if constexpr (!REG) {
         if (tid < CO_BLK && p.bias) ep_bias = p.bias[min(co_blk0 + tid, p.Cout - 1)];
@@ -217,16 +235,21 @@
 #pragma unroll
         for (int r = 0; r < 16; ++r) acc[g][r] = 0.f;
     const int ep_row0 = REG ? co_blk0 + __builtin_amdgcn_readfirstlane(wm) * 32 : 0;
-    const int ep_voff = (q0 + col_e < n_out ? q0 + col_e : 0) * 4;
+    const int ep_q = RP ? 4 * rs_e.tup : q0 + col_e;
+    const int ep_n = RP ? (rs_e.live ? rs_e.n : 0) : n_out;
+    const int ep_voff = RP ? ((RES ? (int)(rs_e.row * p.r_bs) : 0) + ep_q) * 4 :(q0 + col_e < n_out ? q0 + col_e : 0) * 4;
     const int ep_rrow = ep_row0 + 4 * kk;
-    const bfo_i4 ep_rs = bfo_rsrc(RES ? p.res + (int64_t)b * p.r_bs : nullptr, RES ? (unsigned)p.Cout * (unsigned)p.r_cs * 4u : 0u);
+    const bfo_i4 ep_rs = bfo_rsrc(RES ? p.res + (int64_t)b * p.r_bs : nullptr,
+                                  RES ? (RP ? (unsigned)((p.batch - 1) * p.r_bs + (int64_t)p.Cout * p.r_cs) * 4u : (unsigned)p.Cout * (unsigned)p.r_cs * 4u) : 0u);
     const bfo_i4 ep_bs = bfo_rsrc(p.bias, (REG && p.bias) ? (unsigned)p.Cout * 4u : 0u);
     w4_f32x4 rq[RES ? 16 : 1], bsq[REG ? 4 : 1];
     constexpr int EP_T0 = RES ? 16 : 0;
 #define TTS_EPLOAD_JOB(T)                                                                            \
     {                                                                                                \
-        if (RES && (T) < 16)                                                                         \
-            rq[RES ? (T) : 0] = __builtin_bit_cast(w4_f32x4, bfo_ld16(ep_rs, ep_voff + (ep_rrow + ((T) & 3) + 8 * ((T) >> 2)) * p.r_cs * 4, 0, 0)); \
+        if (RES && (T) < 16) {                                                                       \
+            const int rr_ = ep_rrow + ((T) & 3) + 8 * ((T) >> 2);                                    \
+            rq[RES ? (T) : 0] = __builtin_bit_cast(w4_f32x4, bfo_ld16(ep_rs, (RP && rr_ >= p.Cout) ? BFO_OOB : ep_voff + rr_ * p.r_cs * 4, 0, 0)); \
+        }                                                                                            \
         if ((T) >= EP_T0 && (T) < EP_T0 + 4)                                                         \
             bsq[REG ? (T) - EP_T0 : 0] = __builtin_bit_cast(w4_f32x4, bfo_ld16(ep_bs, (ep_rrow + 8 * ((T) - EP_T0)) * 4, 0, 0)); \
     }
@@ -254,7 +277,8 @@
     w4_f32x2 ta[NOCT], tb[NOCT];
     w4_f32x2 tf[PT7 ? 5 : 1], te[PT7 ? 4 : 1], td[PT7 ? 3 : 1], th[PT7 ? 2 : 1];
     const int spe = PK ? r0 + lane : min(lane, ntup_eff - 1);
-    const int xw0 = (q0 + 4 * lane) * 4;
+    const int xw0 = RP ? ((int)(rs_s.row * p.x_bs) + 4 * rs_s.tup) * 4 : (q0 + 4 * lane) * 4;
+    const unsigned x_span = RP ? (unsigned)((p.batch - 1) * p.x_bs + p.Lin) * 4u : 0u;
     constexpr int pad_c = (K - 1) / 2;
     const int ch_off = (4 * sh + skk) * x_cs;
 
@@ -264,12 +288,22 @@
 #define TTS_VLOAD_JOB(PH, J, XSO)                                                                    \
     {                                                                                                \
         TTS_VJOB_IDX(PH, J)                                                                          \
-        const bfo_i4 xrs_ = bfo_rsrc(xb + ((XSO) + ch_off + (8 * ol_ + 2 * pp_) * x_cs), (unsigned)in_len * 4u);     \
+        const bfo_i4 xrs_ = bfo_rsrc(xb + ((XSO) + ch_off + (8 * ol_ + 2 * pp_) * x_cs), RP ? x_span : (unsigned)in_len * 4u);     \
         sv[ol_][pp_][vi_] = __builtin_bit_cast(w4_f32x4, bfo_ld16(xrs_, xw0 + 16 * (G::vlo(PH) + vi_), 0, 0));      \
     }
 #define TTS_VACT_JOB(PH, A)                                                                          \
     {                                                                                                \
         TTS_VJOB_IDX(PH, (A) / 2)                                                                    \
+        if constexpr (RP) {                                                                          \
+            const int va_ = G::vlo(PH) + vi_ - G::VLA;                                         \
+            if ((A) % 2 == 0) {                                                                      \
+                sv[ol_][pp_][vi_].x = vok[va_][0] ? sv[ol_][pp_][vi_].x : 0.f;                       \
+                sv[ol_][pp_][vi_].y = vok[va_][1] ? sv[ol_][pp_][vi_].y : 0.f;                       \
+            } else {                                                                                 \
+                sv[ol_][pp_][vi_].z = vok[va_][2] ? sv[ol_][pp_][vi_].z : 0.f;                       \
+                sv[ol_][pp_][vi_].w = vok[va_][3] ? sv[ol_][pp_][vi_].w : 0.f;                       \
+            }                                                                                        \
+        }                                                                                            \
         if ((A) % 2 == 0) {                                                                          \
             sv[ol_][pp_][vi_].x = bfo_lrelu(sv[ol_][pp_][vi_].x, in_slope);                          \
             sv[ol_][pp_][vi_].y = bfo_lrelu(sv[ol_][pp_][vi_].y, in_slope);                          \
@@ -595,10 +629,12 @@
         return;
     }
     if constexpr (REG) {
-        const int q = q0 + col_e, y_cs = p.y_cs;
-        if (q >= n_out) return;
-        const bool full = q + 3 < n_out;
-        const bfo_i4 ys = bfo_rsrc(yb, (unsigned)Cout * (unsigned)y_cs * 4u);
+        const int q = ep_q, y_cs = p.y_cs;
+        if (q >= ep_n) return;
+        const bool full = q + 3 < ep_n;
+        const int64_t y_row = RP ? rs_e.row * p.y_bs : 0;
+        const int yv_off = RP ? ((int)y_row + q) * 4 : ep_voff;
+        const bfo_i4 ys = bfo_rsrc(yb, RP ? (unsigned)((p.batch - 1) * p.y_bs + (int64_t)Cout * y_cs) * 4u : (unsigned)Cout * (unsigned)y_cs * 4u);
         const float lo = relu_out == 1 ? 0.f : -__builtin_inff();
         constexpr int PB = NPL >= 8 ? 4 : 8;
 #pragma unroll
@@ -608,8 +644,9 @@
             for (int i = 0; i < PB; ++i) {
                 const int r = PB * h + i;
                 pq[i] = w4_f32x4{0.f, 0.f, 0.f, 0.f};
+                const int rr = ep_rrow + (r & 3) + 8 * (r >> 2);
                 if (mode != 0)
-                    pq[i] = __builtin_bit_cast(w4_f32x4, bfo_ld16(ys, ep_voff + (ep_rrow + (r & 3) + 8 * (r >> 2)) * y_cs * 4, 0, 0));
+                    pq[i] = __builtin_bit_cast(w4_f32x4, bfo_ld16(ys, (RP && rr >= Cout) ? BFO_OOB : yv_off + rr * y_cs * 4, 0, 0));
             }
 #pragma unroll
             for (int i = 0; i < PB; ++i) {
@@ -632,13 +669,13 @@
                     }
                 }
                 if (co >= Cout) continue;
-                float* yp = yb + (int64_t)co * y_cs + q;
+                float* yp = yb + y_row + (int64_t)co * y_cs + q;
                 if (full) {
                     *reinterpret_cast<w4_f32x4*>(yp) = v;
                 } else {
 #pragma unroll
                     for (int e = 0; e < 4; ++e)
-                        if (q + e < n_out) yp[e] = v[e];
+                        if (q + e < ep_n) yp[e] = v[e];
                 }
             }
         }
@@ -698,7 +735,8 @@
 template <int K, int NOCT, int NSTAGE, int EPI, int LP, int PT = 6>
 static int32_t launch_wino4_epi(const ConvParams& p, int ksplit, hipStream_t stream) {
     constexpr bool PK = EPI == 7;
-    using G = Wino4Geo<K, NOCT, NSTAGE, PT, LP, 0, PK ? 1 : 0>;
+    constexpr bool RP = EPI == 8 || EPI == 9;
+    using G = Wino4Geo<K, NOCT, NSTAGE, PT, LP, 0, PK ? 1 : 0, RP ? 1 : 0>;
     constexpr size_t ring = (size_t)G::NSTAGE * G::BUF4 * sizeof(float4);
     constexpr size_t epi = ((size_t)G::CO_BLK * G::NT_BLK + G::CO_BLK) * sizeof(float);
     constexpr size_t strip = LP == 2 ? (size_t)G::RAW_BYTES : 0;
@@ -711,7 +749,8 @@
     const int nt = wino4_tile(p.dil, G::NTUP);
     ConvParams q = p;
     q.ksplit = ksplit;
-    const int64_t n_tiles = (int64_t)(PK ? wino4_pk_tiles(p.Nout, p.dil) : (p.Nout + nt - 1) / nt) * p.batch;
+    int64_t n_tiles = (int64_t)(PK ? wino4_pk_tiles(p.Nout, p.dil) : (p.Nout + nt - 1) / nt) * p.batch;
+    if (RP) n_tiles = std::min(n_tiles, wino4_rp_tiles_max(p.batch, p.Nout));
     const int64_t n_blocks = ((n_tiles + 7) / 8) * 8 * (p.CoutP / G::CO_BLK) * q.ksplit;
     TTS_REQUIRE(n_blocks < ((int64_t)1 << 31), "wino4: %lld blocks", (long long)n_blocks);
     dim3 grid((unsigned)n_blocks, 1, 1);
@@ -726,6 +765,11 @@
 static int32_t launch_wino4_cfg(const ConvParams& p, const ConvRoute& r, hipStream_t stream) {
     if (p.dil == 1) {
         if (r.epi == 0) return launch_wino4_epi<K, NOCT, NSTAGE, 0, 1, PT>(p, r.ksplit, stream);
+        if constexpr (K == 3 || PT == 7) {
+            if (r.rowpack) return r.epi == 3 ? launch_wino4_epi<K, NOCT, NSTAGE, 8, 1, PT>(p, r.ksplit, stream)
+                                             : launch_wino4_epi<K, NOCT, NSTAGE, 9, 1, PT>(p, r.ksplit, stream);
+        }
+        TTS_REQUIRE(!r.rowpack, "wino4: no row-packed form of k = %d on six-point groups", K);
         if (r.epi == 3) return launch_wino4_epi<K, NOCT, NSTAGE, 3, 1, PT>(p, r.ksplit, stream);
         return launch_wino4_epi<K, NOCT, NSTAGE, 4, 1, PT>(p, r.ksplit, stream);
     }
diff --git a/tts-arabic-pytorch_amd/ttsamd/engine.py b/tts-arabic-pytorch_amd/ttsamd/engine.py
--- a/tts-arabic-pytorch_amd/ttsamd/engine.py
+++ b/tts-arabic-pytorch_amd/ttsamd/engine.py
@@ -866,6 +866,20 @@
     return route.value, ksplit.value
 
 
+def conv_route_form(batch, cin, cout, k, lin, dilation=1, in_slope=1.0, relu_out=False, has_res=False, mode=0, splitk_floats=None, ragged=True):
+    route, ksplit, form = C.c_int32(-1), C.c_int32(0), C.c_int32(0)
+    L.check(L.load().ttsamd_conv1d_route_form(batch, cin, cout, k, dilation, lin, float(in_slope), int(relu_out), int(bool(has_res)), mode,
+                                              int(splitk_floats or 0), int(bool(ragged)), C.byref(route), C.byref(ksplit), C.byref(form)),
+            'conv1d_route_form')
+    return route.value, ksplit.value, form.value
+
+
+def last_conv_launch_form():
+    form, n = C.c_int32(0), C.c_int64(0)
+    L.check(L.load().ttsamd_conv_last_launch_form(C.byref(form), C.byref(n)), 'conv_last_launch_form')
+    return form.value, n.value
+
+
 def pair_route(batch, channels, k, lin, dilation=1):
     kernel, ntw, wm, points, name = C.c_int32(), C.c_int32(), C.c_int32(), C.c_int32(), C.c_char_p()
     L.check(L.load().ttsamd_resblock_pair_route(batch, channels, k, dilation, lin, C.byref(kernel), C.byref(ntw), C.byref(wm), C.byref(points),
diff --git a/tts-arabic-pytorch_amd/ttsamd/lib.py b/tts-arabic-pytorch_amd/ttsamd/lib.py
--- a/tts-arabic-pytorch_amd/ttsamd/lib.py
+++ b/tts-arabic-pytorch_amd/ttsamd/lib.py
@@ -192,6 +192,9 @@
     'ttsamd_conv1d_splitk': (_I32, [_P, _P, _P, _P, _P, _I32, _I32, _I32, _I32, _I32, _I32, _F, _I32, _I32, _F, _P, _P, _P, _I64, _P]),
     'ttsamd_conv_last_launch': (_I32, [C.POINTER(_I32), C.POINTER(_I32)]),
     'ttsamd_conv1d_route': (_I32, [_I32, _I32, _I32, _I32, _I32, _I32, _F, _I32, _I32, _I32, _I64, C.POINTER(_I32), C.POINTER(_I32)]),
+    'ttsamd_conv1d_route_form': (_I32, [_I32, _I32, _I32, _I32, _I32, _I32, _F, _I32, _I32, _I32, _I64, _I32, C.POINTER(_I32), C.POINTER(_I32),
+                                        C.POINTER(_I32)]),
+    'ttsamd_conv_last_launch_form': (_I32, [C.POINTER(_I32), C.POINTER(_I64)]),
     'ttsamd_convt_packed_floats': (_I64, [_I32, _I32, _I32]),
     'ttsamd_conv_transpose1d': (_I32, [_P, _P, _P, _P, _I32, _I32, _I32, _I32, _I32, _F, _P, _P, _P]),
     'ttsamd_convt_wino_packed_floats': (_I64, [_I32, _I32, _I32]),
```

Measured after the change: 81.33 million (median of 6 runs). About the same (+0.4%).
